# shuaigroup/Renormalizer

Hardware: AMD Instinct MI355X
Metric: TDVP-PS sweep site-updates/sec at (Nsite=50, Dbond=256, dphys=2/16) (higher is better)
Workload: dtype c128

## Files before the change

### include/mpsengine.h

```cpp
#ifndef MPSENGINE_H
#define MPSENGINE_H

#include <stddef.h>
#include <stdint.h>

#ifdef __cplusplus
extern "C" {
#endif

typedef struct mpse_ctx mpse_ctx;

enum {
  MPSE_OK = 0,
  MPSE_ERR_OOM = 1,
  MPSE_ERR_SHAPE = 2,
  MPSE_ERR_NOCONV = 3,
  MPSE_ERR_HIP = 4,
  MPSE_ERR_ARG = 5
};

enum { MPSE_F64 = 0, MPSE_C128 = 1 };
enum { MPSE_DOMAIN_L = 0, MPSE_DOMAIN_R = 1 };


// ... 6 lines not shown

int mpse_prof_get_ktiles(mpse_ctx* ctx, int variant, int64_t* ktiles);
int mpse_prof_get_svd_sweeps(mpse_ctx* ctx, int64_t* sweeps);
int mpse_prof_enable(mpse_ctx* ctx, int on);
int mpse_prof_reset(mpse_ctx* ctx);
int mpse_prof_get(mpse_ctx* ctx, int variant, double* total_ms, double* total_flops, double* total_bytes,
                  int64_t* launches);


int mpse_malloc(mpse_ctx* ctx, size_t bytes, void** dptr);
int mpse_free(mpse_ctx* ctx, void* dptr);
int mpse_pool_trim(mpse_ctx* ctx);
int mpse_mem_info(mpse_ctx* ctx, size_t* pool_bytes, size_t* in_use_bytes, size_t* device_free, size_t* device_total);
int mpse_memcpy_h2d(mpse_ctx* ctx, void* dst, const void* src_host, size_t bytes);
int mpse_memcpy_d2h(mpse_ctx* ctx, void* dst_host, const void* src, size_t bytes);
int mpse_memcpy_d2d(mpse_ctx* ctx, void* dst, const void* src, size_t bytes);
int mpse_memset_zero(mpse_ctx* ctx, void* dst, size_t bytes);
int mpse_memcpy_2d(mpse_ctx* ctx, void* dst, size_t dpitch, const void* src, size_t spitch, size_t width_bytes,
                   size_t height);

int mpse_cast_f64_to_c128(mpse_ctx* ctx, void* dst, const void* src, int64_t n);
int mpse_conj_inplace(mpse_ctx* ctx, void* x, int64_t n);
int mpse_scal(mpse_ctx* ctx, int dtype, void* x, int64_t n, double a_re, double a_im);
int mpse_axpy(mpse_ctx* ctx, int dtype, void* y, const void* x, int64_t n, double a_re, double a_im);
int mpse_mul_real(mpse_ctx* ctx, int dtype, void* x, const void* m_f64, int64_t n);
int mpse_davidson_precond(mpse_ctx* ctx, int dtype, void* out, const void* r, const void* hdiag_f64,
                          const void* mask_f64, int64_t n, double e, double shift);
int mpse_real_part(mpse_ctx* ctx, void* out_f64, const void* z_c128, int64_t n);
int mpse_dotc(mpse_ctx* ctx, int dtype, const void* x, const void* y, int64_t n, double* out_host);
int mpse_nrm2(mpse_ctx* ctx, int dtype, const void* x, int64_t n, double* out_host);

int mpse_scaled_rms(mpse_ctx* ctx, int dtype, const void* x, const void* y1, const void* y2, int64_t n, double rtol,
                    double atol, double* out_host);

int mpse_defer_begin(mpse_ctx* ctx, int list);
int mpse_defer_end(mpse_ctx* ctx);
int mpse_defer_arm(mpse_ctx* ctx, int list);
int mpse_defer_run(mpse_ctx* ctx, int list);
int mpse_defer_discard(mpse_ctx* ctx);


typedef struct {
  int64_t ext;
  int64_t lo_ext;
  int64_t s_hi;
  int64_t s_lo;
} mpse_index;

typedef struct {
  int dtype_a, dtype_b;
  int conj_a, conj_b;
  mpse_index m_a, k_a;
  mpse_index k_b, n_b;
  mpse_index m_c, n_c;
  int64_t batch;
  int64_t sb_a, sb_b, sb_c;
  double alpha_re, alpha_im;
  double beta_re, beta_im;
  int skip_zero_tiles;
} mpse_gemm_desc;

int mpse_gemm(mpse_ctx* ctx, const mpse_gemm_desc* desc, const void* A, const void* B, void* C);

int mpse_gemm_path_stats(mpse_ctx* ctx, int64_t* counts, int n);

int mpse_transpose_inner(mpse_ctx* ctx, int dtype, void* out, const void* in,
                         int64_t d0, int64_t d1, int64_t d2, int conj);


typedef struct {
  int64_t Dl_bra, Dl_ket;
  int64_t Dr_bra, Dr_ket;
  int64_t d0, d1;
  int64_t danc;
  int64_t wl, wm, wr;
  int64_t env_unit;
  int64_t danc1;
} mpse_dims;

int mpse_env_update(mpse_ctx* ctx, int dtype, int domain, const mpse_dims* dims,
                    const void* env, int env_dtype, const void* ket, const void* bra, int bra_conj,
                    const void* W, int w_dtype, void* out);

int mpse_env_update_multi(mpse_ctx* ctx, int dtype, int domain, const mpse_dims* dims, int n_mpo,
                          const int64_t* wl, const int64_t* wr, const void* env, int env_dtype,
                          const void* ket, const void* bra, int bra_conj, const void* const* W, int w_dtype, void* out);

int mpse_env_unit_channel(mpse_ctx* ctx, int dtype, const void* env, int64_t D, int64_t w, double tol,
                          int64_t* unit_host);

typedef struct {
  int nsite;
  mpse_dims dims;
  const void* L; int l_dtype;
  const void* R; int r_dtype;
  const void* W0; const void* W1; int w_dtype;
  int64_t l_unit, r_unit;
} mpse_heff;

int mpse_heff_apply(mpse_ctx* ctx, int dtype, const mpse_heff* h, const void* C, void* out);

int mpse_mpo_site_hint(mpse_ctx* ctx, const void* W_dev, const double* W_host_f64, int64_t wl, int64_t d, int64_t wr);

int mpse_heff_fused_stats(mpse_ctx* ctx, int64_t* bond_launches, int64_t* site_launches);

int mpse_heff_apply2(mpse_ctx* ctx, int dtype, const mpse_heff* h, const void* C, void* out);

enum { MPSE_LEG_UP = 0, MPSE_LEG_DOWN = 1 };
typedef struct {
  int64_t Dl, Dr, d_up, d_down;
  int64_t wl1, wr1, wl2, wr2;
  int leg1, leg2;
  int trans1, trans2;
  const void* L; int l_dtype;
  const void* R; int r_dtype;
  const void* W1; const void* W2; int w_dtype;
} mpse_heff_ft;

int mpse_heff_apply_ft(mpse_ctx* ctx, int dtype, const mpse_heff_ft* h, const void* C, void* out);

int mpse_env_update_ft(mpse_ctx* ctx, int dtype, int domain, const mpse_heff_ft* h, const void* env, int env_dtype,
                       const void* X, void* out);

int mpse_expm_centre_mask(mpse_ctx* ctx, const void* mask_dev, int64_t nbytes);

int mpse_expm_lanczos(mpse_ctx* ctx, int dtype, const mpse_heff* h, double dt_re, double dt_im,
                      const void* C, void* out, double rtol, double atol, int max_dim, int* nvec);
int mpse_expm_lanczos_batch(mpse_ctx* ctx, int dtype, int count, const mpse_heff* h, double dt_re, double dt_im,
                            const void* const* C, void* const* out, double rtol, double atol, int max_dim, int* nvec);
int mpse_expm_lanczos_batch_stats(mpse_ctx* ctx, int64_t* batched_members, int64_t* single_members);
int mpse_expm_lanczos_path_stats(mpse_ctx* ctx, int64_t* counts, int n);

int mpse_davidson(mpse_ctx* ctx, int dtype, const mpse_heff* h, int twolayer, const void* hdiag_f64,
                  const void* mask_f64, int nroots, int nguess, const void* guess, double tol, int max_cycle,
                  int max_space, double lindep, double shift, double* e_host, void* x_out, int* ncycle, int* nmatvec);

int mpse_pcg(mpse_ctx* ctx, int dtype, const mpse_heff* h, int twolayer, double shift, const void* diag_f64,
             const void* mask_f64, const void* b, void* x, double tol, int max_iter, int* iters_host,
             double* relres_host, double* lvalue_host);
int mpse_pcg_stats(mpse_ctx* ctx, int64_t* counts, int n);

int mpse_pcg_batch(mpse_ctx* ctx, int dtype, int count, const mpse_heff* h, int twolayer, const double* shift_host,
                   const void* const* diag_f64, const void* const* mask_f64, const void* const* b, void* const* x,
                   double tol, int max_iter, int* status_host, int* iters_host, double* relres_host,
                   double* lvalue_host);
int mpse_pcg_batch_stats(mpse_ctx* ctx, int64_t* counts, int n);
int mpse_pcg_batch_plan(int dtype, int64_t Dl, int64_t d, int64_t Dr, int64_t wl, int64_t wr, int64_t* info, int n);

int mpse_pcg_sum(mpse_ctx* ctx, int dtype, int nterms, const mpse_heff_ft* terms, const double* weights_host,
                 double shift, const void* diag_f64, const void* mask_f64, const void* b, void* x, double tol,
                 int max_iter, int* iters_host, double* relres_host, double* lvalue_host);
int mpse_pcg_sum_stats(mpse_ctx* ctx, int64_t* counts, int n);

int mpse_site_factor_ft(mpse_ctx* ctx, const mpse_heff_ft* h, void* S_f64);
int mpse_diag_ft(mpse_ctx* ctx, const mpse_heff_ft* h, const void* S_f64, double weight, double shift, int accumulate,
                 void* diag_f64);


int mpse_mps_overlap(mpse_ctx* ctx, int nsite, const void* const* bra, const int* bra_dtype, const void* const* ket,
                     const int* ket_dtype, const int64_t* dims , int conj_bra, double* out_re_im_host);
int mpse_mps_overlap_stats(mpse_ctx* ctx, int64_t* counts, int n);
int mpse_mps_overlap_plan(int nsite, const int64_t* dims, int any_complex, int64_t* info, int n);


int mpse_mps_sandwich(mpse_ctx* ctx, int nsite, const void* const* bra, const int* bra_dtype, const void* const* ket,
                      const int* ket_dtype, const void* const* W, const int* w_dtype, const int64_t* dims ,
// ... 60 lines not shown
```

### renormalizer_amd/csrc/mpse_contract.hip

```cpp
#include <deque>

#include "mpse_internal.h"
#include "mpse_plans.h"

using namespace mpse_plan;

namespace {

__device__ __forceinline__ long long off2(const mpse_index m, long long i) {
  if (m.lo_ext >= m.ext) return i * m.s_lo;
  const long long hi = i / m.lo_ext;
  return hi * m.s_hi + (i - hi * m.lo_ext) * m.s_lo;
}

template <typename T>
__global__ __launch_bounds__(256) void k_copy_strided(T* dst, const T* src, mpse_index mi, mpse_index ni, mpse_index mo,
                                                      mpse_index no, const int* skip) {
  if (skip && *skip) return;
  const long long nn = ni.ext;
  const long long total = mi.ext * nn;
  const long long stride = (long long)gridDim.x * blockDim.x;
  for (long long t = (long long)blockIdx.x * blockDim.x + threadIdx.x; t < total; t += stride) {
    const long long i = t / nn, j = t - i * nn;
    dst[off2(mo, i) + off2(no, j)] = src[off2(mi, i) + off2(ni, j)];
  }
}

template <bool CPLX>
__global__ __launch_bounds__(256) void k_unit_deviation(const double* env, int D, int w, unsigned long long* dev) {
  constexpr int E = CPLX ? 2 : 1;
  const int a = blockIdx.x;
  __shared__ double red[4];
  for (int b = 0; b < w; ++b) {
    const double* row = env + ((long long)a * w + b) * D * E;
    double m = 0.0;
    for (int c = threadIdx.x; c < D; c += 256) {
      double re = row[c * E] - (c == a ? 1.0 : 0.0);
      double v = fabs(re);
      if (!(v <= 1e300)) v = 1e300;
      if (CPLX) {
        double vi = fabs(row[c * E + 1]);
        if (!(vi <= 1e300)) vi = 1e300;
        v = fmax(v, vi);
      }
      m = fmax(m, v);
    }
    for (int o = 32; o > 0; o >>= 1) m = fmax(m, __shfl_xor(m, o));
    if ((threadIdx.x & 63) == 0) red[threadIdx.x >> 6] = m;
    __syncthreads();
    if (threadIdx.x == 0) {
      m = fmax(fmax(red[0], red[1]), fmax(red[2], red[3]));
      atomicMax(dev + b, (unsigned long long)__double_as_longlong(m));
    }
    __syncthreads();
  }
}

struct WsmArgs {
  const double* T1;
  double* T2;
  const double* W;
  int Da, d, wl, wr, N;
  const int* skip;
  const double* slices;
  long long slice_stride;
  int nslices, b_lo, b_hi;
};

template <bool CPLX>
__global__ __launch_bounds__(256) void k_wsmall(const WsmArgs g) {
  if (g.skip && *g.skip) return;
  constexpr int E = CPLX ? 2 : 1;
  __shared__ double s_w[16][16];
  const int nrow = g.wl * g.d, no = g.d * g.wr;
  {
    const int o = threadIdx.x >> 4, be = threadIdx.x & 15;
    double v = 0.0;
    if (o < no && be < nrow) {
      const int dd = o / g.wr, f = o - dd * g.wr, b = be / g.d, e = be - b * g.d;
      v = g.W[(((long long)b * g.d + dd) * g.d + e) * g.wr + f];
    }
    s_w[o][be] = v;
  }
  __syncthreads();
  const long long idx = (long long)blockIdx.x * 256 + threadIdx.x;
  if (idx >= (long long)g.Da * g.N) return;
  const int a = (int)(idx / g.N), n = (int)(idx - (long long)a * g.N);
  double xr[16], xi[16];
#pragma unroll
  for (int be = 0; be < 16; ++be) {
    xr[be] = 0.0;
    xi[be] = 0.0;
    if (be < nrow) {
      const int b = be / g.d, e = be - b * g.d;
      if (g.nslices > 0 && b >= g.b_lo && b < g.b_hi) {
        const double* src = g.slices + ((((long long)(b - g.b_lo) * g.Da + a) * g.d + e) * g.N + n) * E;
        for (int sl = 0; sl < g.nslices; ++sl) {
          xr[be] += src[0];
          if constexpr (CPLX) xi[be] += src[1];
          src += g.slice_stride * E;
        }
      } else {
        const double* src = g.T1 + ((((long long)b * g.Da + a) * g.d + e) * g.N + n) * E;
        xr[be] = src[0];
        if constexpr (CPLX) xi[be] = src[1];
      }
    }
// ... 57 lines not shown
  const int x0 = q * WM_CHUNK;
  for (int j = 0; j < g.ndst; ++j) {
    const WmixDstDev& D = g.dst[j];
    double ar[WM_CHUNK], ai[WM_CHUNK];
#pragma unroll
    for (int i = 0; i < WM_CHUNK; ++i) ar[i] = 0.0, ai[i] = 0.0;
    for (int t = 0; t < D.nterm; ++t) {
      const WmixTermDev& tm = D.term[t];
      const double* src = tm.src + ((long long)a * tm.s_a + k) * E;
      if (tm.ident) {
#pragma unroll
        for (int i = 0; i < WM_CHUNK; ++i)
          if (x0 + i < d) {
            const double* p = src + (long long)(x0 + i) * tm.s_d * E;
            ar[i] += p[0];
            if constexpr (CPLX) ai[i] += p[1];
          }
        continue;
      }
      const double* blk = s_blk + tm.slot * dd2;
      const int lo = tm.e_lo[q], hi = tm.e_hi[q];
      for (int e0 = lo; e0 < hi; e0 += 8) {
        double vr[8], vi[8];
#pragma unroll
        for (int u = 0; u < 8; ++u) {
          vr[u] = 0.0, vi[u] = 0.0;
          if (e0 + u < hi) {
            const double* p = src + (long long)(e0 + u) * tm.s_d * E;
            vr[u] = p[0];
            if constexpr (CPLX) vi[u] = p[1];
          }
        }
#pragma unroll
        for (int u = 0; u < 8; ++u)
          if (e0 + u < hi) {
#pragma unroll
            for (int i = 0; i < WM_CHUNK; ++i)
              if (x0 + i < d) {
                const double w = blk[(x0 + i) * d + e0 + u];
                ar[i] += w * vr[u];
                if constexpr (CPLX) ai[i] += w * vi[u];
              }
          }
      }
    }
    double* dst = D.dst + ((long long)a * D.s_a + k) * E;
#pragma unroll
    for (int i = 0; i < WM_CHUNK; ++i)
      if (x0 + i < d) {
        double* p = dst + (long long)(x0 + i) * D.s_d * E;
        if constexpr (CPLX)
          *reinterpret_cast<double2*>(p) = make_double2(ar[i], ai[i]);
        else
          p[0] = ar[i];
      }
  }
}

int copy_call(mpse_ctx* ctx, int dtype, const void* src, void* dst, mpse_index mi, mpse_index ni, mpse_index mo,
              mpse_index no, const int* skip) {
  const long long total = mi.ext * ni.ext;
  if (total <= 0) return MPSE_OK;
  long long nb = (total + 255) / 256;
  if (nb > 65536) nb = 65536;
  if (dtype == MPSE_C128)
    hipLaunchKernelGGL((k_copy_strided<double2>), dim3((unsigned)nb), dim3(256), 0, ctx->stream, (double2*)dst,
                       (const double2*)src, mi, ni, mo, no, skip);
  else
    hipLaunchKernelGGL((k_copy_strided<double>), dim3((unsigned)nb), dim3(256), 0, ctx->stream, (double*)dst,
                       (const double*)src, mi, ni, mo, no, skip);
  MPSE_HIP(ctx, hipGetLastError());
  return MPSE_OK;
}

struct PlanRun {
  mpse_ctx* ctx;
  int dtype;
  size_t es;
  const void* bufs[B_COUNT];
  SolveScope* sc;
  MatvecReq* mv;
  const int* skip;
  MatvecReq::Dot* dot;
  TmpBuf slices;
  int slices_used = 0;
  PlanRun(mpse_ctx* c, int dt, const void* const* b, SolveScope* s, MatvecReq* m)
      : ctx(c), dtype(dt), es(dtype_size(dt)), sc(s), mv(m), skip(s ? s->skip : nullptr),
        dot(m && m->dot.y ? &m->dot : nullptr), slices(c) {
    for (int i = 0; i < B_COUNT; ++i) bufs[i] = b[i];
  }
  template <class T>
  int resolve(int buf, int64_t off, int dt, T** p) const {
    if (!bufs[buf]) return mpse_fail(ctx, MPSE_ERR_ARG, "plan: missing buffer");
    *p = (T*)((char*)const_cast<void*>(bufs[buf]) + size_t(off) * dtype_size(dt));
    return MPSE_OK;
  }
};

int run_wsmall(PlanRun& r, const Step& s) {
  WsmArgs g;
  MPSE_TRY(r.resolve(s.a, s.a_off, s.dta, &g.W));
  MPSE_TRY(r.resolve(s.b, s.b_off, s.dtb, &g.T1));
  MPSE_TRY(r.resolve(s.c, s.c_off, s.dtb, &g.T2));
  g.Da = (int)s.w_Da, g.d = (int)s.w_d, g.wl = (int)s.w_wl, g.wr = (int)s.w_wr, g.N = (int)s.w_N;
  g.skip = r.skip;
  g.slices = r.slices_used > 0 ? r.slices.as<const double>() : nullptr;
  g.nslices = r.slices_used, g.slice_stride = s.slice_elems, g.b_lo = (int)s.slice_b_lo, g.b_hi = (int)s.slice_b_hi;
  r.slices_used = 0;
  const long long total = s.w_Da * s.w_N;
  const dim3 grid((unsigned)((total + 255) / 256));
  if (s.dtb == MPSE_C128)
    hipLaunchKernelGGL((k_wsmall<true>), grid, dim3(256), 0, r.ctx->stream, g);
  else
    hipLaunchKernelGGL((k_wsmall<false>), grid, dim3(256), 0, r.ctx->stream, g);
  MPSE_HIP(r.ctx, hipGetLastError());
  return MPSE_OK;
}

int run_wmix(PlanRun& r, const Step& s) {
  WmixArgs g;
  memset(&g, 0, sizeof(g));
  MPSE_TRY(r.resolve(s.b, 0, MPSE_F64, &g.W));
  g.ndst = (int)s.mix.size();
  g.Da = (int)s.wp_Da, g.d = (int)s.wp_d, g.wr = (int)s.wp_wr, g.Dk = (int)s.wp_Dk;
  g.nchunk = (g.d + WM_CHUNK - 1) / WM_CHUNK;
  g.skip = r.skip;
  int nslot = 0;
  for (int j = 0; j < g.ndst; ++j) {
    const WMixDst& q = s.mix[j];
    MPSE_TRY(r.resolve(q.dst, q.dst_off, r.dtype, &g.dst[j].dst));
    g.dst[j].s_a = q.s_a, g.dst[j].s_d = q.s_d, g.dst[j].nterm = q.nterm;
    for (int t = 0; t < q.nterm; ++t) {
      const WMixTerm& tm = q.term[t];
      WmixTermDev& o = g.dst[j].term[t];
      MPSE_TRY(r.resolve(tm.src, tm.src_off, r.dtype, &o.src));
      o.s_a = tm.s_a, o.s_d = tm.s_d, o.b = tm.b, o.f = tm.f, o.ident = tm.ident ? 1 : 0;
      o.slot = tm.ident ? 0 : nslot++;
      memcpy(o.e_lo, tm.e_lo, sizeof(o.e_lo));
      memcpy(o.e_hi, tm.e_hi, sizeof(o.e_hi));
    }
  }
  g.nslot = nslot;
  const size_t lds = size_t(nslot > 0 ? nslot : 1) * g.d * g.d * sizeof(double);
  if (lds > 64 * 1024) return mpse_fail(r.ctx, MPSE_ERR_SHAPE, "plan: MPO blocks of the elementwise step exceed the LDS");
  const long long total = (long long)s.wp_Da * g.nchunk * s.wp_Dk;
  const dim3 grid((unsigned)((total + 255) / 256));
  if (r.dtype == MPSE_C128)
    hipLaunchKernelGGL((k_wmix<true>), grid, dim3(256), lds, r.ctx->stream, g);
  else
    hipLaunchKernelGGL((k_wmix<false>), grid, dim3(256), lds, r.ctx->stream, g);
  ++r.ctx->gemm_paths[mpse_ctx::GP_WMIX];
  MPSE_HIP(r.ctx, hipGetLastError());
  return MPSE_OK;
}

int scan_flags(PlanRun& r, const ScanDesc& sd, TmpBuf& tmp, const unsigned char** flags, int* pitch, bool* stable) {
  if (!sd.on || !r.bufs[sd.buf]) return MPSE_OK;
  const char* ptr;
  MPSE_TRY(r.resolve(sd.buf, sd.off, sd.dt, &ptr));
  bool st = false;
  MPSE_TRY(occ_mask_get(r.ctx, r.sc, ptr, sd.dt, sd.r, sd.k, tmp, flags, pitch, &st));
  *stable = *stable && st;
  return MPSE_OK;
}

const unsigned char* centre_mask(const PlanRun& r, const Step& s, int* pitch) {
  const int64_t K = s.kb.ext, N = s.nb.ext;
  const int64_t nkw = ((K + 15) / 16 + 7) / 8, ntn = (N + 63) / 64;
  if (!r.sc || !r.sc->in_krylov(r.bufs[B_C]) || r.sc->cmask.bytes != ntn * nkw * 8) return nullptr;
  *pitch = (int)(nkw * 8);
  return static_cast<const unsigned char*>(r.sc->cmask.ptr);
}

int bind_epilogue_mix(PlanRun& r, const GGroupPlan& g, int i, GroupedDesc& gd) {
  if (gd.nmix > 0 || !r.bufs[g.wbuf]) return mpse_fail(r.ctx, MPSE_ERR_ARG, "plan: bad epilogue mix");
  gd.nmix = g.nmix, gd.mix_grp = i;
  gd.mix_w = r.bufs[g.wbuf];
  gd.mix_d = (int)g.mix_d, gd.mix_wr = (int)g.mix_wr, gd.mix_ld = g.mix_ld;
  for (int t = 0; t < g.nmix; ++t) {
    const EpiTerm& m = g.mix[t];
    MPSE_TRY(r.resolve(m.src, m.src_off, r.dtype, &gd.mix[t].src));
    gd.mix[t].b = m.b, gd.mix[t].f = m.f, gd.mix[t].delta = m.delta;
  }
  return MPSE_OK;
}

int run_ggemm(PlanRun& r, const Step& s) {
  GroupedDesc gd;
  gd.dta = s.dta, gd.dtb = s.dtb;
  gd.ma = s.ma, gd.ka = s.ka, gd.kb = s.kb, gd.nb = s.nb, gd.mc = s.mc, gd.nc = s.nc;
  gd.ngrp = (int)s.groups.size();
  TmpBuf MA(r.ctx), MB(r.ctx);
  const unsigned char *fa = nullptr, *fb = nullptr;
  bool stable = true;
  MPSE_TRY(scan_flags(r, s.scan_a, MA, &fa, &gd.am_pitch, &stable));
  MPSE_TRY(scan_flags(r, s.scan_b, MB, &fb, &gd.bm_pitch, &stable));
  int cm_pitch = 0;
  const unsigned char* cm = centre_mask(r, s, &cm_pitch);
  for (int i = 0; i < gd.ngrp; ++i) {
    const GGroupPlan& g = s.groups[i];
    GroupedGrp& o = gd.grp[i];
    MPSE_TRY(r.resolve(g.cbuf, g.c_off, r.dtype, &o.C));
    o.nseg = g.nseg;
    o.beta = g.beta;
    if (g.nmix > 0) MPSE_TRY(bind_epilogue_mix(r, g, i, gd));
    for (int q = 0; q < g.nseg; ++q) {
      const GSegPlan& sg = g.seg[q];
      MPSE_TRY(r.resolve(sg.abuf, sg.a_off, s.dta, &o.seg[q].A));
      MPSE_TRY(r.resolve(sg.bbuf, sg.b_off, s.dtb, &o.seg[q].B));
      if (fa && sg.am_row0 >= 0) o.seg[q].am = fa + size_t(sg.am_row0) * gd.am_pitch;
      if (sg.bm_kind == BM_SCAN && fb) {
        o.seg[q].bm = fb + sg.bm_kt0;
      } else if (sg.bm_kind == BM_CENTRE && cm) {
        o.seg[q].bm = cm;
        gd.bm_pitch = cm_pitch;
      }
    }
  }
  gd.masks_stable = stable;
  if (gd.ngrp == 1 && s.groups[0].split2) {
    if (!r.bufs[B_OUT2]) return mpse_fail(r.ctx, MPSE_ERR_ARG, "plan: missing second result");
    gd.split2 = true;
    gd.c2 = const_cast<void*>(r.bufs[B_OUT2]);
  }
  MPSE_TRY(gemm_grouped(r.ctx, gd, r.sc, s.completes ? r.dot : nullptr,
                        s.completes && r.mv && r.mv->out_mask.mask ? &r.mv->out_mask : nullptr));
  return MPSE_OK;
}

int run_product(PlanRun& r, const Step& s) {
  const int dtc = (s.dta == MPSE_C128 || s.dtb == MPSE_C128) ? MPSE_C128 : MPSE_F64;
  if (dtc != r.dtype)
    return mpse_fail(r.ctx, MPSE_ERR_ARG, "plan step dtype mismatch (got %d want %d)", dtc, r.dtype);
  const char *a, *b;
  char* c;
  MPSE_TRY(r.resolve(s.a, s.a_off, s.dta, &a));
  MPSE_TRY(r.resolve(s.b, s.b_off, s.dtb, &b));
  MPSE_TRY(r.resolve(s.c, s.c_off, dtc, &c));
  if (s.kind == K_COPY) return copy_call(r.ctx, dtc, a, c, s.ma, s.ka, s.mc, s.nc, r.skip);
  ProductReq rq;
  if (s.completes) rq.dot = r.dot;
  if (s.cin >= 0) {
    if (!r.bufs[s.cin]) return mpse_fail(r.ctx, MPSE_ERR_ARG, "plan: missing beta source");
    rq.cin = (const char*)r.bufs[s.cin] + size_t(s.cin_off) * dtype_size(dtc);
    rq.cin_m = s.mcin;
    rq.cin_n = s.ncin;
  }
  if (s.slices_to >= 0) {
    const size_t blk = size_t(s.mc.ext) * size_t(s.nc.ext) * dtype_size(dtc);
    if (r.slices.alloc(4 * blk) == MPSE_OK) {
      rq.slices = r.slices.p;
      rq.slices_cap = 4 * blk;
    }
  }
  MPSE_TRY(gemm_call(r.ctx, s.dta, s.dtb, s.conja, s.conjb, s.ma, s.ka, s.kb, s.nb, s.mc, s.nc, s.batch, s.sba, s.sbb,
                     s.sbc, a, b, c, 1.0, s.beta, s.skip_zero, r.sc, &rq));
  if (rq.slices_used > 0) r.slices_used = rq.slices_used;
  return MPSE_OK;
}

}

static int run_plan(mpse_ctx* ctx, int dtype, const Plan& p, const void* bufs_in[B_COUNT],
                    SolveScope* sc = nullptr, MatvecReq* mv = nullptr) {
  if (p.error) return mpse_fail(ctx, MPSE_ERR_SHAPE, "%s", p.error);
  TmpBuf t1(ctx), t2(ctx), t3(ctx);
  TmpBuf* tmp[3] = {&t1, &t2, &t3};
  PlanRun r(ctx, dtype, bufs_in, sc, mv);
  for (int i = 0; i < 3; ++i)
    if (p.tmp_elems[i]) {
      MPSE_TRY(tmp[i]->alloc(size_t(p.tmp_elems[i]) * r.es));
      r.bufs[B_T1 + i] = tmp[i]->p;
    }
  for (const Step& s : p.steps)
    MPSE_TRY(s.elementwise_w ? run_wsmall(r, s)
             : s.kind == K_WMIX ? run_wmix(r, s)
             : s.kind == K_GGEMM ? run_ggemm(r, s)
                                 : run_product(r, s));
  return MPSE_OK;
}

int heff_apply(mpse_ctx* ctx, int dtype, const mpse_heff* h, const void* C, void* out, SolveScope* sc,
               MatvecReq* mv) {
  if (!ctx || !h || !C || !out || !h->L || !h->R) return MPSE_ERR_ARG;
  MPSE_BIND(ctx);
  if (dtype != MPSE_C128 && (h->l_dtype == MPSE_C128 || h->r_dtype == MPSE_C128 || h->w_dtype == MPSE_C128))
    return mpse_fail(ctx, MPSE_ERR_ARG, "heff_apply: real centre with complex operator parts");
  std::shared_ptr<void> wi_keep;
  if (h->nsite == 1 && h->W0) {
    std::lock_guard<std::mutex> lock(ctx->pool_mu);
    auto it = ctx->wsite_info.find(h->W0);
    if (it != ctx->wsite_info.end()) wi_keep = it->second.info;
  }
  {
    bool taken = false;
    MPSE_TRY(heff_small_try(ctx, dtype, h, C, out, sc, mv, &taken));
    if (taken) return MPSE_OK;
    const WSiteInfo* wi0 = static_cast<const WSiteInfo*>(wi_keep.get());
    const bool wi_ok = wi0 && h->nsite == 1 && wi0->wl == h->dims.wl && wi0->d == h->dims.d0 && wi0->wr == h->dims.wr;
    MPSE_TRY(heff0_fused_try(ctx, dtype, h, C, wi_ok ? wi0->w.data() : nullptr, sc, mv, &taken));
    if (taken) return MPSE_OK;
  }
  MatvecReq::Parts* pr = mv && mv->parts.ptr ? &mv->parts : nullptr;
  const bool two_ok = pr && pr->cap_elems >= 2 * pr->n;
  Plan p = plan_heff(dtype, *h, static_cast<const WSiteInfo*>(wi_keep.get()), two_ok, fold_epi());
  if (pr) pr->used = 0;
  const void* bufs[B_COUNT] = {nullptr};
  bind_heff(bufs, *h, C, out);
  if (p.two_results) bufs[B_OUT2] = static_cast<char*>(pr->ptr) + size_t(pr->n) * dtype_size(dtype);
  MPSE_TRY(run_plan(ctx, dtype, p, bufs, sc, mv));
  if (p.two_results) pr->used = -2;
  return MPSE_OK;
}

extern "C" int mpse_heff_apply(mpse_ctx* ctx, int dtype, const mpse_heff* h, const void* C, void* out) {
  return heff_apply(ctx, dtype, h, C, out, nullptr, nullptr);
}

extern "C" int mpse_mpo_site_hint(mpse_ctx* ctx, const void* W_dev, const double* W_host, int64_t wl, int64_t d,
                                  int64_t wr) {
  if (!ctx || !W_dev) return MPSE_ERR_ARG;
  if (!W_host) {
    std::lock_guard<std::mutex> lock(ctx->pool_mu);
    ctx->wsite_info.erase(W_dev);
    return MPSE_OK;
  }
  if (wl <= 0 || d <= 0 || wr <= 0) return mpse_fail(ctx, MPSE_ERR_SHAPE, "mpo_site_hint: empty MPO site");
  std::shared_ptr<void> info = std::make_shared<WSiteInfo>(analyse_mpo_site(W_host, wl, d, wr));
  std::lock_guard<std::mutex> lock(ctx->pool_mu);
  ctx->wsite_info[W_dev] = mpse_ctx::WSiteEntry{info, size_t(wl) * size_t(d) * size_t(d) * size_t(wr) * sizeof(double)};
  return MPSE_OK;
}

extern "C" int mpse_env_update(mpse_ctx* ctx, int dtype, int domain, const mpse_dims* dims, const void* env,
                               int env_dtype, const void* ket, const void* bra, int bra_conj, const void* W,
                               int w_dtype, void* out) {
  if (!ctx || !dims || !env || !ket || !W || !out) return MPSE_ERR_ARG;
  if (MPSE_RECORDING(ctx)) {
    const mpse_dims dc = *dims;
    ctx->defer_ops[ctx->defer_recording].push_back([=] {
      return mpse_env_update(ctx, dtype, domain, &dc, env, env_dtype, ket, bra, bra_conj, W, w_dtype, out);
    });
    return MPSE_OK;
  }
  MPSE_BIND(ctx);
  if (dtype != MPSE_C128 && (env_dtype == MPSE_C128 || w_dtype == MPSE_C128))
    return mpse_fail(ctx, MPSE_ERR_ARG, "env_update: real sites with complex env/mpo");
  if (!bra) {
    bra = ket;
    if (dims->Dl_bra != dims->Dl_ket || dims->Dr_bra != dims->Dr_ket)
      return mpse_fail(ctx, MPSE_ERR_SHAPE, "env_update: bra==NULL needs equal bonds");
  }
  std::shared_ptr<void> wi_keep;
  {
    static const bool fold_on = [] {
      const char* e = getenv("MPSE_ENV_WFOLD");
      return !(e && e[0] == '0');
    }();
    std::lock_guard<std::mutex> lock(ctx->pool_mu);
    auto it = ctx->wsite_info.find(W);
    if (fold_on && it != ctx->wsite_info.end()) wi_keep = it->second.info;
  }
  Plan p = plan_env(dtype, domain, *dims, env_dtype, w_dtype, bra_conj, static_cast<const WSiteInfo*>(wi_keep.get()));
  const void* bufs[B_COUNT] = {nullptr};
  bind_env(bufs, env, ket, bra, out, 1, &W);
  return run_plan(ctx, dtype, p, bufs);
}

extern "C" int mpse_env_update_multi(mpse_ctx* ctx, int dtype, int domain, const mpse_dims* dims, int n_mpo,
                                     const int64_t* wl, const int64_t* wr, const void* env, int env_dtype,
                                     const void* ket, const void* bra, int bra_conj, const void* const* W, int w_dtype,
                                     void* out) {
  if (!ctx || !dims || !env || !ket || !W || !wl || !wr || !out) return MPSE_ERR_ARG;
  MPSE_BIND(ctx);
  if (n_mpo < 1 || n_mpo > 4) return mpse_fail(ctx, MPSE_ERR_ARG, "env_update_multi: 1 to 4 MPO layers, got %d", n_mpo);
  if (dtype != MPSE_C128 && (env_dtype == MPSE_C128 || w_dtype == MPSE_C128))
    return mpse_fail(ctx, MPSE_ERR_ARG, "env_update_multi: real sites with complex env/mpo");
  if (!bra) {
    bra = ket;
    if (dims->Dl_bra != dims->Dl_ket || dims->Dr_bra != dims->Dr_ket)
      return mpse_fail(ctx, MPSE_ERR_SHAPE, "env_update_multi: bra==NULL needs equal bonds");
  }
  Plan p = plan_env_multi(dtype, domain, *dims, n_mpo, wl, wr, env_dtype, w_dtype, bra_conj);
  for (int i = 0; i < n_mpo; ++i)
    if (!W[i]) return MPSE_ERR_ARG;
  const void* bufs[B_COUNT] = {nullptr};
  bind_env(bufs, env, ket, bra, out, n_mpo, W);
  return run_plan(ctx, dtype, p, bufs);
}

int heff_apply2(mpse_ctx* ctx, int dtype, const mpse_heff* h, const void* C, void* out, SolveScope* sc) {
  if (!ctx || !h || !C || !out || !h->L || !h->R || !h->W0) return MPSE_ERR_ARG;
  MPSE_BIND(ctx);
  if (dtype != MPSE_C128 && (h->l_dtype == MPSE_C128 || h->r_dtype == MPSE_C128 || h->w_dtype == MPSE_C128))
    return mpse_fail(ctx, MPSE_ERR_ARG, "heff_apply2: real centre with complex operator parts");
  Plan p = plan_heff2(dtype, *h);
  const void* bufs[B_COUNT] = {nullptr};
  bind_heff(bufs, *h, C, out);
  return run_plan(ctx, dtype, p, bufs, sc);
}

extern "C" int mpse_heff_apply2(mpse_ctx* ctx, int dtype, const mpse_heff* h, const void* C, void* out) {
  return heff_apply2(ctx, dtype, h, C, out, nullptr);
}

int heff_apply_ft(mpse_ctx* ctx, int dtype, const mpse_heff_ft* h, const void* C, void* out, SolveScope* sc) {
  if (!ctx || !h || !C || !out || !h->L || !h->R || !h->W1 || !h->W2) return MPSE_ERR_ARG;
  MPSE_BIND(ctx);
  if (dtype != MPSE_C128 && (h->l_dtype == MPSE_C128 || h->r_dtype == MPSE_C128 || h->w_dtype == MPSE_C128))
    return mpse_fail(ctx, MPSE_ERR_ARG, "heff_apply_ft: real centre with complex operator parts");
  Plan p = plan_heff_ft(dtype, *h);
  const void* bufs[B_COUNT] = {nullptr};
  bind_heff_ft(bufs, *h, C, out);
  return run_plan(ctx, dtype, p, bufs, sc);
}

extern "C" int mpse_heff_apply_ft(mpse_ctx* ctx, int dtype, const mpse_heff_ft* h, const void* C, void* out) {
  return heff_apply_ft(ctx, dtype, h, C, out, nullptr);
}

extern "C" int mpse_env_update_ft(mpse_ctx* ctx, int dtype, int domain, const mpse_heff_ft* h, const void* env,
                                  int env_dtype, const void* X, void* out) {
  if (!ctx || !h || !env || !X || !out || !h->W1 || !h->W2) return MPSE_ERR_ARG;
  MPSE_BIND(ctx);
  if (dtype != MPSE_C128 && (env_dtype == MPSE_C128 || h->w_dtype == MPSE_C128))
    return mpse_fail(ctx, MPSE_ERR_ARG, "env_update_ft: real site with complex env/mpo");
  Plan p = plan_env_ft(dtype, domain, *h, env_dtype);
  const void* const W[2] = {h->W1, h->W2};
  const void* bufs[B_COUNT] = {nullptr};
  bind_env(bufs, env, X, X, out, 2, W);
  return run_plan(ctx, dtype, p, bufs);
}

extern "C" int mpse_env_unit_channel(mpse_ctx* ctx, int dtype, const void* env, int64_t D, int64_t w, double tol,
                                     int64_t* unit_host) {
  if (!ctx || !env || !unit_host) return MPSE_ERR_ARG;
  MPSE_BIND(ctx);
  *unit_host = 0;
  if (D <= 0 || w <= 0 || w > 2048) return MPSE_OK;
  unsigned long long* dev = reinterpret_cast<unsigned long long*>(ctx->dscratch);
  MPSE_HIP(ctx, hipMemsetAsync(dev, 0, size_t(w) * sizeof(double), ctx->stream));
  if (dtype == MPSE_C128)
    hipLaunchKernelGGL((k_unit_deviation<true>), dim3((unsigned)D), dim3(256), 0, ctx->stream, (const double*)env, (int)D,
                       (int)w, dev);
  else
    hipLaunchKernelGGL((k_unit_deviation<false>), dim3((unsigned)D), dim3(256), 0, ctx->stream, (const double*)env,
                       (int)D, (int)w, dev);
  MPSE_HIP(ctx, hipGetLastError());
  if (w <= 1024) {
// ... 14 lines not shown
```

### renormalizer_amd/csrc/mpse_gemm.hip

```cpp
#include <cstdlib>

#include "mpse_device.h"
#include "mpse_internal.h"
#include "mpse_plans.h"

typedef double v4d __attribute__((ext_vector_type(4)));

static unsigned long long* gemm_trace_ptr(const mpse_ctx* ctx) {
  static const bool f0_only = [] {
    const char* e = getenv("MPSE_GEMM_TRACE_ONLY");
    return e && e[0] == 'f';
  }();
  return (ctx->prof_on && !f0_only) ? ctx->gemm_trace : nullptr;
}

namespace {

struct IdxMap {
  long long s_hi, s_lo;
  int ext, lo;
};

constexpr int GMAX_GRP = 8, GMAX_SEG = 4, GMAX_MIX = 8;
struct GMix {
  const double* src;
  int b, f, delta, pad;
};
struct GSeg {
  const double* A;
  const double* B;
  const unsigned char* am;
  const unsigned char* bm;
};
struct GGrp {
  GSeg seg[GMAX_SEG];
  double* C;
  int nseg;
  int use_beta;
};
struct GemmGroups {
  GGrp g[GMAX_GRP];
  int ngrp, tiles_m_grp, nkt_seg, am_pitch, bm_pitch;
  int split2, cpd;
  double* C2;
  const unsigned long long* flags;
  int nmix, mix_grp, mix_d, mix_wr;
  long long mix_ld;
  const double* mix_w;
  GMix mix[GMAX_MIX];
  const unsigned char* omask;
  int om_pitch, om_d;
  int dot4;
};

struct GemmArgs {
  const double* A;
  const double* B;
  double* C;
  IdxMap mA, kA, kB, nB, mC, nC;
  long long sbA, sbB, sbC;
  int M, N, K;
  int tiles_m, tiles_n;
  int mtiles_m, mtiles_n;
  int a_kfast, b_kfast;
  int conjA, conjB;
  int use_beta;
  double alpha_re, alpha_im, beta_re, beta_im;
  int skew;
  int die_group;
  int slice_fast;
  const int* perm;
  int ksplit;
  int kt_per_split;
  double* ws;
  const unsigned long long* amask;
  const unsigned long long* bmask;
  int nkw;
  unsigned long long* kt_counter;
  const int* skip;
  const double* dot_y;
  double* dot_part;
  const double* Cin;
  IdxMap mCin, nCin;
  unsigned long long* trace;
  GemmGroups gg;
};


__device__ __forceinline__ void dot_acc(double& re, double& im, double2 c, double2 y) {
  re += c.x * y.x + c.y * y.y;
  im += c.x * y.y - c.y * y.x;
}

__device__ __forceinline__ long long idx_off(const IdxMap& m, int i) {
  if (m.lo == 0x7fffffff) return (long long)i * m.s_lo;
  const int hi = i / m.lo;
  const int l = i - hi * m.lo;
  return (long long)hi * m.s_hi + (long long)l * m.s_lo;
}

__device__ __forceinline__ void trace_record(const GemmArgs& g, bool ca, bool cb, unsigned long long t0,
                                             unsigned long long rt0, unsigned long long t1, unsigned long long t2,
                                             unsigned long long t3, int ktd) {
  const unsigned long long slot = atomicAdd(g.trace, 1ull);
  if (slot >= GEMM_TRACE_CAP) return;
  unsigned long long* r = g.trace + 1 + slot * GEMM_TRACE_WORDS;
  r[0] = ((unsigned long long)gridDim.x << 32) | (unsigned long long)blockIdx.x;
  r[1] = ((unsigned long long)(ca ? 1 : 0) << 62) | ((unsigned long long)(cb ? 1 : 0) << 61) |
         ((unsigned long long)g.ksplit << 40) | ((unsigned long long)(unsigned)g.K << 8);
  const unsigned hw = __builtin_amdgcn_s_getreg((31 << 11) | 4), xc = __builtin_amdgcn_s_getreg((31 << 11) | 20);
  r[2] = (unsigned long long)(unsigned)ktd | ((unsigned long long)(((xc & 0xf) << 16) | (hw & 0xffff)) << 32);
  r[3] = t0;
  r[4] = t1;
  r[5] = t2;
  r[6] = t3;
  r[7] = __builtin_readcyclecounter();
  r[8] = rt0;
  r[9] = __builtin_amdgcn_s_memrealtime();
}

#ifndef MPSE_GEMM_3M
#define MPSE_GEMM_3M 1
#endif
constexpr int BM = 64, BN = 64, BK = 16, LDK = BK + 1;

template <bool CA, bool CB, bool KS, int WS, int WI = 2, bool GRP = false>
__global__ __launch_bounds__(64 * WS * WS * (2 / WI), WS == 1 ? 1 : WI == 1 ? 4 : ((CA && CB) ? 2 : 3)) void k_gemm(const GemmArgs g) {
  static_assert(!GRP || (KS && WS == 2), "grouped launches use the single-level 64 x 64 kernel");
  constexpr int TBM = 32 * WS, TBN = 32 * WS, NT = 64 * WS * WS * (2 / WI);
  static_assert(WI == 2 || (WI == 1 && WS == 2), "eight-wave form only for 64 x 64 tiles");
  constexpr int LD = WS == 2 ? 80 : 48;
  constexpr int NLD = TBM * BK / NT;
  constexpr bool CC = CA || CB;
  constexpr int EA = CA ? 2 : 1, EB = CB ? 2 : 1, EC = CC ? 2 : 1;
  __shared__ double smem[(2 + (CA ? 1 : 0) + (CB ? 1 : 0)) * BK * LD];
  if (g.skip && *g.skip) return;
  const unsigned long long tr0 = g.trace ? __builtin_readcyclecounter() : 0ull;
  const unsigned long long rt0 = g.trace ? __builtin_amdgcn_s_memrealtime() : 0ull;
  unsigned long long tr1 = 0, tr2 = 0, tr3 = 0;
  double* sAr = smem;
  double* sAi = sAr + BK * LD;
  double* sBr = smem + (CA ? 2 : 1) * BK * LD;
  double* sBi = sBr + BK * LD;

  const int tid = threadIdx.x;
  const int lane = tid & 63;
  const int wave = tid >> 6;
  const int wm = WS == 2 ? wave >> 1 : 0, wn = WS == 2 ? wave & 1 : 0;
  constexpr int WROWS = 16 * WI;

  const int ntile = g.tiles_m * g.tiles_n;
  const int bid = blockIdx.x;
  int bs = bid / ntile;
  int t = bid - bs * ntile;
  int half = 0;
  if constexpr (GRP) {
    if (g.gg.split2) {
      if ((ntile & 7) == 0) {
        const int m2 = 2 * (ntile >> 3), r = bid >> 3, cpd = g.gg.cpd;
        const int q = (r < cpd || m2 <= cpd) ? r : (m2 - 1) - (r - cpd);
        half = q & 1;
        t = ((q >> 1) << 3) | (bid & 7);
      } else {
        half = bid & 1;
        t = bid >> 1;
      }
      bs = half;
    }
  }
  if (g.slice_fast) {
    t = bid / g.ksplit;
    bs = bid - t * g.ksplit;
  }
  const int b = bs / g.ksplit;
  const int ks_id = bs - b * g.ksplit;
  bool dead = false;
  if (g.perm) {
    t = g.perm[(ks_id & 1) ? ntile - 1 - t : t];
    if constexpr (GRP) {
      dead = t < 0;
      t = dead ? ~t : t;
    }
  }
  int tm = t / g.tiles_n;
  int tn = t - tm * g.tiles_n;
  if constexpr (GRP) {
    if (dead) {
      if (g.dot_y && tid == 0) {
        const long long slot = (long long)bs * ntile + t;
        g.dot_part[2 * slot] = 0.0;
        g.dot_part[2 * slot + 1] = 0.0;
      }
      if (g.trace && tid == 0) trace_record(g, CA, CB, tr0, rt0, tr0, tr0, tr0, 0);
      return;
    }
  }
  if (g.die_group == 1) {
    const int x = t & 7, j = t >> 3;
    tm = x + 8 * (j / g.tiles_n);
    tn = j % g.tiles_n;
  } else if (g.die_group == 2) {
    const int x = t & 7, j = t >> 3;
    tn = x + 8 * (j / g.tiles_m);
    tm = j % g.tiles_m;
  }
  if (g.skew && !g.perm && !g.die_group) tn = (tn + tm) % g.tiles_n;

  int grp = 0;
  if constexpr (GRP) {
    grp = tm / g.gg.tiles_m_grp;
    tm -= grp * g.gg.tiles_m_grp;
  }
  const GGrp& gp = g.gg.g[grp];
  const double* A = GRP ? gp.seg[0].A : g.A + (long long)b * g.sbA * EA;
  const double* B = GRP ? gp.seg[0].B : g.B + (long long)b * g.sbB * EB;
  double* C = GRP ? (half ? g.gg.C2 : gp.C) : g.C + (long long)b * g.sbC * EC;

  int ai[NLD], ak[NLD], bj[NLD], bk[NLD];
  long long aoff[NLD], boff[NLD];
#pragma unroll
  for (int r = 0; r < NLD; ++r) {
    if (g.a_kfast) {
      ak[r] = tid % BK;
      ai[r] = tid / BK + (NT / BK) * r;
    } else {
      ai[r] = tid % TBM;
      ak[r] = tid / TBM + (NT / TBM) * r;
    }
    if (g.b_kfast) {
      bk[r] = tid % BK;
      bj[r] = tid / BK + (NT / BK) * r;
    } else {
      bj[r] = tid % TBN;
      bk[r] = tid / TBN + (NT / TBN) * r;
// ... 697 lines not shown
  __shared__ unsigned key[2048], ckey[2048];
  __shared__ int colw[2048];
  __shared__ unsigned char die_of[2048], dead[2048];
  const int ntile = tiles_m * tiles_n, tid = threadIdx.x;
  const bool part = by_die && tiles_n % 8 == 0 && tiles_n <= 2048;
  for (int c = tid; c < 2048; c += 1024) colw[c] = 0;
  __syncthreads();
  for (int i = tid; i < 2048; i += 1024) {
    unsigned cnt = 0;
    dead[i] = 0;
    if (i < ntile) {
      const int tm = i / tiles_n, tn = i - tm * tiles_n;
      if (gg.ngrp > 0) {
        const int grp = tm / gg.tiles_m_grp, tml = tm - grp * gg.tiles_m_grp;
        const GGrp& G = gg.g[grp];
        const bool off = gg.omask && !mpse_plan::out_tile_live(gg.omask, gg.om_pitch, gg.om_d, om_N, om_M, tm, tn);
        dead[i] = off ? 1 : 0;
        for (int q = 0; q < G.nseg; ++q)
          for (int l = 0; l < gg.nkt_seg; ++l) {
            unsigned v = off ? 0 : 1;
            if (G.seg[q].am) v &= G.seg[q].am[(long long)tml * gg.am_pitch + l];
            if (G.seg[q].bm) v &= G.seg[q].bm[(long long)tn * gg.bm_pitch + l];
            cnt += v;
            if (flags_out) flags_out[(long long)i * flags_pitch + q * gg.nkt_seg + l] = (unsigned char)v;
          }
        if (flags_out)
          for (int l = G.nseg * gg.nkt_seg; l < flags_pitch; ++l) flags_out[(long long)i * flags_pitch + l] = 0;
      } else {
        for (int w = 0; w < nkw; ++w) {
          unsigned long long x = 0x0101010101010101ull;
          if (amask) x &= amask[(long long)tm * nkw + w];
          if (bmask) x &= bmask[(long long)tn * nkw + w];
          const int valid = nkt - 8 * w;
          if (valid < 8) x &= (1ull << (8 * valid)) - 1ull;
          cnt += __popcll(x);
        }
      }
      if (part) atomicAdd(&colw[tn], (int)cnt);
    }
    key[i] = cnt;
  }
  __syncthreads();
  if (part) {
    for (int c = tid; c < 2048; c += 1024) ckey[c] = c < tiles_n ? ((unsigned)colw[c] << 11) | (unsigned)(2047 - c) : 0u;
    __syncthreads();
    bitonic_desc(ckey, tid, pow2_at_least(tiles_n));
    for (int r = tid; r < tiles_n; r += 1024) {
      const int c = 2047 - (int)(ckey[r] & 2047u), r16 = r & 15;
      die_of[c] = (unsigned char)(r16 < 8 ? r16 : 15 - r16);
    }
    __syncthreads();
  }
  for (int i = tid; i < 2048; i += 1024) {
    unsigned k = 0;
    if (i < ntile) {
      const unsigned die = part ? die_of[i % tiles_n] : 0u;
      k = (die << 28) | (key[i] << 16) | (unsigned)(0xFFFF - i);
    }
    key[i] = k;
  }
  __syncthreads();
  bitonic_desc(key, tid, pow2_at_least(ntile));
  const int per_die = ntile / 8;
  for (int i = tid; i < ntile; i += 1024) {
    const int s = part ? (7 - (i & 7)) * per_die + (i >> 3) : i;
    const int t = 0xFFFF - (int)(key[s] & 0xFFFFu);
    perm[i] = dead[t] ? ~t : t;
  }
}

template <bool CC>
__global__ __launch_bounds__(256) void k_splitk_reduce(const GemmArgs g, int batch) {
  constexpr int EC = CC ? 2 : 1;
  if (g.skip && *g.skip) return;
  const long long mn = (long long)g.M * g.N;
  const int rows = g.M * batch;
  double dre = 0.0, dim = 0.0;
  for (int row = blockIdx.y; row < rows; row += gridDim.y) {
    const int b = row / g.M;
    const int i = row - b * g.M;
    const double* wrow = g.ws + ((long long)b * g.ksplit * mn + (long long)i * g.N) * EC;
    double* crow = g.C + ((long long)b * g.sbC + idx_off(g.mC, i)) * EC;
    for (int j = blockIdx.x * 256 + threadIdx.x; j < g.N; j += gridDim.x * 256) {
      const double* w = wrow + (long long)j * EC;
      double xr = 0, xi = 0;
      int s = 0;
      for (; s + 4 <= g.ksplit; s += 4) {
        if constexpr (CC) {
          const double2 v0 = *reinterpret_cast<const double2*>(w + (long long)s * mn * EC);
          const double2 v1 = *reinterpret_cast<const double2*>(w + (long long)(s + 1) * mn * EC);
          const double2 v2 = *reinterpret_cast<const double2*>(w + (long long)(s + 2) * mn * EC);
          const double2 v3 = *reinterpret_cast<const double2*>(w + (long long)(s + 3) * mn * EC);
          xr += v0.x;
          xi += v0.y;
          xr += v1.x;
          xi += v1.y;
          xr += v2.x;
          xi += v2.y;
          xr += v3.x;
          xi += v3.y;
        } else {
          const double v0 = w[(long long)s * mn], v1 = w[(long long)(s + 1) * mn];
          const double v2 = w[(long long)(s + 2) * mn], v3 = w[(long long)(s + 3) * mn];
          xr += v0;
          xr += v1;
          xr += v2;
          xr += v3;
        }
      }
      for (; s < g.ksplit; ++s) {
        if constexpr (CC) {
          const double2 v = *reinterpret_cast<const double2*>(w + (long long)s * mn * EC);
          xr += v.x;
          xi += v.y;
        } else {
          xr += w[(long long)s * mn];
        }
      }
      const long long co = idx_off(g.nC, j);
      double* p = crow + co * EC;
      const double* pin = g.Cin ? g.Cin + (idx_off(g.mCin, i) + idx_off(g.nCin, j)) * EC : p;
      if constexpr (CC) {
        double2 o = make_double2(g.alpha_re * xr - g.alpha_im * xi, g.alpha_re * xi + g.alpha_im * xr);
        if (g.use_beta) {
          const double2 c0 = *reinterpret_cast<const double2*>(pin);
          o.x += g.beta_re * c0.x - g.beta_im * c0.y;
          o.y += g.beta_re * c0.y + g.beta_im * c0.x;
        }
        *reinterpret_cast<double2*>(p) = o;
        if (g.dot_y) dot_acc(dre, dim, o, reinterpret_cast<const double2*>(g.dot_y)[idx_off(g.mC, i) + co]);
      } else {
        double o = g.alpha_re * xr;
        if (g.use_beta) o += g.beta_re * (*pin);
        *p = o;
        if (g.dot_y) dre += o * g.dot_y[idx_off(g.mC, i) + co];
      }
    }
  }
  if (g.dot_y) {
    block_allsum2(dre, dim);
    if (threadIdx.x == 0) {
      const long long bid = (long long)blockIdx.y * gridDim.x + blockIdx.x;
      g.dot_part[2 * bid] = dre;
      g.dot_part[2 * bid + 1] = dim;
    }
  }
}

struct OccOperand {
  const double* base;
  IdxMap rmap, kmap;
  int nrows, tiles, cplx, kfast;
  long long sb;
  unsigned char* flags;
};
__global__ __launch_bounds__(256) void k_tile_occ(OccOperand oa, OccOperand ob, int K, int nkw, int batch,
                                                  const int* skip) {
  if (skip && *skip) return;
  const int wave = threadIdx.x >> 6, lane = threadIdx.x & 63;
  const int kt = blockIdx.x * 4 + wave, t = blockIdx.y;
  const bool second = (int)blockIdx.z >= batch;
  const OccOperand& o = second ? ob : oa;
  const int b = second ? blockIdx.z - batch : blockIdx.z;
  if (t >= o.tiles || kt * BK >= K) return;
  const int E = o.cplx ? 2 : 1;
  const double* base = o.base + (long long)b * o.sb * E;
  bool nz = false;
  if (o.kfast) {
    const int k = kt * BK + (lane & 15);
    const bool kin = k < K;
    const long long ko = idx_off(o.kmap, kin ? k : K - 1);
    double v0[16], v1[16];
#pragma unroll
    for (int i = 0; i < 16; ++i) {
      const int r = min(t * BM + i * 4 + (lane >> 4), o.nrows - 1);
      const double* q = base + (idx_off(o.rmap, r) + ko) * E;
      v0[i] = q[0];
      v1[i] = o.cplx ? q[1] : 0.0;
    }
#pragma unroll
    for (int i = 0; i < 16; ++i) {
      const bool in = (t * BM + i * 4 + (lane >> 4)) < o.nrows && kin;
      nz |= in && (v0[i] != 0.0 || v1[i] != 0.0);
    }
  } else {
    const int r = t * BM + lane;
    if (r < o.nrows) {
      const double* p = base + idx_off(o.rmap, r) * E;
      double v0[16], v1[16];
#pragma unroll
      for (int i = 0; i < 16; ++i) {
        const int k = min(kt * BK + i, K - 1);
        const double* q = p + idx_off(o.kmap, k) * E;
        v0[i] = q[0];
        v1[i] = o.cplx ? q[1] : 0.0;
      }
#pragma unroll
      for (int i = 0; i < 16; ++i) nz |= (kt * BK + i < K) && (v0[i] != 0.0 || v1[i] != 0.0);
    }
  }
  const bool any = __ballot(nz) != 0ull;
  if (lane == 0) o.flags[((long long)b * o.tiles + t) * nkw * 8 + kt] = any ? 1 : 0;
}

bool to_map(const mpse_index& s, IdxMap* m) {
  if (s.ext < 0 || s.ext > 0x7fffffffLL) return false;
  m->ext = (int)s.ext;
  long long lo = s.lo_ext <= 0 ? 1 : s.lo_ext;
  m->s_hi = s.s_hi;
  m->s_lo = s.s_lo;
  if (lo >= s.ext) {
    m->s_hi = 0;
  } else if (lo == 1) {
    m->s_lo = s.s_hi;
    m->s_hi = 0;
    lo = s.ext;
  } else if (s.s_hi == lo * s.s_lo) {
    m->s_hi = 0;
    lo = s.ext;
  }
  if (lo >= s.ext) lo = 0x7fffffffLL;
  m->lo = (int)lo;
  return true;
}

inline bool is_single(const IdxMap& m) { return m.lo == 0x7fffffff; }

template <bool CPLX>
__global__ __launch_bounds__(256) void k_transpose_inner(double* out, const double* in, long long d0, int d1,
                                                         int d2, int conj) {
  constexpr int E = CPLX ? 2 : 1;
// ... 37 lines not shown
    return double((x.ext - 1) / x.lo) * double(x.s_hi) + double(x.lo - 1) * double(x.s_lo);
  };
  return (span(m) + span(k) + 1.0) * (cplx ? 16.0 : 8.0) < 4.0e9;
}
bool fast_ok(const GemmArgs& g, bool ca, bool cb) { return span_ok(g.mA, g.kA, ca) && span_ok(g.nB, g.kB, cb); }

bool fill_maps(GemmArgs& g, const mpse_index& ma, const mpse_index& ka, const mpse_index& kb, const mpse_index& nb,
               const mpse_index& mc, const mpse_index& nc) {
  if (!to_map(ma, &g.mA) || !to_map(ka, &g.kA) || !to_map(kb, &g.kB) || !to_map(nb, &g.nB) || !to_map(mc, &g.mC) ||
      !to_map(nc, &g.nC))
    return false;
  g.M = g.mA.ext, g.N = g.nB.ext, g.K = g.kA.ext;
  g.tiles_m = g.mtiles_m = (g.M + BM - 1) / BM;
  g.tiles_n = g.mtiles_n = (g.N + BN - 1) / BN;
  g.a_kfast = fastest(g.kA) <= fastest(g.mA);
  g.b_kfast = fastest(g.kB) <= fastest(g.nB);
  return true;
}

SolveScope::OccKey occ_key(const void* p, const IdxMap& rm, const IdxMap& km, long long sb, long long batch, bool cplx) {
  SolveScope::OccKey k;
  memset(&k, 0, sizeof(k));
  k.ptr = p;
  k.r_ext = rm.ext, k.r_lo = rm.lo, k.r_shi = rm.s_hi, k.r_slo = rm.s_lo;
  k.k_ext = km.ext, k.k_lo = km.lo, k.k_shi = km.s_hi, k.k_slo = km.s_lo;
  k.sb = sb, k.nrows = rm.ext, k.tiles = (rm.ext + BM - 1) / BM, k.nkw = ((km.ext + BK - 1) / BK + 7) / 8;
  k.batch = (int)batch, k.K = km.ext, k.cplx = cplx ? 1 : 0;
  return k;
}
size_t occ_bytes(const SolveScope::OccKey& k) { return size_t(k.batch) * k.tiles * k.nkw * 8; }

struct OccMask {
  void* mask = nullptr;
  bool scan = false;
  bool stable = true;
};
int occ_mask_source(mpse_ctx* ctx, SolveScope* keep, const SolveScope::OccKey& key, const void* given, void* tmp,
                    OccMask* m) {
  m->stable = keep || given;
  if (keep)
    for (const auto& e : keep->occ_cache)
      if (memcmp(&e.key, &key, sizeof(key)) == 0) {
        m->mask = e.mask;
        return MPSE_OK;
      }
  m->scan = !given;
  if (given) {
    m->mask = const_cast<void*>(given);
  } else if (keep) {
    MPSE_TRY(mpse_malloc(ctx, occ_bytes(key), &m->mask));
    keep->occ_cache.push_back({key, m->mask});
  } else {
    m->mask = tmp;
  }
  return MPSE_OK;
}
OccOperand occ_operand(const SolveScope::OccKey& k, const IdxMap& rm, const IdxMap& km, int kfast, const OccMask& m) {
  return OccOperand{static_cast<const double*>(k.ptr), rm, km, k.nrows, m.scan ? k.tiles : 0, k.cplx, kfast, k.sb,
                    static_cast<unsigned char*>(m.mask)};
}

int perm_source(mpse_ctx* ctx, SolveScope* keep, SolveScope::PermEntry key, size_t bytes, TmpBuf& tmp, int** perm,
                bool* sort) {
  *sort = false;
  if (keep)
    for (const auto& e : keep->perm_cache)
      if (e.amask == key.amask && e.bmask == key.bmask && e.tiles_m == key.tiles_m && e.tiles_n == key.tiles_n &&
          e.nkt == key.nkt) {
        *perm = static_cast<int*>(e.perm);
        return MPSE_OK;
      }
  *sort = true;
  if (keep) {
    MPSE_TRY(mpse_malloc(ctx, bytes, &key.perm));
    keep->perm_cache.push_back(key);
    *perm = static_cast<int*>(key.perm);
  } else {
    MPSE_TRY(tmp.alloc(bytes));
    *perm = tmp.as<int>();
  }
  return MPSE_OK;
}

void launch_gemm(mpse_ctx* ctx, const GemmArgs& g, long long nwg, bool ca, bool cb, bool fast, bool wide, bool grouped,
                 dim3 rgrid = dim3(0), int batch = 1) {
  using Kern = void (*)(const GemmArgs);
  static const Kern plain[4][3] = {
      {k_gemm<true, true, true, 2, 1>, k_gemm<true, true, true, 2>, k_gemm<true, true, false, 2>},
      {k_gemm<true, false, true, 2, 1>, k_gemm<true, false, true, 2>, k_gemm<true, false, false, 2>},
      {k_gemm<false, true, true, 2, 1>, k_gemm<false, true, true, 2>, k_gemm<false, true, false, 2>},
      {k_gemm<false, false, true, 2, 1>, k_gemm<false, false, true, 2>, k_gemm<false, false, false, 2>}};
  static void (*const reduce[2])(const GemmArgs, int) = {k_splitk_reduce<true>, k_splitk_reduce<false>};
  static const Kern groups[2][2] = {
      {k_gemm<true, true, true, 2, 1, true>, k_gemm<true, true, true, 2, 2, true>},
      {k_gemm<false, true, true, 2, 1, true>, k_gemm<false, true, true, 2, 2, true>}};
  const int form = fast && wide ? 0 : fast ? 1 : 2;
  const Kern k = grouped ? groups[ca ? 0 : 1][form] : plain[(ca ? 0 : 2) + (cb ? 0 : 1)][form];
  hipLaunchKernelGGL(k, dim3((unsigned)nwg), dim3(form == 0 ? 512 : 256), 0, ctx->stream, g);
  if (rgrid.x) hipLaunchKernelGGL(reduce[(ca || cb) ? 0 : 1], rgrid, dim3(256), 0, ctx->stream, g, batch);
}

void count_paths(long long* gp, const mpse_plan::GemmPlan& p, bool batched) {
  const bool masked = p.fast && p.masks;
  ++gp[mpse_ctx::GP_LAUNCH];
  gp[mpse_ctx::GP_GENERAL] += !p.fast;
  gp[mpse_ctx::GP_WIDE] += p.wide;
  gp[mpse_ctx::GP_SPLIT_B1] += p.ksplit > 1 && !batched;
  gp[mpse_ctx::GP_SPLIT_BN] += p.ksplit > 1 && batched;
  gp[mpse_ctx::GP_DIE1] += p.die_group == 1;
  gp[mpse_ctx::GP_DIE2] += p.die_group == 2;
  gp[mpse_ctx::GP_SKEW] += !p.order && !p.die_group;
  gp[mpse_ctx::GP_ORDER] += p.order;
  gp[mpse_ctx::GP_MASK] += masked;
  gp[mpse_ctx::GP_MASK_GLOBAL] += masked && p.nkw > 64;
}
void count_paths(long long* gp, const GroupedDesc& d) {
  ++gp[mpse_ctx::GP_GROUPED];
  gp[mpse_ctx::GP_GROUPED_SPLIT2] += d.split2;
  gp[mpse_ctx::GP_GROUPED_MIX] += d.nmix > 0;
}

}

static int gemm_impl(mpse_ctx* ctx, const mpse_gemm_desc* d, const void* A, const void* B, void* C, int skip_zero,
                     SolveScope* sc, ProductReq* rq) {
  if (!ctx || !d) return MPSE_ERR_ARG;
  MPSE_BIND(ctx);
  if ((d->dtype_a != MPSE_F64 && d->dtype_a != MPSE_C128) || (d->dtype_b != MPSE_F64 && d->dtype_b != MPSE_C128))
    return mpse_fail(ctx, MPSE_ERR_ARG, "mpse_gemm: unknown dtype");
  if (d->m_a.ext != d->m_c.ext || d->n_b.ext != d->n_c.ext || d->k_a.ext != d->k_b.ext)
    return mpse_fail(ctx, MPSE_ERR_SHAPE, "mpse_gemm: extents disagree (M %lld/%lld N %lld/%lld K %lld/%lld)",
                     (long long)d->m_a.ext, (long long)d->m_c.ext, (long long)d->n_b.ext, (long long)d->n_c.ext,
                     (long long)d->k_a.ext, (long long)d->k_b.ext);
  if (d->m_a.ext == 0 || d->n_b.ext == 0 || d->batch <= 0) return MPSE_OK;
  if (!A || !B || !C) return mpse_fail(ctx, MPSE_ERR_ARG, "mpse_gemm: null operand");
  GemmArgs g = {};
  g.A = (const double*)A;
  g.B = (const double*)B;
  g.C = (double*)C;
  if (!fill_maps(g, d->m_a, d->k_a, d->k_b, d->n_b, d->m_c, d->n_c))
    return mpse_fail(ctx, MPSE_ERR_SHAPE, "mpse_gemm: extent out of range");
  g.sbA = d->sb_a;
  g.sbB = d->sb_b;
  g.sbC = d->sb_c;
  const bool ca = d->dtype_a == MPSE_C128, cb = d->dtype_b == MPSE_C128;
  g.conjA = d->conj_a && ca;
  g.conjB = d->conj_b && cb;
  g.alpha_re = d->alpha_re;
  g.alpha_im = d->alpha_im;
  g.beta_re = d->beta_re;
  g.beta_im = d->beta_im;
  g.use_beta = (d->beta_re != 0.0 || d->beta_im != 0.0);
  if (rq && rq->cin) {
    if (d->batch != 1 || !g.use_beta || !to_map(rq->cin_m, &g.mCin) || !to_map(rq->cin_n, &g.nCin) ||
        g.mCin.ext != g.mC.ext || g.nCin.ext != g.nC.ext)
      return mpse_fail(ctx, MPSE_ERR_ARG, "mpse_gemm: beta source needs batch == 1, beta != 0 and the extents of C");
    g.Cin = static_cast<const double*>(rq->cin);
  }
  g.skip = sc ? sc->skip : nullptr;
  g.skew = 1;
  if (!ctx->gemm_trace_checked) {
    ctx->gemm_trace_checked = true;
    if (getenv("MPSE_GEMM_TRACE")) {
      void* pt = nullptr;
      if (hipMalloc(&pt, (1 + GEMM_TRACE_CAP * GEMM_TRACE_WORDS) * sizeof(unsigned long long)) == hipSuccess) {
        (void)hipMemsetAsync(pt, 0, sizeof(unsigned long long), ctx->stream);
        ctx->gemm_trace = static_cast<unsigned long long*>(pt);
      }
    }
  }
  g.trace = gemm_trace_ptr(ctx);

  MatvecReq::Dot* dot = rq ? rq->dot : nullptr;
  const bool compact = is_single(g.mC) && is_single(g.nC) && g.mC.s_lo == g.N && (g.nC.s_lo == 1 || g.N == 1);
  const bool slices = rq && rq->slices && compact && d->alpha_re == 1.0 && d->alpha_im == 0.0;
  const mpse_plan::GemmPlan p = mpse_plan::launch_plan(
      {g.M, g.N, g.K, d->batch, n_cu_of(ctx), ca, cb, skip_zero, is_single(g.kA) && is_single(g.kB), fast_ok(g, ca, cb),
       dot != nullptr, dot ? dot->cap : 0, slices, slices ? rq->slices_cap : 0, g.use_beta != 0});
  if (p.nwg > 0x7fffffffLL) return mpse_fail(ctx, MPSE_ERR_SHAPE, "mpse_gemm: grid too large");
  g.ksplit = p.ksplit;
  g.kt_per_split = p.kt_per_split;
  g.slice_fast = g.ksplit > 1 && d->batch == 1;
  g.die_group = p.die_group;
  TmpBuf WSB(ctx), MSK(ctx), PERM(ctx);
  if (p.leave_slices) {
    g.ws = static_cast<double*>(rq->slices);
    rq->slices_used = g.ksplit;
  } else if (g.ksplit > 1) {
    MPSE_TRY(WSB.alloc(p.ws_bytes));
    g.ws = WSB.as<double>();
  }
  if (p.dot_producers) {
    g.dot_y = static_cast<const double*>(dot->y);
    g.dot_part = dot->part;
    dot->nb_out = (int)p.dot_producers;
  }
  mpse_ctx::ProfRec rec;
  const int variant = (ca ? 1 : 0) + (cb ? 2 : 0);
  const double mnk = double(g.M) * double(g.N) * double(g.K) * double(d->batch);
  const bool prof_this = prof_begin(
      ctx, variant, mnk * ((ca && cb) ? 8.0 : (ca || cb) ? 4.0 : 2.0),
      double(d->batch) * (double(g.M) * g.K * (ca ? 16 : 8) + double(g.K) * g.N * (cb ? 16 : 8) +
                          double(g.M) * g.N * ((ca || cb) ? 16 : 8) * (g.use_beta ? 2 : 1)),
      &rec);
  g.kt_counter = prof_this && ctx->prof_ktiles ? ctx->prof_ktiles + variant : nullptr;

  OccMask ma, mb;
  if (p.masks) {
    g.nkw = p.nkw;
    const bool sa = skip_zero & 1, sb = skip_zero & 2;
    const SolveScope::OccKey ka = occ_key(g.A, g.mA, g.kA, g.sbA, d->batch, ca);
    const SolveScope::OccKey kb = occ_key(g.B, g.nB, g.kB, g.sbB, d->batch, cb);
    SolveScope* const keep_a = sa && sc && sc->in_env(g.A) ? sc : nullptr;
    SolveScope* const keep_b = sb && sc && sc->in_env(g.B) ? sc : nullptr;
    const void* centre = (sb && sc && sc->in_krylov(g.B) && d->batch == 1 && (long long)occ_bytes(kb) == sc->cmask.bytes)
                             ? sc->cmask.ptr : nullptr;
    const size_t tmp_a = sa && !keep_a ? occ_bytes(ka) : 0, tmp_b = sb && !keep_b && !centre ? occ_bytes(kb) : 0;
    if (tmp_a + tmp_b) MPSE_TRY(MSK.alloc(tmp_a + tmp_b));
    if (sa) MPSE_TRY(occ_mask_source(ctx, keep_a, ka, nullptr, MSK.p, &ma));
    if (sb) MPSE_TRY(occ_mask_source(ctx, keep_b, kb, centre, MSK.as<char>() + tmp_a, &mb));
    if (ma.scan || mb.scan) {
      const OccOperand oa = occ_operand(ka, g.mA, g.kA, g.a_kfast, ma), ob = occ_operand(kb, g.nB, g.kB, g.b_kfast, mb);
      const dim3 og((p.nkt + 3) / 4, oa.tiles > ob.tiles ? oa.tiles : ob.tiles, (unsigned)(2 * d->batch));
      hipLaunchKernelGGL(k_tile_occ, og, dim3(256), 0, ctx->stream, oa, ob, g.K, g.nkw, (int)d->batch, g.skip);
    }
    g.amask = static_cast<const unsigned long long*>(ma.mask);
    g.bmask = static_cast<const unsigned long long*>(mb.mask);
  }

  if (p.order) {
    SolveScope* const keep = sc && sc->keeps_env_masks && ma.stable && mb.stable ? sc : nullptr;
    int* pp = nullptr;
    bool sort = false;
    MPSE_TRY(perm_source(ctx, keep, {g.amask, g.bmask, g.tiles_m, g.tiles_n, p.nkt, nullptr},
                         size_t(g.tiles_m) * g.tiles_n * sizeof(int), PERM, &pp, &sort));
    if (sort)
      hipLaunchKernelGGL(k_tile_order, dim3(1), dim3(1024), 0, ctx->stream, g.amask, g.bmask, g.nkw, p.nkt, g.tiles_m,
                         g.tiles_n, 1, pp, g.skip, GemmGroups(), (unsigned char*)nullptr, 0, 0, 0);
    g.perm = pp;
  }

  count_paths(ctx->gemm_paths, p, d->batch > 1);
  const bool reduce = g.ksplit > 1 && !p.leave_slices;
  launch_gemm(ctx, g, p.nwg, ca, cb, p.fast, p.wide, false, reduce ? dim3((unsigned)p.rgx, (unsigned)p.rgy) : dim3(0),
              (int)d->batch);
  if (prof_this) prof_end(ctx, rec);
  MPSE_HIP(ctx, hipGetLastError());
  return MPSE_OK;
}

int occ_mask_get(mpse_ctx* ctx, SolveScope* sc, const void* ptr, int dtype, mpse_index r, mpse_index k,
                 TmpBuf& tmp, const unsigned char** flags, int* pitch, bool* stable) {
  IdxMap rm, km;
  if (!to_map(r, &rm) || !to_map(k, &km) || !is_single(km))
    return mpse_fail(ctx, MPSE_ERR_SHAPE, "occupancy scan: K index must be single level");
  const SolveScope::OccKey key = occ_key(ptr, rm, km, 0, 1, dtype == MPSE_C128);
  SolveScope* const keep = sc && sc->in_env(ptr) ? sc : nullptr;
  OccMask m;
  if (!keep) MPSE_TRY(tmp.alloc(occ_bytes(key)));
  MPSE_TRY(occ_mask_source(ctx, keep, key, nullptr, tmp.p, &m));
  if (m.scan) {
    const OccOperand oa = occ_operand(key, rm, km, fastest(km) <= fastest(rm), m);
    OccOperand ob = oa;
    ob.tiles = 0;
    hipLaunchKernelGGL(k_tile_occ, dim3(((key.K + BK - 1) / BK + 3) / 4, key.tiles, 2), dim3(256), 0, ctx->stream, oa, ob,
                       key.K, key.nkw, 1, sc ? sc->skip : nullptr);
    MPSE_HIP(ctx, hipGetLastError());
  }
  *flags = static_cast<const unsigned char*>(m.mask);
  *pitch = key.nkw * 8;
  *stable = m.stable;
  return MPSE_OK;
}

static double grouped_bytes(const GroupedDesc& d, double M, double N, double K, bool ca) {
  const void* seen[3][GMAX_GRP * GMAX_SEG + GMAX_MIX];
  int n[3] = {0, 0, 0};
  auto fresh = [&](int w, const void* p) {
    for (int i = 0; i < n[w]; ++i)
      if (seen[w][i] == p) return false;
    seen[w][n[w]++] = p;
    return true;
  };
  double bytes = 0.0, betas = 0.0;
  for (int i = 0; i < d.ngrp; ++i) {
    for (int q = 0; q < d.grp[i].nseg; ++q) {
      if (fresh(0, d.grp[i].seg[q].A)) bytes += M * K * (ca ? 16.0 : 8.0);
      if (fresh(1, d.grp[i].seg[q].B)) bytes += K * N * 16.0;
    }
    bytes += M * N * 16.0;
    betas += d.grp[i].beta != 0.0 ? 1.0 : 0.0;
  }
  if (d.nmix > 0) {
    betas -= 1.0;
    const int w = (K == N && ca) ? 0 : 2;
    for (int t = 0; t < d.nmix; ++t)
      if (fresh(w, d.mix[t].src)) bytes += M * N * 16.0;
  }
  return bytes + betas * M * N * 16.0;
}

int gemm_grouped(mpse_ctx* ctx, const GroupedDesc& d, SolveScope* sc, MatvecReq::Dot* dot,
                 const MatvecReq::OutMask* om) {
  GemmArgs g = {};
  if (d.ngrp < 1 || d.ngrp > GMAX_GRP) return mpse_fail(ctx, MPSE_ERR_ARG, "grouped product: 1 .. %d groups", GMAX_GRP);
  if (!fill_maps(g, d.ma, d.ka, d.kb, d.nb, d.mc, d.nc))
    return mpse_fail(ctx, MPSE_ERR_SHAPE, "grouped product: extent out of range");
  if (g.M != g.mC.ext || g.N != g.nC.ext || g.K != g.kB.ext) return mpse_fail(ctx, MPSE_ERR_SHAPE, "grouped product: extents disagree");
  if (g.M == 0 || g.N == 0) return MPSE_OK;
  const bool ca = d.dta == MPSE_C128, cb = d.dtb == MPSE_C128;
  if (!is_single(g.kA) || !is_single(g.kB) || !fast_ok(g, ca, cb) || g.K % BK != 0 || g.K < BK ||
      (d.ngrp > 1 && g.M % BM != 0) || !cb)
    return mpse_fail(ctx, MPSE_ERR_SHAPE, "grouped product: needs single-level K indices, K a multiple of %d, group "
                     "heights a multiple of %d and a complex second operand", BK, BM);
  if (d.split2 && (d.ngrp != 1 || !d.c2 || g.M % BM != 0))
    return mpse_fail(ctx, MPSE_ERR_ARG, "grouped product: halved tiles need one group, whole tile rows and a second result");
  g.alpha_re = 1.0, g.beta_re = 1.0;
  g.ksplit = 1;
  g.skip = sc ? sc->skip : nullptr;
  g.skew = 1;
  g.trace = gemm_trace_ptr(ctx);
  GemmGroups& gg = g.gg;
// ... 154 lines not shown
```

### renormalizer_amd/csrc/mpse_internal.h

```cpp
#pragma once
#include <hip/hip_runtime.h>

#include <cstdarg>
#include <cstdlib>
#include <cstdint>
#include <cstdio>
#include <cstring>
#include <functional>
#include <map>
#include <memory>
#include <mutex>
#include <string>
#include <unordered_map>
#include <vector>

#include "../../include/mpsengine.h"

struct mpse_ctx {
  int device = 0;
  hipStream_t stream = nullptr;
  int n_cu = 0;
  char err[512] = {0};
  char dev_name[128] = {0};

  std::mutex pool_mu;
  std::multimap<size_t, void*> free_blocks;
  std::unordered_map<void*, size_t> live;
  size_t pool_bytes = 0;
  size_t in_use_bytes = 0;
  unsigned long long n_device_allocs = 0;

  struct ProfRec {
    hipEvent_t e0, e1;
    int variant;
    double flops, bytes;
  };
  bool prof_on = false;
  int prof_stride = 1;
  long long prof_counter = 0;
  std::vector<ProfRec> prof_pending;
  std::vector<hipEvent_t> prof_free_events;
  static constexpr int PROF_NVAR = 8;
  int64_t prof_svd_sweeps = 0;
  double prof_ms[PROF_NVAR] = {0};
  double prof_flops[PROF_NVAR] = {0};
  double prof_bytes[PROF_NVAR] = {0};
  int64_t prof_launches[PROF_NVAR] = {0};
  unsigned long long* prof_ktiles = nullptr;

  char* stage = nullptr;
  char* stage_dev = nullptr;
  size_t stage_size = 0, stage_pos = 0;

  enum PinnedSlot {
    PIN_SCALAR2 = 0,
    PIN_FLAG = 8,
    PIN_LZ_SCAL = 16,
    PIN_LZ_CTL = 24,
    PIN_ENV_UNIT = 32,
    PIN_PCG_CTL = 40,
    PIN_DAVIDSON = 64,
    PIN_BATCH_CTL = 3700,
    PIN_QR_STATUS = 3990,
    PIN_SLOTS_END = 4000,
    PIN_DOUBLES = 4096,
    PIN_SEQ = PIN_DOUBLES - 1
  };
  double* pinned = nullptr;
  double* pinned_dev = nullptr;
  unsigned long long publish_seq = 0;
  double* dscratch = nullptr;
  unsigned int flag_gen = 0;
  std::unordered_map<unsigned long long, int> lz_hint;
  struct WSiteEntry {
    std::shared_ptr<void> info;
    size_t bytes = 0;
  };
  std::unordered_map<const void*, WSiteEntry> wsite_info;
  std::vector<std::function<int()>> defer_ops[2];
  int defer_recording = -1;
  int defer_armed = -1;
  bool defer_hold = false;
  std::vector<void*> defer_frees;
  struct CMask {
    const void* ptr = nullptr;
    long long bytes = 0;
  } cmask_pending;
  unsigned long long* gemm_trace = nullptr;
  bool gemm_trace_checked = false;
  long long f0_launches[2] = {0, 0};
  enum GemmPath {
    GP_LAUNCH, GP_GENERAL, GP_WIDE, GP_SPLIT_B1, GP_SPLIT_BN, GP_DIE1, GP_DIE2, GP_SKEW, GP_ORDER, GP_MASK,
    GP_MASK_GLOBAL, GP_GROUPED, GP_GROUPED_SPLIT2, GP_GROUPED_MIX, GP_WMIX, GP_GROUPED_OUTMASK, GP_COUNT
  };
  long long gemm_paths[GP_COUNT] = {0};
  long long qr_chol_calls = 0, qr_chol_fallbacks = 0, qr_calls = 0;
  bool qr_optimistic = false;
  int qr_scheme = -1;
  int* qr_words_dev = nullptr;
  long long lz_batch_members = 0, lz_batch_single = 0;
  enum LzPath {
    LP_SYNC, LP_ASYNC_DONE, LP_HOST_FIRST, LP_HOST_LATER, LP_LIMIT, LP_BD_ASYNC, LP_BD_SYNC, LP_FULL, LP_CONV,
    LP_NOCONV, LP_MERGED, LP_WAITS, LP_GROW, LP_PARTS, LP_VMASK, LP_UNVEC, LP_RESCALE, LP_ALIAS_RESTART, LP_COUNT
  };
  long long lz_paths[LP_COUNT] = {0};
  enum PcgStat {
    PS_SOLVES, PS_ITERS, PS_MATVECS, PS_WAITS, PS_END_TOL, PS_END_MAXITER, PS_END_CURVATURE, PS_TWOLAYER, PS_MASKED,
    PS_COUNT
  };
  long long pcg_stats[PS_COUNT] = {0};
  enum PcgSumStat { PSS_SOLVES, PSS_ITERS, PSS_TERM_APPLIES, PSS_WAITS, PSS_DIAGS, PSS_COUNT };
  long long pcg_sum_stats[PSS_COUNT] = {0};
  enum PcgBatchStat { PB_MEMBERS, PB_SINGLE, PB_SETS, PB_MATVEC_LAUNCHES, PB_WAITS, PB_COUNT };
  long long pcg_batch_stats[PB_COUNT] = {0};
  enum OverlapStat { OV_CHAIN, OV_ENQUEUED, OV_SITES, OV_COUNT };
  long long overlap_stats[OV_COUNT] = {0};
  enum SandwichStat { SW_CHAIN, SW_ENQUEUED, SW_SITES, SW_COUNT };
  long long sandwich_stats[SW_COUNT] = {0};
  enum CorrStat { CR_CHAIN, CR_ENQUEUED, CR_SITES, CR_ENTRIES, CR_COUNT };
  long long corr_stats[CR_COUNT] = {0};
  enum Rdm1Stat { RD_CHAIN, RD_ENQUEUED, RD_SITES, RD_MATRICES, RD_COUNT };
  long long rdm1_stats[RD_COUNT] = {0};
  enum Rdm2Stat { RD2_CHAIN, RD2_ENQUEUED, RD2_SITES, RD2_PAIRS, RD2_COUNT };
  long long rdm2_stats[RD2_COUNT] = {0};
};
int qr_words(mpse_ctx* ctx);

int mpse_fail(mpse_ctx* ctx, int code, const char* fmt, ...);
inline int mpse_bind(mpse_ctx* ctx) {
  int cur = -1;
  if (hipGetDevice(&cur) == hipSuccess && cur == ctx->device) return MPSE_OK;
  if (hipSetDevice(ctx->device) != hipSuccess) return mpse_fail(ctx, MPSE_ERR_HIP, "hipSetDevice(%d) failed", ctx->device);
  return MPSE_OK;
}
int stage_h2d(mpse_ctx* ctx, void* dst, const void* src_host, size_t bytes);
int device_zero(mpse_ctx* ctx, void* dst, size_t bytes);
inline void wsite_written(mpse_ctx* ctx, const void* dst, size_t bytes) {
  if (!dst || !bytes) return;
  std::lock_guard<std::mutex> lock(ctx->pool_mu);
  if (ctx->wsite_info.empty()) return;
  const char* lo = static_cast<const char*>(dst);
  for (auto it = ctx->wsite_info.begin(); it != ctx->wsite_info.end();) {
    const char* w = static_cast<const char*>(it->first);
    if (lo < w + it->second.bytes && w < lo + bytes)
      it = ctx->wsite_info.erase(it);
    else
      ++it;
  }
}
void prof_drain(mpse_ctx* ctx);
bool prof_begin(mpse_ctx* ctx, int variant, double flops, double bytes, mpse_ctx::ProfRec* rec);
void prof_end(mpse_ctx* ctx, const mpse_ctx::ProfRec& rec);
struct ProfScope {
  mpse_ctx* ctx;
  mpse_ctx::ProfRec rec;
  bool on;
  ProfScope(mpse_ctx* c, int variant, double flops, double bytes) : ctx(c), on(prof_begin(c, variant, flops, bytes, &rec)) {}
  ProfScope(const ProfScope&) = delete;
  ProfScope& operator=(const ProfScope&) = delete;
  void end() {
    if (on) prof_end(ctx, rec);
    on = false;
  }
  ~ProfScope() {
    if (!on) return;
    ctx->prof_free_events.push_back(rec.e0);
    ctx->prof_free_events.push_back(rec.e1);
  }
};

#define MPSE_HIP(ctx, call)                                                              \
  do {                                                                                   \
    hipError_t _e = (call);                                                              \
    if (_e != hipSuccess)                                                                \
      return mpse_fail((ctx), (_e == hipErrorOutOfMemory) ? MPSE_ERR_OOM : MPSE_ERR_HIP, \
                       "%s:%d %s -> %s", __FILE__, __LINE__, #call, hipGetErrorString(_e)); \
// ... 54 lines not shown
  mpse_ctx* ctx;
  const int* skip = nullptr;
  bool keeps_env_masks = false;
  const char* env_lo[2] = {nullptr, nullptr};
  const char* env_hi[2] = {nullptr, nullptr};
  mpse_ctx::CMask cmask;
  const char* krylov_lo = nullptr;
  const char* krylov_hi = nullptr;

  struct OccKey {
    const void* ptr;
    long long r_ext, r_lo, r_shi, r_slo, k_ext, k_lo, k_shi, k_slo, sb;
    int nrows, tiles, nkw, batch, K, cplx;
  };
  struct OccEntry {
    OccKey key;
    void* mask;
  };
  std::vector<OccEntry> occ_cache;
  struct PermEntry {
    const void *amask, *bmask;
    int tiles_m, tiles_n, nkt;
    void* perm;
  };
  std::vector<PermEntry> perm_cache;
  struct SmallRt {
    const void* src = nullptr;
    void* rt = nullptr;
    size_t bytes = 0;
  } small_rt;
  struct F0Cache {
    void* buf = nullptr;
    const void *L = nullptr, *R = nullptr, *W = nullptr, *cmask = nullptr;
    int Dl = 0, Dr = 0, w = 0, nsite = -1;
  } f0;

  explicit SolveScope(mpse_ctx* c) : ctx(c) {}
  SolveScope(const SolveScope&) = delete;
  SolveScope& operator=(const SolveScope&) = delete;
  ~SolveScope() {
    for (auto& e : occ_cache) mpse_free(ctx, e.mask);
    for (auto& e : perm_cache) mpse_free(ctx, e.perm);
    if (f0.buf) mpse_free(ctx, f0.buf);
    if (small_rt.rt) mpse_free(ctx, small_rt.rt);
  }
  bool in_env(const void* p) const {
    const char* c = static_cast<const char*>(p);
    return keeps_env_masks && ((c >= env_lo[0] && c < env_hi[0]) || (c >= env_lo[1] && c < env_hi[1]));
  }
  bool in_krylov(const void* p) const {
    const char* c = static_cast<const char*>(p);
    return cmask.ptr && c && c >= krylov_lo && c < krylov_hi;
  }
};

struct MatvecReq {
  struct Dot {
    const void* y = nullptr;
    double* part = nullptr;
    int cap = 0;
    int nb_out = 0;
  } dot;
  struct Parts {
    void* ptr = nullptr;
    long long cap_elems = 0, n = 0;
    int used = 0;
    bool masked_ok = false;
    const unsigned long long* mask = nullptr;
    int mask_row = 0, mask_tiles = 0;
  } parts;
  struct OutMask {
    const unsigned char* mask = nullptr;
    int row = 0, pitch = 0;
  } out_mask;
};

struct ProductReq {
  MatvecReq::Dot* dot = nullptr;
  const void* cin = nullptr;
  mpse_index cin_m{}, cin_n{};
  void* slices = nullptr;
  size_t slices_cap = 0;
  int slices_used = 0;
};

int heff_apply(mpse_ctx* ctx, int dtype, const mpse_heff* h, const void* C, void* out, SolveScope* sc,
               MatvecReq* mv);
int heff_apply2(mpse_ctx* ctx, int dtype, const mpse_heff* h, const void* C, void* out, SolveScope* sc);
int heff_apply_ft(mpse_ctx* ctx, int dtype, const mpse_heff_ft* h, const void* C, void* out, SolveScope* sc);
int heff_small_try(mpse_ctx* ctx, int dtype, const mpse_heff* h, const void* C, void* out, SolveScope* sc,
                   MatvecReq* mv, bool* taken);

struct BatchMember {
  const void* L;
  const void* R;
  const void* W;
  void* Rt;
  const void* C;
  void* out;
};
template <class T>
__host__ __device__ inline T* member_ptr(T* p, unsigned m, long long mstride) {
  return p ? reinterpret_cast<T*>(reinterpret_cast<uintptr_t>(p) + uintptr_t(m) * uintptr_t(mstride)) : p;
}
bool heff_small_batch_plan(const mpse_heff* h, int dtype, int64_t n, int dot_cap, size_t* rt_bytes, int* nparts,
                           int* nb_dot);
int heff_small_batch_rt(mpse_ctx* ctx, int dtype, const mpse_heff* h, int B, const BatchMember* mem, const int* skip0,
                        long long mstride);
int heff_small_batch_apply(mpse_ctx* ctx, int dtype, const mpse_heff* h, int B, const BatchMember* mem,
                           const void* C0, void* parts0, int64_t n, double* dot_part0, int dot_cap, const int* skip0,
                           long long mstride);
constexpr int SM2_WMAX = 8;
constexpr int SM2_DMAX = 16;
constexpr int SM2_BMAX = 64;
constexpr int SM2_LDS_MAX = 65536;
constexpr int SM2_NNZ_LDS = 1024;
struct Small2Plan {
  int Dl, Dr, d, wl, wr;
  int jh, nslice, G;
  int rows, pitch, nnz_lds;
  int ptr_dbl, idx_dbl, csr_dbl;
  int off_A, off_B;
  int lds;
};
struct Pcg2Member {
  const double *L, *R, *W;
  double* Lt;
  int *csr_ptr, *csr_idx;
  double* csr_val;
  const double *mask, *diag, *b;
  double *x, *y, *q, *r, *p;
  double *part_bb, *part_pq, *part_bx, *part_rz0, *part_rz1;
  void* ctl;
  double shift;
};
bool small2_plan(int dtype, int64_t Dl, int64_t d, int64_t Dr, int64_t wl, int64_t wr, Small2Plan* p);
int small2_prep(mpse_ctx* ctx, int dtype, const Small2Plan& p, int B, const Pcg2Member* mem);
int small2_apply(mpse_ctx* ctx, int dtype, const Small2Plan& p, int B, const Pcg2Member* mem, int mode);
int heff0_fused_parts(const mpse_heff* h, int dtype);
int heff0_fused_try(mpse_ctx* ctx, int dtype, const mpse_heff* h, const void* C, const double* w_host,
                    SolveScope* sc, MatvecReq* mv, bool* taken);

int gemm_call(mpse_ctx* ctx, int dta, int dtb, int conja, int conjb, mpse_index ma, mpse_index ka,
              mpse_index kb, mpse_index nb, mpse_index mc, mpse_index nc, int64_t batch, int64_t sba,
              int64_t sbb, int64_t sbc, const void* A, const void* B, void* C, double alpha = 1.0,
              double beta = 0.0, int skip_zero = 0, SolveScope* sc = nullptr, ProductReq* rq = nullptr);

struct GroupedSeg {
  const void* A = nullptr;
  const void* B = nullptr;
  const unsigned char* am = nullptr;
  const unsigned char* bm = nullptr;
};
struct GroupedMixTerm {
  const void* src = nullptr;
  int b = 0, f = 0, delta = 0;
};
struct GroupedGrp {
  GroupedSeg seg[4];
  void* C = nullptr;
  int nseg = 0;
  double beta = 0.0;
};
struct GroupedDesc {
  int dta = MPSE_F64, dtb = MPSE_F64;
  mpse_index ma{}, ka{}, kb{}, nb{}, mc{}, nc{};
// ... 53 lines not shown
```

### renormalizer_amd/csrc/mpse_plans.h

```cpp
#pragma once
#include <cassert>
#include <cstdint>
#include <cstdlib>
#include <algorithm>
#include <cstring>
#include <utility>
#include <vector>

#include "../../include/mpsengine.h"

namespace mpse_plan {

enum Buf { B_L = 0, B_R, B_W0, B_W1, B_C, B_BRA, B_OUT, B_T1, B_T2, B_T3, B_W2, B_W3, B_OUT2, B_COUNT };
inline int w_buf(int layer) { return layer == 0 ? B_W0 : layer == 1 ? B_W1 : layer == 2 ? B_W2 : B_W3; }

enum Kind { K_GEMM = 0, K_COPY = 1, K_WMIX = 2, K_GGEMM = 3 };


constexpr int G_MAXGRP = 8, G_MAXSEG = 4, WM_MAXDST = 4, WM_MAXTERM = 4;
constexpr int EPI_MAXTERM = 8, EPI_MAXBAND = 2;

struct WBlock {
  int b, f;
  bool ident;
// ... 14 lines not shown
        for (int64_t e = 0; e < d; ++e) {
          const double v = w[((b * d + x) * d + e) * wr + f];
          if (v != 0.0) any = true;
          if (v != (x == e ? 1.0 : 0.0)) ident = false;
        }
      if (any) r.blocks.push_back(WBlock{(int)b, (int)f, ident});
    }
  return r;
}

constexpr int WM_CHUNK = 4, WM_MAXCHUNKS = 8;
struct WMixTerm {
  int b = 0, f = 0;
  bool ident = false;
  int src = 0;
  int64_t src_off = 0, s_a = 0, s_d = 0;
  unsigned char e_lo[WM_MAXCHUNKS] = {0}, e_hi[WM_MAXCHUNKS] = {0};
};
struct WMixDst {
  int dst = 0;
  int64_t dst_off = 0, s_a = 0, s_d = 0;
  int nterm = 0;
  WMixTerm term[WM_MAXTERM];
};
enum BMaskKind { BM_NONE = 0, BM_SCAN = 1, BM_CENTRE = 2 };
struct GSegPlan {
  int abuf = 0;
  int64_t a_off = 0;
  int bbuf = 0;
  int64_t b_off = 0;
  int64_t am_row0 = -1;
  int bm_kind = BM_NONE;
  int64_t bm_kt0 = 0;
};
struct EpiTerm {
  int src = 0;
  int64_t src_off = 0;
  int b = 0, f = 0;
  int delta = 0;
};
struct GGroupPlan {
  int nseg = 0;
  GSegPlan seg[G_MAXSEG];
  int cbuf = 0;
  int64_t c_off = 0;
  double beta = 0.0;
  int nmix = 0;
  EpiTerm mix[EPI_MAXTERM];
  int wbuf = B_W0;
  int64_t mix_d = 0, mix_wr = 0, mix_ld = 0;
  bool split2 = false;
};
struct ScanDesc {
  bool on = false;
  int buf = 0, dt = MPSE_F64;
  int64_t off = 0;
  mpse_index r{}, k{};
};

struct Step {
  int a, b, c;
  int64_t a_off, b_off, c_off;
  int dta, dtb;
  int conja, conjb;
  mpse_index ma, ka, kb, nb, mc, nc;
  int64_t batch, sba, sbb, sbc;
  int kind = K_GEMM;
  double beta = 0.0;
  int skip_zero = 0;
  bool is_wstep = false;
  int64_t w_Da = 0, w_wl = 0, w_d = 0, w_wr = 0, w_N = 0;
  std::vector<WMixDst> mix;
  int64_t wp_Da = 0, wp_d = 0, wp_Dk = 0, wp_wr = 0;
  std::vector<GGroupPlan> groups;
  ScanDesc scan_a, scan_b;
  int cin = -1;
  int64_t cin_off = 0;
  mpse_index mcin{}, ncin{};
  bool elementwise_w = false;
  int slices_to = -1;
  int64_t slice_b_lo = 0, slice_b_hi = 0;
  int64_t slice_elems = 0;
  bool completes = false;
};

struct Plan {
  std::vector<Step> steps;
  int64_t tmp_elems[3] = {0, 0, 0};
  bool two_results = false;
  const char* error = nullptr;
};

inline mpse_index i1(int64_t ext, int64_t stride) { return mpse_index{ext, ext > 0 ? ext : 1, 0, stride}; }
inline mpse_index i2(int64_t hi, int64_t lo, int64_t s_hi, int64_t s_lo) {
  return mpse_index{hi * lo, lo > 0 ? lo : 1, s_hi, s_lo};
}

constexpr int VIEW_MAXDIM = 8;
struct View {
  int buf = 0, dt = MPSE_F64;
  int64_t off = 0;
  int n = 0;
  char lab[VIEW_MAXDIM] = {0};
  int64_t ex[VIEW_MAXDIM] = {0}, st[VIEW_MAXDIM] = {0};
  View() {}
  View(int b, int d, std::initializer_list<std::pair<char, int64_t>> l) : buf(b), dt(d) {
    assert(l.size() <= size_t(VIEW_MAXDIM));
    for (auto& q : l) lab[n] = q.first, ex[n] = q.second, ++n;
    int64_t s = 1;
    for (int i = n; i-- > 0;) st[i] = s, s *= ex[i];
  }
  int find(char c) const {
    for (int i = 0; i < n; ++i)
      if (lab[i] == c) return i;
    return -1;
  }
  int64_t ext(char c) const {
    const int i = find(c);
    return i < 0 ? -1 : ex[i];
  }
  int64_t stride(char c) const {
    const int i = find(c);
    return i < 0 ? 0 : st[i];
  }
  View sub(char c, int64_t first, int64_t count) const {
    View v = *this;
    const int i = find(c);
    assert(i >= 0);
    v.off += first * st[i], v.ex[i] = count;
    return v;
  }
  View as(const char* labels) const {
    View v = *this;
    for (int i = 0; i < n && labels[i]; ++i) v.lab[i] = labels[i];
    return v;
  }
};

inline bool labels_index(const View& v, const char* labels, mpse_index* out) {
  int64_t le[2], ls[2], total = 1;
  int nl = 0;
  for (const char* c = labels; *c; ++c) {
    const int i = v.find(*c);
    if (i < 0) return false;
    const int64_t e = v.ex[i], st = v.st[i];
    total *= e;
    if (e == 1) continue;
    if (nl > 0 && ls[nl - 1] == e * st) {
      le[nl - 1] *= e, ls[nl - 1] = st;
    } else {
      if (nl == 2) return false;
      le[nl] = e, ls[nl] = st, ++nl;
    }
  }
  *out = nl == 0 ? i1(total, 1) : nl == 1 ? i1(le[0], ls[0]) : i2(le[0], le[1], ls[0], ls[1]);
  return true;
}

inline bool product_maps(Step& s, const View& A, const View& B, const View& C, const char* m, const char* k, const char* n) {
  return labels_index(A, m, &s.ma) && labels_index(A, k, &s.ka) && labels_index(B, k, &s.kb) && labels_index(B, n, &s.nb) &&
         labels_index(C, m, &s.mc) && labels_index(C, n, &s.nc);
}

inline Step* contract(Plan& p, const View& A, const View& B, const View& C, const char* m, const char* k, const char* n,
                      const char* batch = "", const char* loops = "", int conja = 0) {
  if (p.error) return nullptr;
// ... 423 lines not shown
  for (int64_t b = 0; b < (int64_t)a.tmp_of.size(); ++b) {
    if (a.direct_f[b] < 0 && a.tmp_of[b] < 0) continue;
    const View Lb = a.L.sub('b', b, 1), dst = a.direct_f[b] >= 0 ? a.dest(a.direct_f[b]) : a.T1.sub('t', a.tmp_of[b], 1);
    GGroupPlan g;
    g.nseg = 1;
    g.seg[0].abuf = Lb.buf, g.seg[0].a_off = Lb.off, g.seg[0].am_row0 = b * (a.L.ext('a') / 64);
    g.seg[0].bbuf = a.C.buf, g.seg[0].b_off = a.C.off, g.seg[0].bm_kind = BM_CENTRE;
    g.cbuf = dst.buf, g.c_off = dst.off;
    ga.groups.push_back(g);
  }
  if (!ga.groups.empty()) p.steps.push_back(ga);
}

inline void fold_emit_mix(Plan& p, const FoldAnalysis& a) {
  Step mix{};
  mix.kind = K_WMIX;
  mix.b = B_W0;
  mix.dta = a.C.dt, mix.dtb = MPSE_F64;
  mix.wp_Da = a.L.ext('a'), mix.wp_d = a.C.ext('x'), mix.wp_Dk = a.C.ext('k'), mix.wp_wr = a.R.ext('f');
  for (int64_t f : a.mixed) {
    const View dst = a.dest(f);
    WMixDst q;
    q.dst = dst.buf, q.dst_off = dst.off, q.s_a = dst.stride('a'), q.s_d = dst.stride('x');
    for (const WBlock* k : a.by_f[f]) q.term[q.nterm++] = wmix_term(*a.wi, *k, a.src(k->b));
    mix.mix.push_back(q);
  }
  if (!mix.mix.empty()) p.steps.push_back(mix);
}

inline void fold_emit_r(Plan& p, const FoldAnalysis& a) {
  Step gc{};
  gc.kind = K_GGEMM;
  gc.dta = a.C.dt, gc.dtb = a.R.dt;
  product_maps(gc, a.T2, a.R, a.OUT, "ax", "k", "l");
  gc.batch = 1;
  gc.scan_b.on = true;
  gc.scan_b.buf = a.R.buf, gc.scan_b.dt = a.R.dt, gc.scan_b.off = a.R.off;
  labels_index(a.R, "l", &gc.scan_b.r), labels_index(a.R, "fk", &gc.scan_b.k);
  std::vector<GSegPlan> segs;
  for (int64_t f = 0; f < (int64_t)a.present.size(); ++f) {
    if (!a.present[f] || f == a.ru) continue;
    const View P = a.alias[f] ? a.C : a.T2.sub('p', a.plane_of[f], 1), Rf = a.R.sub('f', f, 1);
    GSegPlan sg;
    sg.abuf = P.buf, sg.a_off = P.off;
    sg.bbuf = Rf.buf, sg.b_off = Rf.off;
    sg.bm_kind = BM_SCAN, sg.bm_kt0 = f * (a.R.ext('k') / 16);
    segs.push_back(sg);
  }
  for (size_t i = 0; i < segs.size(); i += G_MAXSEG) {
    Step st = gc;
    GGroupPlan g;
    g.cbuf = a.OUT.buf, g.c_off = a.OUT.off;
    g.beta = (a.out_init || i > 0) ? 1.0 : 0.0;
    if (a.split2) g.split2 = true, p.two_results = true;
    for (size_t j = i; j < segs.size() && j < i + G_MAXSEG; ++j) g.seg[g.nseg++] = segs[j];
    if (a.epi && i == 0) {
      g.wbuf = B_W0, g.mix_d = a.C.ext('x'), g.mix_wr = a.R.ext('f'), g.mix_ld = a.T2.stride('x');
      for (const auto& kd : a.epi_diag) {
        const View src = a.src(kd.first->b);
        EpiTerm& t = g.mix[g.nmix++];
        t.b = kd.first->b, t.f = kd.first->f, t.delta = kd.second;
        t.src = src.buf, t.src_off = src.off;
      }
    }
    st.groups.push_back(g);
    p.steps.push_back(st);
  }
}

inline Plan plan_heff1_fold(int dtype, const mpse_heff& h, const WSiteInfo& wi, bool two_results = false,
                            bool mix_epilogue = false) {
  Plan p;
  const FoldAnalysis a = fold_analyse(dtype, h, wi, two_results, mix_epilogue);
  if ((p.error = a.error)) return p;
  p.tmp_elems[0] = a.ntmp * a.T1.stride('t');
  p.tmp_elems[1] = a.nplanes * a.T2.stride('p');
  fold_emit_l(p, a);
  fold_emit_mix(p, a);
  fold_emit_r(p, a);
  return marked(std::move(p));
}


inline bool push_env_wmix(Plan& p, const WSiteInfo& wi, bool in_left, int w_dtype, const View& src, const View& dst) {
  const int64_t d = wi.d, nout = in_left ? wi.wr : wi.wl;
  if (d > 32 || (d + WM_CHUNK - 1) / WM_CHUNK > WM_MAXCHUNKS) return false;
  std::vector<std::vector<const WBlock*>> by_out(nout);
  int64_t nslot = 0;
  for (const WBlock& k : wi.blocks) {
    by_out[in_left ? k.f : k.b].push_back(&k);
    nslot += k.ident ? 0 : 1;
  }
  for (auto& v : by_out)
    if ((int)v.size() > WM_MAXTERM) return false;
  if (!wmix_fits_lds(nslot, d)) return false;
  Step mix{};
  mix.kind = K_WMIX;
  mix.b = B_W0;
  mix.dta = src.dt, mix.dtb = w_dtype;
  mix.wp_Da = src.ext('a'), mix.wp_d = d, mix.wp_Dk = src.ext('k'), mix.wp_wr = wi.wr;
  Step part = mix;
  for (int64_t o = 0; o < nout; ++o) {
    const View dv = dst.sub('c', o, 1);
    WMixDst q;
    q.dst = dv.buf, q.dst_off = dv.off, q.s_a = dv.stride('a'), q.s_d = dv.stride('x');
    for (const WBlock* k : by_out[o]) q.term[q.nterm++] = wmix_term(wi, *k, src.sub('c', in_left ? k->b : k->f, 1));
    part.mix.push_back(q);
    if ((int)part.mix.size() == WM_MAXDST) {
      p.steps.push_back(part);
      part = mix;
    }
  }
  if (!part.mix.empty()) p.steps.push_back(part);
  return true;
}

inline Step* push_bra_l(Plan& p, int ybuf, int dtype, int bra_conj, int64_t A, int64_t anc, int64_t wr, int64_t Drk, int64_t Drb) {
  const View BRA(B_BRA, dtype, {{'A', A}, {'g', anc}, {'p', Drb}}), Y(ybuf, dtype, {{'A', A}, {'f', wr}, {'g', anc}, {'h', Drk}});
  return contract(p, BRA, Y, View(B_OUT, dtype, {{'p', Drb}, {'f', wr}, {'h', Drk}}), "p", "Ag", "fh", "", "", bra_conj);
}
inline Step* push_bra_r(Plan& p, int ybuf, int dtype, int bra_conj, int64_t K, int64_t wl, int64_t Dlk, int64_t Dlb) {
  const View BRA(B_BRA, dtype, {{'p', Dlb}, {'K', K}}), Y(ybuf, dtype, {{'h', Dlk}, {'q', wl}, {'K', K}});
  return contract(p, BRA, Y, View(B_OUT, dtype, {{'p', Dlb}, {'q', wl}, {'h', Dlk}}), "p", "K", "qh", "", "", bra_conj);
}

inline Plan plan_env(int dtype, int domain, const mpse_dims& s, int env_dtype, int w_dtype, int bra_conj,
                     const WSiteInfo* wi = nullptr) {
  Plan p;
  const bool wfold = wi && dtype == MPSE_C128 && w_dtype == MPSE_F64 && s.d0 >= 8 && (s.danc <= 1) && wi->wl == s.wl &&
                     wi->d == s.d0 && wi->wr == s.wr;
  const int64_t d = s.d0, wl = s.wl, wr = s.wr;
  const int64_t anc = s.danc > 0 ? s.danc : 1;
  const int64_t Dlb = s.Dl_bra, Dlk = s.Dl_ket, Drb = s.Dr_bra, Drk = s.Dr_ket;
  if (domain == MPSE_DOMAIN_L) {
    const int64_t N = d * anc * Drk;
    p.tmp_elems[0] = Dlb * wl * N;
    p.tmp_elems[1] = Dlb * d * wr * anc * Drk;
    push_env_times(p, B_L, env_dtype, B_C, dtype, B_T1, Dlb, wl, Dlk, N, s.env_unit, true);
    if (!(wfold && push_env_wmix(p, *wi, true, w_dtype, View(B_T1, dtype, {{'c', wl}, {'a', Dlb}, {'x', d}, {'k', Drk}}),
                                 View(B_T2, dtype, {{'a', Dlb}, {'x', d}, {'c', wr}, {'k', Drk}}))))
      push_w(p, B_W0, w_dtype, B_T1, B_T2, dtype, Dlb, wl, d, wr, anc * Drk);
    if (Step* st = push_bra_l(p, B_T2, dtype, bra_conj, Dlb * d, anc, wr, Drk, Drb))
      st->skip_zero = skip_pays(Drb, Dlb * d * anc, wr * Drk, 1);
    return marked(std::move(p));
  }
  if (domain == MPSE_DOMAIN_R) {
    p.tmp_elems[0] = Dlk * d * anc * wr * Drb;
    p.tmp_elems[1] = Dlk * wl * d * anc * Drb;
    const int64_t M = Dlk * d * anc;
    const int64_t u = (s.env_unit >= 1 && s.env_unit <= wr && Drb == Drk && unit_pays(M, Drk, Drb)) ? s.env_unit - 1 : -1;
    const View A(B_C, dtype, {{'m', M}, {'c', Drk}}), R(B_L, env_dtype, {{'a', Drb}, {'b', wr}, {'c', Drk}});
    const View X(B_T1, dtype, {{'m', M}, {'b', wr}, {'a', Drb}});
    if (u >= 0) copy(p, A.as("ma"), X.sub('b', u, 1), "m", "a");
    const ChannelRanges cr(u, wr);
    for (int r = 0; r < 2; ++r) {
      const int64_t b0 = cr.lo[r], nb = cr.hi[r] - cr.lo[r];
      if (nb <= 0) continue;
      if (Step* st = contract(p, A, R.sub('b', b0, nb), X.sub('b', b0, nb), "m", "c", "ba"))
        st->skip_zero = skip_pays(M, Drk, nb * Drb);
    }
    if (!(wfold && push_env_wmix(p, *wi, false, w_dtype, View(B_T1, dtype, {{'a', Dlk}, {'x', d}, {'c', wr}, {'k', Drb}}),
                                 View(B_T2, dtype, {{'a', Dlk}, {'c', wl}, {'x', d}, {'k', Drb}}))))
      contract(p, View(B_W0, w_dtype, {{'q', wl}, {'y', d}, {'e', d}, {'b', wr}}),
               View(B_T1, dtype, {{'h', Dlk}, {'e', d}, {'g', anc}, {'b', wr}, {'a', Drb}}),
               View(B_T2, dtype, {{'h', Dlk}, {'q', wl}, {'y', d}, {'g', anc}, {'a', Drb}}), "qy", "eb", "a", "h", "g");
    if (Step* st = push_bra_r(p, B_T2, dtype, bra_conj, d * anc * Drb, wl, Dlk, Dlb))
      st->skip_zero = skip_pays(Dlb, d * anc * Drb, wl * Dlk, 1);
    return marked(std::move(p));
  }
  p.error = "env: bad domain";
  return p;
}


inline Plan plan_env_multi(int dtype, int domain, const mpse_dims& s, int n, const int64_t* wl, const int64_t* wr,
                           int env_dtype, int w_dtype, int bra_conj) {
  Plan p;
  if (n < 1 || n > 4) {
    p.error = "env_multi: 1 to 4 MPO layers";
    return p;
  }
  const int64_t d = s.d0, anc = s.danc > 0 ? s.danc : 1;
  const int64_t Dlb = s.Dl_bra, Dlk = s.Dl_ket, Drb = s.Dr_bra, Drk = s.Dr_ket;
  int64_t WL = 1, WR = 1;
  for (int i = 0; i < n; ++i) WL *= wl[i], WR *= wr[i];
  const bool left = domain == MPSE_DOMAIN_L;
  if (!left && domain != MPSE_DOMAIN_R) {
    p.error = "env: bad domain";
    return p;
  }
  int64_t win[4], wout[4];
  for (int i = 0; i < n; ++i) win[i] = left ? wl[i] : wr[i], wout[i] = left ? wr[i] : wl[i];
  const int64_t Da = left ? Dlb : Drb;
  const int64_t Dh = left ? Drk : Dlk;
  int64_t cur = Da * d * anc * Dh;
  for (int i = 0; i < n; ++i) cur *= win[i];
  int64_t maxsz = cur;
  {
    int64_t t = cur;
    for (int i = n - 1; i >= 0; --i) {
      t = t / win[i] * wout[i];
      if (t > maxsz) maxsz = t;
    }
  }
  p.tmp_elems[0] = p.tmp_elems[1] = maxsz;
  int tb = B_T1;
  if (left) {
    push_env_times(p, B_L, env_dtype, B_C, dtype, tb, Dlb, WL, Dlk, d * anc * Drk, 0, true);
    int64_t P = WL, F = 1;
    for (int i = n - 1; i >= 0; --i) {
      P /= wl[i];
      View W(w_buf(i), w_dtype, {{'b', wl[i]}, {'y', d}, {'x', d}, {'f', wr[i]}});
      View Tin(tb, dtype, {{'P', P}, {'b', wl[i]}, {'a', Dlb}, {'x', d}, {'N', F * anc * Drk}});
      const int to = tb == B_T1 ? B_T2 : B_T1;
      View Tout(to, dtype, {{'P', P}, {'a', Dlb}, {'y', d}, {'f', wr[i]}, {'N', F * anc * Drk}});
      contract(p, W, Tin, Tout, "yf", "bx", "N", "a", "P");
      tb = to;
      F *= wr[i];
    }
    push_bra_l(p, tb, dtype, bra_conj, Dlb * d, anc, WR, Drk, Drb);
    return marked(std::move(p));
  }
  contract(p, View(B_C, dtype, {{'m', Dlk * d * anc}, {'c', Drk}}), View(B_L, env_dtype, {{'a', Drb}, {'b', WR}, {'c', Drk}}),
           View(tb, dtype, {{'m', Dlk * d * anc}, {'b', WR}, {'a', Drb}}), "m", "c", "ba");
  int64_t P = WR, Q = 1;
  for (int i = n - 1; i >= 0; --i) {
    P /= wr[i];
    View W(w_buf(i), w_dtype, {{'q', wl[i]}, {'y', d}, {'x', d}, {'b', wr[i]}});
    View Tin(tb, dtype, {{'h', Dlk}, {'Q', Q}, {'x', d}, {'g', anc}, {'P', P}, {'b', wr[i]}, {'a', Drb}});
    const int to = tb == B_T1 ? B_T2 : B_T1;
    View Tout(to, dtype, {{'h', Dlk}, {'q', wl[i]}, {'Q', Q}, {'y', d}, {'g', anc}, {'P', P}, {'a', Drb}});
    contract(p, W, Tin, Tout, "qy", "xb", "Pa", "h", "Qg");
    tb = to;
    Q *= wl[i];
  }
  push_bra_r(p, tb, dtype, bra_conj, d * anc * Drb, WL, Dlk, Dlb);
  return marked(std::move(p));
}

inline Plan plan_heff2(int dtype, const mpse_heff& h) {
  Plan p;
  const mpse_dims& s = h.dims;
  const int64_t Dl = s.Dl_ket, Dr = s.Dr_ket, wl = s.wl, wr = s.wr, d0 = s.d0;
  if (h.nsite != 1 && h.nsite != 2) {
    p.error = "heff (two layers): one- or two-site centres only";
    return p;
  }
  if ((s.Dl_bra > 0 && s.Dl_bra != Dl) || (s.Dr_bra > 0 && s.Dr_bra != Dr)) {
    p.error = "heff (two layers): bra bonds must equal ket bonds";
    return p;
// ... 123 lines not shown
inline Plan plan_env_ft(int dtype, int domain, const mpse_heff_ft& h, int env_dtype) {
  Plan p;
  if ((p.error = ft_check(h))) return p;
  p.tmp_elems[0] = p.tmp_elems[1] = p.tmp_elems[2] = ft_tmp_elems(h, domain == MPSE_DOMAIN_R);
  const int64_t Dl = h.Dl, Dr = h.Dr, du = h.d_up, dv = h.d_down;
  const int conj = dtype == MPSE_C128 ? 1 : 0;
  if (domain == MPSE_DOMAIN_L) {
    mpse_heff_ft hl = h;
    hl.l_dtype = env_dtype;
    char dud[4] = "d";
    const char* kr;
    View T3 = ft_chain_l(p, dtype, hl, &dud[1], &dud[2], &kr);
    View BRA(B_BRA, dtype, {{'d', Dl}, {dud[1], du}, {dud[2], dv}, {'k', Dr}});
    View O(B_OUT, dtype, {{'j', Dr}, {'g', h.wr1}, {'i', h.wr2}, {'k', Dr}});
    contract(p, BRA, T3, O, "k", dud, kr, "", "", conj);
    return marked(std::move(p));
  }
  if (domain != MPSE_DOMAIN_R) {
    p.error = "env: bad domain";
    return p;
  }
  const bool t1 = h.trans1 != 0, t2 = h.trans2 != 0;
  View X(B_C, dtype, {{'a', Dl}, {'u', du}, {'v', dv}, {'j', Dr}});
  View R(B_L, env_dtype, {{'j', Dr}, {'g', h.wr1}, {'i', h.wr2}, {'k', Dr}});
  View T1(B_T1, dtype, {{'a', Dl}, {'u', du}, {'v', dv}, {'g', h.wr1}, {'i', h.wr2}, {'k', Dr}});
  contract(p, X, R, T1, "auv", "j", "gik");
  View O(B_OUT, dtype, {{'a', Dl}, {'b', h.wl1}, {'c', h.wl2}, {'d', Dl}});
  if (h.leg1 == MPSE_LEG_UP && h.leg2 == MPSE_LEG_UP) {
    View W1 = ft_w_view(B_W0, h.w_dtype, t1, 'b', h.wl1, 'u', 'x', du, 'g', h.wr1);
    View W2 = ft_w_view(B_W1, h.w_dtype, t2, 'c', h.wl2, 'x', 'y', du, 'i', h.wr2);
    View T2(B_T2, dtype, {{'a', Dl}, {'b', h.wl1}, {'x', du}, {'v', dv}, {'i', h.wr2}, {'k', Dr}});
    contract(p, W1, T1, T2, "bx", "ug", "vik", "a");
    View T3(B_T3, dtype, {{'a', Dl}, {'b', h.wl1}, {'c', h.wl2}, {'y', du}, {'v', dv}, {'k', Dr}});
    contract(p, W2, T2, T3, "cy", "xi", "vk", "ab");
    View BRA(B_BRA, dtype, {{'d', Dl}, {'y', du}, {'v', dv}, {'k', Dr}});
    contract(p, BRA, T3, O, "d", "yvk", "abc", "", "", conj);
    return marked(std::move(p));
  }
  if (h.leg1 == MPSE_LEG_DOWN && h.leg2 == MPSE_LEG_DOWN) {
    View W1 = ft_w_view(B_W0, h.w_dtype, t1, 'b', h.wl1, 'v', 's', dv, 'g', h.wr1);
    View W2 = ft_w_view(B_W1, h.w_dtype, t2, 'c', h.wl2, 's', 't', dv, 'i', h.wr2);
    View T2(B_T2, dtype, {{'a', Dl}, {'u', du}, {'b', h.wl1}, {'s', dv}, {'i', h.wr2}, {'k', Dr}});
    contract(p, W1, T1, T2, "bs", "vg", "ik", "au");
    View T3(B_T3, dtype, {{'a', Dl}, {'u', du}, {'b', h.wl1}, {'c', h.wl2}, {'t', dv}, {'k', Dr}});
    contract(p, W2, T2, T3, "ct", "si", "k", "aub");
    View BRA(B_BRA, dtype, {{'d', Dl}, {'u', du}, {'t', dv}, {'k', Dr}});
    contract(p, BRA, T3, O, "d", "utk", "abc", "", "", conj);
    return marked(std::move(p));
  }
  View W1 = ft_w_view(B_W0, h.w_dtype, t1, 'b', h.wl1, 'u', 'x', du, 'g', h.wr1);
  View W2 = ft_w_view(B_W1, h.w_dtype, t2, 'c', h.wl2, 'v', 's', dv, 'i', h.wr2);
  View T2(B_T2, dtype, {{'a', Dl}, {'b', h.wl1}, {'x', du}, {'v', dv}, {'i', h.wr2}, {'k', Dr}});
  contract(p, W1, T1, T2, "bx", "ug", "vik", "a");
  View T3(B_T3, dtype, {{'a', Dl}, {'b', h.wl1}, {'x', du}, {'c', h.wl2}, {'s', dv}, {'k', Dr}});
  contract(p, W2, T2, T3, "cs", "vi", "k", "abx");
  View BRA(B_BRA, dtype, {{'d', Dl}, {'x', du}, {'s', dv}, {'k', Dr}});
  contract(p, BRA, T3, O, "d", "xsk", "abc", "", "", conj);
  return marked(std::move(p));
}


inline int die_group_rule(long long ntile, int tiles_m, int tiles_n, double size_a, double size_b) {
  if (ntile < 64) return 0;
  if (size_a >= size_b && tiles_m % 8 == 0) return 1;
  if (tiles_n % 8 == 0) return 2;
  return tiles_m % 8 == 0 ? 1 : 0;
}
inline bool order_pays(long long ntile, long long nwg, int n_cu, bool always = false) {
  return (always || nwg > 2LL * n_cu) && ntile <= 2048;
}

struct GemmShape {
  long long M, N, K, batch;
  int n_cu;
  bool ca, cb;
  int skip_hint;
  bool k_single;
  bool fast_ok;
  bool dot;
  long long dot_cap;
  bool slices;
  unsigned long long slices_cap;
  bool use_beta;
};
struct GemmPlan {
  int tiles_m, tiles_n, nkt;
  int ksplit, kt_per_split;
  unsigned long long ws_bytes;
  bool leave_slices;
  long long nwg;
  bool fast, wide;
  bool masks;
  int nkw;
  bool order;
  int die_group;
  long long rgx, rgy;
  long long dot_producers;
};
inline GemmPlan launch_plan(const GemmShape& s) {
  GemmPlan p{};
  p.tiles_m = int((s.M + 63) / 64), p.tiles_n = int((s.N + 63) / 64), p.nkt = int((s.K + 15) / 16);
  const long long ntile = (long long)p.tiles_m * p.tiles_n, base = ntile * s.batch;
  p.ksplit = 1;
  p.kt_per_split = p.nkt > 0 ? p.nkt : 1;
  if (base < s.n_cu && p.nkt >= 4) {
    const long long want = (s.n_cu + base - 1) / base, maxs = p.nkt / 2;
    const int S = int(want < maxs ? want : maxs);
    if (S > 1) {
      p.kt_per_split = (p.nkt + S - 1) / S;
      p.ksplit = (p.nkt + p.kt_per_split - 1) / p.kt_per_split;
      p.ws_bytes = (unsigned long long)s.batch * p.ksplit * s.M * s.N * ((s.ca || s.cb) ? 16 : 8);
      p.leave_slices = s.slices && !s.dot && s.batch == 1 && !s.use_beta && p.ws_bytes <= s.slices_cap;
    }
  }
  p.nwg = base * p.ksplit;
  p.rgx = (s.N + 255) / 256 > 64 ? 64 : (s.N + 255) / 256;
  p.rgy = s.M * s.batch > 32768 ? 32768 : s.M * s.batch;
  if (s.dot && s.batch == 1) {
    long long producers = base;
    if (p.ksplit > 1) {
      const long long cap_y = s.dot_cap / p.rgx;
      if (cap_y >= 1 && p.rgy > cap_y) p.rgy = cap_y;
      producers = p.rgx * p.rgy;
    }
    if (producers >= 1 && producers <= s.dot_cap) p.dot_producers = producers;
  }
  p.masks = (s.skip_hint & 3) && s.k_single && p.nkt >= 2 && s.batch <= 16384;
  p.nkw = p.masks ? (p.nkt + 7) / 8 : 0;
  p.order = s.batch == 1 && p.masks && order_pays(ntile, ntile * p.ksplit, s.n_cu);
  if (!p.order && p.ksplit == 1 && s.batch == 1)
    p.die_group = die_group_rule(ntile, p.tiles_m, p.tiles_n, double(s.M) * (s.ca ? 2 : 1), double(s.N) * (s.cb ? 2 : 1));
  p.fast = s.k_single && s.fast_ok;
  p.wide = p.fast && p.nwg <= s.n_cu && p.nkt >= 2;
  return p;
}

#if defined(__HIPCC__)
__host__ __device__
#endif
inline bool out_tile_live(const unsigned char* mask, int pitch, int d, int Dr, int M, int tm, int tn) {
  const int r1 = 64 * tm + 64 < M ? 64 * tm + 64 : M, l0 = 64 * tn, l1 = 64 * tn + 63 < Dr - 1 ? 64 * tn + 63 : Dr - 1;
  for (int r = 64 * tm; r < r1; ++r) {
    const int a = r / d, sg = r - a * d;
    for (int ct = (sg * Dr + l0) >> 6; ct <= (sg * Dr + l1) >> 6; ++ct)
      if (mask[(long long)ct * pitch + (a >> 4)]) return true;
  }
  return false;
}

struct GroupedPlan {
  int tiles_m, tiles_n, nkw, die_group;
  bool order, wide;
  long long nwg;
};
inline GroupedPlan grouped_plan(long long M, long long N, int ngrp, int nkt_max, bool any_mask, bool split2, bool ca,
                                int n_cu, bool out_mask = false) {
  GroupedPlan p{};
  p.tiles_m = int((M + 63) / 64) * ngrp, p.tiles_n = int((N + 63) / 64);
  const long long ntile = (long long)p.tiles_m * p.tiles_n;
  p.nwg = ntile * (split2 ? 2 : 1);
  p.nkw = (any_mask && (nkt_max + 7) / 8 <= 64) ? (nkt_max + 7) / 8 : 0;
  p.order = p.nkw > 0 && order_pays(ntile, ntile, n_cu, split2 || out_mask);
  if (!p.order) p.die_group = die_group_rule(ntile, p.tiles_m, p.tiles_n, double(M) * ngrp * (ca ? 2 : 1), double(N) * 2);
  p.wide = p.nwg <= n_cu;
  return p;
}

}
```

### renormalizer_amd/engine.py

```python
import collections
import ctypes as C
import math
import os
import threading

import numpy as np

_HERE = os.path.dirname(os.path.abspath(__file__))
LIB_PATH = os.environ.get("RENO_MPSENGINE") or os.path.join(_HERE, "csrc", "libmpsengine.so")

F64, C128 = 0, 1
MPSE_OK, MPSE_ERR_OOM, MPSE_ERR_SHAPE, MPSE_ERR_NOCONV, MPSE_ERR_HIP, MPSE_ERR_ARG = 0, 1, 2, 3, 4, 5
DOMAIN_L, DOMAIN_R = 0, 1

STATUS = {0: "OK", 1: "OOM", 2: "SHAPE", 3: "NOCONV", 4: "HIP", 5: "ARG"}


PcgResult = collections.namedtuple("PcgResult", "status iters relres lvalue")


class EngineError(RuntimeError):
    pass


# ... 34 lines not shown

class mpse_heff_ft(C.Structure):
    _fields_ = [("Dl", C.c_int64), ("Dr", C.c_int64), ("d_up", C.c_int64), ("d_down", C.c_int64),
                ("wl1", C.c_int64), ("wr1", C.c_int64), ("wl2", C.c_int64), ("wr2", C.c_int64),
                ("leg1", C.c_int), ("leg2", C.c_int), ("trans1", C.c_int), ("trans2", C.c_int),
                ("L", C.c_void_p), ("l_dtype", C.c_int),
                ("R", C.c_void_p), ("r_dtype", C.c_int),
                ("W1", C.c_void_p), ("W2", C.c_void_p), ("w_dtype", C.c_int)]


def idx1(ext, stride):
    return mpse_index(int(ext), max(int(ext), 1), 0, int(stride))


def idx2(hi, lo, s_hi, s_lo):
    return mpse_index(int(hi) * int(lo), max(int(lo), 1), int(s_hi), int(s_lo))


def dtype_code(dt):
    dt = np.dtype(dt)
    if dt == np.float64:
        return F64
    if dt == np.complex128:
        return C128
    raise TypeError(f"unsupported dtype {dt}; the engine computes in float64 / complex128")


_i64p = C.POINTER(C.c_int64)
_dblp = C.POINTER(C.c_double)

_SIGNATURES = {
    "mpse_ctx_create": [C.c_int, C.POINTER(C.c_void_p)],
    "mpse_ctx_destroy": [C.c_void_p],
    "mpse_sync": [C.c_void_p],
    "mpse_device_info": [C.c_void_p, C.c_char_p, C.c_size_t, C.POINTER(C.c_int), C.POINTER(C.c_void_p)],
    "mpse_prof_enable": [C.c_void_p, C.c_int],
    "mpse_prof_reset": [C.c_void_p],
    "mpse_prof_get": [C.c_void_p, C.c_int, _dblp, _dblp, _dblp, C.POINTER(C.c_int64)],
    "mpse_prof_get_ktiles": [C.c_void_p, C.c_int, C.POINTER(C.c_int64)],
    "mpse_prof_get_svd_sweeps": [C.c_void_p, C.POINTER(C.c_int64)],
    "mpse_mpo_site_hint": [C.c_void_p, C.c_void_p, C.c_void_p, C.c_int64, C.c_int64, C.c_int64],
    "mpse_block_qr_stats": [C.c_void_p] + [C.POINTER(C.c_int64)] * 3,
    "mpse_heff_fused_stats": [C.c_void_p] + [C.POINTER(C.c_int64)] * 2,
    "mpse_block_qr_optimistic": [C.c_void_p, C.c_int],
    "mpse_block_qr_scheme": [C.c_void_p, C.c_int],
    "mpse_block_qr_check": [C.c_void_p, C.POINTER(C.c_int)],
    "mpse_block_qr_pass_stats": [C.c_void_p] + [C.POINTER(C.c_int64)] * 2,
    "mpse_malloc": [C.c_void_p, C.c_size_t, C.POINTER(C.c_void_p)],
    "mpse_free": [C.c_void_p, C.c_void_p],
    "mpse_pool_trim": [C.c_void_p],
    "mpse_mem_info": [C.c_void_p] + [C.POINTER(C.c_size_t)] * 4,
    "mpse_memcpy_h2d": [C.c_void_p, C.c_void_p, C.c_void_p, C.c_size_t],
    "mpse_memcpy_d2h": [C.c_void_p, C.c_void_p, C.c_void_p, C.c_size_t],
    "mpse_memcpy_d2d": [C.c_void_p, C.c_void_p, C.c_void_p, C.c_size_t],
    "mpse_memset_zero": [C.c_void_p, C.c_void_p, C.c_size_t],
    "mpse_memcpy_2d": [C.c_void_p, C.c_void_p, C.c_size_t, C.c_void_p, C.c_size_t, C.c_size_t, C.c_size_t],
    "mpse_cast_f64_to_c128": [C.c_void_p, C.c_void_p, C.c_void_p, C.c_int64],
    "mpse_conj_inplace": [C.c_void_p, C.c_void_p, C.c_int64],
    "mpse_scal": [C.c_void_p, C.c_int, C.c_void_p, C.c_int64, C.c_double, C.c_double],
    "mpse_axpy": [C.c_void_p, C.c_int, C.c_void_p, C.c_void_p, C.c_int64, C.c_double, C.c_double],
    "mpse_mul_real": [C.c_void_p, C.c_int, C.c_void_p, C.c_void_p, C.c_int64],
    "mpse_davidson_precond": [C.c_void_p, C.c_int, C.c_void_p, C.c_void_p, C.c_void_p, C.c_void_p, C.c_int64,
                              C.c_double, C.c_double],
    "mpse_real_part": [C.c_void_p, C.c_void_p, C.c_void_p, C.c_int64],
    "mpse_dotc": [C.c_void_p, C.c_int, C.c_void_p, C.c_void_p, C.c_int64, _dblp],
    "mpse_nrm2": [C.c_void_p, C.c_int, C.c_void_p, C.c_int64, _dblp],
    "mpse_scaled_rms": [C.c_void_p, C.c_int, C.c_void_p, C.c_void_p, C.c_void_p, C.c_int64, C.c_double, C.c_double, _dblp],
    "mpse_expm_centre_mask": [C.c_void_p, C.c_void_p, C.c_int64],
    "mpse_defer_begin": [C.c_void_p, C.c_int],
    "mpse_defer_end": [C.c_void_p],
    "mpse_defer_arm": [C.c_void_p, C.c_int],
    "mpse_defer_run": [C.c_void_p, C.c_int],
    "mpse_defer_discard": [C.c_void_p],
    "mpse_gemm": [C.c_void_p, C.POINTER(mpse_gemm_desc), C.c_void_p, C.c_void_p, C.c_void_p],
    "mpse_gemm_path_stats": [C.c_void_p, _i64p, C.c_int],
    "mpse_transpose_inner": [C.c_void_p, C.c_int, C.c_void_p, C.c_void_p, C.c_int64, C.c_int64, C.c_int64, C.c_int],
    "mpse_env_update": [C.c_void_p, C.c_int, C.c_int, C.POINTER(mpse_dims), C.c_void_p, C.c_int, C.c_void_p,
                        C.c_void_p, C.c_int, C.c_void_p, C.c_int, C.c_void_p],
    "mpse_heff_apply": [C.c_void_p, C.c_int, C.POINTER(mpse_heff), C.c_void_p, C.c_void_p],
    "mpse_heff_apply2": [C.c_void_p, C.c_int, C.POINTER(mpse_heff), C.c_void_p, C.c_void_p],
    "mpse_env_update_multi": [C.c_void_p, C.c_int, C.c_int, C.POINTER(mpse_dims), C.c_int, _i64p, _i64p, C.c_void_p,
                              C.c_int, C.c_void_p, C.c_void_p, C.c_int, C.POINTER(C.c_void_p), C.c_int, C.c_void_p],
    "mpse_env_unit_channel": [C.c_void_p, C.c_int, C.c_void_p, C.c_int64, C.c_int64, C.c_double, _i64p],
    "mpse_expm_lanczos": [C.c_void_p, C.c_int, C.POINTER(mpse_heff), C.c_double, C.c_double, C.c_void_p, C.c_void_p,
                          C.c_double, C.c_double, C.c_int, C.POINTER(C.c_int)],
    "mpse_expm_lanczos_batch": [C.c_void_p, C.c_int, C.c_int, C.POINTER(mpse_heff), C.c_double, C.c_double,
                                C.POINTER(C.c_void_p), C.POINTER(C.c_void_p), C.c_double, C.c_double, C.c_int,
                                C.POINTER(C.c_int)],
    "mpse_expm_lanczos_batch_stats": [C.c_void_p, _i64p, _i64p],
    "mpse_expm_lanczos_path_stats": [C.c_void_p, _i64p, C.c_int],
    "mpse_davidson": [C.c_void_p, C.c_int, C.POINTER(mpse_heff), C.c_int, C.c_void_p, C.c_void_p, C.c_int, C.c_int,
                      C.c_void_p, C.c_double, C.c_int, C.c_int, C.c_double, C.c_double, _dblp, C.c_void_p,
                      C.POINTER(C.c_int), C.POINTER(C.c_int)],
    "mpse_pcg": [C.c_void_p, C.c_int, C.POINTER(mpse_heff), C.c_int, C.c_double, C.c_void_p, C.c_void_p, C.c_void_p,
                 C.c_void_p, C.c_double, C.c_int, C.POINTER(C.c_int), _dblp, _dblp],
    "mpse_pcg_stats": [C.c_void_p, _i64p, C.c_int],
    "mpse_pcg_batch": [C.c_void_p, C.c_int, C.c_int, C.POINTER(mpse_heff), C.c_int, _dblp, C.POINTER(C.c_void_p),
                       C.POINTER(C.c_void_p), C.POINTER(C.c_void_p), C.POINTER(C.c_void_p), C.c_double, C.c_int,
                       C.POINTER(C.c_int), C.POINTER(C.c_int), _dblp, _dblp],
    "mpse_pcg_batch_stats": [C.c_void_p, _i64p, C.c_int],
    "mpse_pcg_batch_plan": [C.c_int, C.c_int64, C.c_int64, C.c_int64, C.c_int64, C.c_int64, _i64p, C.c_int],
    "mpse_heff_apply_ft": [C.c_void_p, C.c_int, C.POINTER(mpse_heff_ft), C.c_void_p, C.c_void_p],
    "mpse_env_update_ft": [C.c_void_p, C.c_int, C.c_int, C.POINTER(mpse_heff_ft), C.c_void_p, C.c_int, C.c_void_p,
                           C.c_void_p],
    "mpse_pcg_sum": [C.c_void_p, C.c_int, C.c_int, C.POINTER(mpse_heff_ft), _dblp, C.c_double, C.c_void_p, C.c_void_p,
                     C.c_void_p, C.c_void_p, C.c_double, C.c_int, C.POINTER(C.c_int), _dblp, _dblp],
    "mpse_pcg_sum_stats": [C.c_void_p, _i64p, C.c_int],
    "mpse_site_factor_ft": [C.c_void_p, C.POINTER(mpse_heff_ft), C.c_void_p],
    "mpse_diag_ft": [C.c_void_p, C.POINTER(mpse_heff_ft), C.c_void_p, C.c_double, C.c_double, C.c_int, C.c_void_p],
    "mpse_mps_overlap": [C.c_void_p, C.c_int, C.POINTER(C.c_void_p), C.POINTER(C.c_int), C.POINTER(C.c_void_p),
                         C.POINTER(C.c_int), _i64p, C.c_int, _dblp],
    "mpse_mps_overlap_stats": [C.c_void_p, _i64p, C.c_int],
    "mpse_mps_overlap_plan": [C.c_int, _i64p, C.c_int, _i64p, C.c_int],
    "mpse_mps_sandwich": [C.c_void_p, C.c_int, C.POINTER(C.c_void_p), C.POINTER(C.c_int), C.POINTER(C.c_void_p),
                          C.POINTER(C.c_int), C.POINTER(C.c_void_p), C.POINTER(C.c_int), _i64p, C.c_int, _dblp],
    "mpse_mps_sandwich_stats": [C.c_void_p, _i64p, C.c_int],
    "mpse_mps_sandwich_plan": [C.c_int, _i64p, C.c_int, _i64p, C.c_int],
    "mpse_mps_corr": [C.c_void_p, C.c_int, C.POINTER(C.c_void_p), C.POINTER(C.c_int), _i64p, C.c_int, C.POINTER(C.c_int),
                      _dblp, _dblp, _dblp, _dblp],
    "mpse_mps_corr_stats": [C.c_void_p, _i64p, C.c_int],
    "mpse_mps_corr_plan": [C.c_int, _i64p, C.c_int, C.c_int, _i64p, C.c_int],
    "mpse_mps_rdm1": [C.c_void_p, C.c_int, C.POINTER(C.c_void_p), C.POINTER(C.c_int), _i64p, C.c_int, C.POINTER(C.c_int),
                      _dblp],
    "mpse_mps_rdm1_stats": [C.c_void_p, _i64p, C.c_int],
    "mpse_mps_rdm1_plan": [C.c_int, _i64p, C.c_int, C.c_int, _i64p, C.c_int],
    "mpse_mps_rdm2": [C.c_void_p, C.c_int, C.POINTER(C.c_void_p), C.POINTER(C.c_int), _i64p, C.c_int, C.POINTER(C.c_int),
                      _dblp],
    "mpse_mps_rdm2_stats": [C.c_void_p, _i64p, C.c_int],
    "mpse_mps_rdm2_plan": [C.c_int, _i64p, C.c_int, C.POINTER(C.c_int), C.c_int, _i64p, C.c_int],
    "mpse_truncate_select": [_dblp, _i64p, C.c_int64, C.c_int64, C.c_double, _i64p, _i64p],
    "mpse_block_qr": [C.c_void_p, C.c_int, C.c_void_p, C.c_int64, C.c_int64, C.c_int, _i64p, _i64p, _i64p, _i64p,
                      C.c_int, C.c_void_p, C.c_void_p, C.c_int64],
    "mpse_block_svd": [C.c_void_p, C.c_int, C.c_void_p, C.c_int64, C.c_int64, C.c_int, _i64p, _i64p, _i64p, _i64p,
                       C.c_void_p, C.c_void_p, _dblp, C.c_int64],
    "mpse_block_svd_full": [C.c_void_p, C.c_int, C.c_void_p, C.c_int64, C.c_int64, C.c_int, _i64p, _i64p, _i64p, _i64p,
                            _i64p, C.c_void_p, C.c_int64, C.c_void_p, C.c_int64, _dblp, C.c_int64],
    "mpse_gather_cols": [C.c_void_p, C.c_int, C.c_void_p, C.c_void_p, C.c_int64, C.c_int64, _i64p, _dblp, C.c_int64],
    "mpse_gather_rows": [C.c_void_p, C.c_int, C.c_void_p, C.c_void_p, C.c_int64, _i64p, _dblp, C.c_int64],
}
EXPORTED_SYMBOLS = sorted(list(_SIGNATURES) + ["mpse_last_error", "mpse_version"])


def load_library(path=LIB_PATH):
    if not os.path.exists(path):
        raise EngineError(
            f"{path} not found: build it with `python -c 'import __graft_entry__ as g; g.build()'` "
            "(hipcc --offload-arch=gfx950).  renormalizer_amd has no CPU fallback.")
    lib = C.CDLL(path)
    for name, args in _SIGNATURES.items():
        fn = getattr(lib, name)
        fn.argtypes = args
        fn.restype = C.c_int
    lib.mpse_last_error.argtypes = [C.c_void_p]
    lib.mpse_last_error.restype = C.c_char_p
    lib.mpse_version.argtypes = []
    lib.mpse_version.restype = C.c_char_p
    return lib


def _chain_plan(lib_fn, dims, row_len, row, info_names, *extra):
    rows = [[int(x) for x in r] for r in dims]
    assert all(len(r) == row_len for r in rows), f"dims rows are ({row})"
    flat = (C.c_int64 * max(row_len * len(rows), 1))(*[x for r in rows for x in r])
    info = (C.c_int64 * len(info_names))()
    ok = lib_fn(len(rows), flat, *extra, info, len(info))
    return bool(ok), dict(zip(info_names, (int(v) for v in info)))
# ... 504 lines not shown
        rows = cls.corr_dims(sites)
        n = len(rows)
        if n == 0:
            raise ValueError(f"{call}: no sites")
        sel = check_selection(call, sel, n)
        return rows, n, sel, (C.c_int64 * (4 * n))(*[int(x) for r in rows for x in r])

    def mps_corr(self, sites, sel, x_mats, y_mats, z_mats):
        rows = self.corr_dims(sites)
        n, nsel = len(rows), len(sel)
        if n == 0 or nsel == 0 or not (len(x_mats) == len(y_mats) == len(z_mats) == nsel):
            raise ValueError(f"mps_corr: {n} sites, {nsel} selected, {len(x_mats)}/{len(y_mats)}/{len(z_mats)} matrices")
        packed = []
        for mats in (x_mats, y_mats, z_mats):
            flat = []
            for k, m in zip(sel, mats):
                m = np.ascontiguousarray(m, dtype=np.complex128)
                d = rows[k][1] if 0 <= int(k) < n else m.shape[0]
                if m.shape != (d, d):
                    raise ValueError(f"mps_corr: a local matrix of site {k} has shape {m.shape}, the site has d = {d}")
                flat.append(m.reshape(-1))
            packed.append(np.ascontiguousarray(np.concatenate(flat)).view(np.float64))
        dims = (C.c_int64 * (4 * n))(*[int(x) for r in rows for x in r])
        out = np.zeros((nsel, nsel), dtype=np.complex128)
        self._check(self.lib.mpse_mps_corr(
            self.ctx, n, *_site_args(sites), dims, nsel, (C.c_int * nsel)(*[int(k) for k in sel]),
            *[p.ctypes.data_as(_dblp) for p in packed], out.ctypes.data_as(_dblp)))
        return out

    RDM1_STATS = ("chain_kernel", "enqueued", "sites", "matrices")

    def mps_rdm1_stats(self):
        return self._stats_dict(self.lib.mpse_mps_rdm1_stats, self.RDM1_STATS)

    def mps_rdm1(self, sites, sel):
        rows, n, sel, dims = self._sel_dims("mps_rdm1", sites, sel)
        sizes = [rows[k][1] ** 2 for k in sel]
        out = np.zeros(sum(sizes), dtype=np.complex128)
        self._check(self.lib.mpse_mps_rdm1(
            self.ctx, n, *_site_args(sites), dims, len(sel), (C.c_int * len(sel))(*sel), out.ctypes.data_as(_dblp)))
        ends = np.cumsum(sizes)
        return [out[e - sz:e].reshape(rows[k][1], rows[k][1]) for k, sz, e in zip(sel, sizes, ends)]

    RDM2_STATS = ("chain_kernel", "enqueued", "sites", "pairs")

    def mps_rdm2_stats(self):
        return self._stats_dict(self.lib.mpse_mps_rdm2_stats, self.RDM2_STATS)

    def mps_rdm2(self, sites, sel):
        rows, n, sel, dims = self._sel_dims("mps_rdm2", sites, sel)
        if len(sel) < 2:
            raise ValueError(f"mps_rdm2: a pair needs two selected sites, the selection is {sel}")
        pairs = [(k, l) for i, k in enumerate(sel) for l in sel[i + 1:]]
        sizes = [rows[k][1] ** 2 * rows[l][1] ** 2 for k, l in pairs]
        out = np.zeros(sum(sizes), dtype=np.complex128)
        self._check(self.lib.mpse_mps_rdm2(
            self.ctx, n, *_site_args(sites), dims, len(sel), (C.c_int * len(sel))(*sel), out.ctypes.data_as(_dblp)))
        ends = np.cumsum(sizes)
        return {(k, l): out[e - sz:e].reshape(rows[k][1], rows[k][1], rows[l][1], rows[l][1])
                for (k, l), sz, e in zip(pairs, sizes, ends)}

    def block_qr_stats(self):
        a, b, c = C.c_int64(), C.c_int64(), C.c_int64()
        self._check(self.lib.mpse_block_qr_stats(self.ctx, C.byref(a), C.byref(b), C.byref(c)))
        return a.value, b.value, c.value

    def heff_fused_stats(self):
        a, b = C.c_int64(), C.c_int64()
        self._check(self.lib.mpse_heff_fused_stats(self.ctx, C.byref(a), C.byref(b)))
        return a.value, b.value

    GEMM_PATHS = ("launches", "general", "eight_wave", "split_b1", "split_batched", "die_group1", "die_group2", "skew",
                  "tile_order", "masks", "masks_global", "grouped", "grouped_split2")

    def gemm_path_stats(self):
        return self._stats_dict(self.lib.mpse_gemm_path_stats, self.GEMM_PATHS)

    def wfold_path_stats(self):
        n = len(self.GEMM_PATHS)
        v = (C.c_int64 * (n + 3))()
        self._check(self.lib.mpse_gemm_path_stats(self.ctx, v, n + 3))
        return {"grouped_mix": int(v[n]), "wmix": int(v[n + 1]), "grouped_outmask": int(v[n + 2])}

    def block_qr_optimistic(self, on):
        self._check(self.lib.mpse_block_qr_optimistic(self.ctx, int(bool(on))))

    def block_qr_scheme(self, scheme):
        self._check(self.lib.mpse_block_qr_scheme(self.ctx, int(scheme)))

    def block_qr_check(self):
        v = C.c_int(0)
        self._check(self.lib.mpse_block_qr_check(self.ctx, C.byref(v)))
        return bool(v.value)

    def block_qr_pass_stats(self):
        a, b = C.c_int64(0), C.c_int64(0)
        self._check(self.lib.mpse_block_qr_pass_stats(self.ctx, C.byref(a), C.byref(b)))
        return a.value, b.value

    def prof_get(self):
        names = {0: "f64xf64", 1: "c128xf64", 2: "f64xc128", 3: "c128xc128", 4: "lanczos_vec", 5: "block_qr", 6: "block_svd",
                 7: "heff_fused"}
        issued_per_mac = {0: 2.0, 1: 4.0, 2: 4.0, 3: 6.0}
        out = {}
        for v, nm in names.items():
            ms, fl, by, n = C.c_double(), C.c_double(), C.c_double(), C.c_int64()
            self._check(self.lib.mpse_prof_get(self.ctx, v, C.byref(ms), C.byref(fl), C.byref(by), C.byref(n)))
            out[nm] = dict(ms=ms.value, flops=fl.value, bytes=by.value, launches=n.value)
            if v < 4:
                kt = C.c_int64()
                self._check(self.lib.mpse_prof_get_ktiles(self.ctx, v, C.byref(kt)))
                out[nm]["ktiles"] = kt.value
                out[nm]["issued_flops"] = kt.value * 65536.0 * issued_per_mac[v]
        sw = C.c_int64()
        self._check(self.lib.mpse_prof_get_svd_sweeps(self.ctx, C.byref(sw)))
        out["block_svd"]["sweeps"] = sw.value
        return out

    def empty(self, shape, dtype=np.float64):
        if isinstance(shape, (int, np.integer)):
            shape = (shape,)
        dtype = np.dtype(dtype)
        dtype_code(dtype)
        n = math.prod(int(x) for x in shape)
        buf = _Buffer(self, n * dtype.itemsize)
        return DeviceTensor(self, buf, 0, shape, dtype)

    def zeros(self, shape, dtype=np.float64):
        t = self.empty(shape, dtype)
        self._check(self.lib.mpse_memset_zero(self.ctx, t.ptr, t.nbytes))
        return t

    def asdevice(self, a, dtype=None):
        if isinstance(a, DeviceTensor):
            if dtype is not None and np.dtype(dtype) != a.dtype:
                if np.dtype(dtype) == np.complex128:
                    return a.to_complex()
                raise TypeError("cannot cast complex device tensor to real")
            return a
        a = np.asarray(a)
        if dtype is None:
            dtype = np.complex128 if np.iscomplexobj(a) else np.float64
        a = np.ascontiguousarray(a, dtype=dtype)
        t = self.empty(a.shape, a.dtype)
        if a.size:
            self._check(self.lib.mpse_memcpy_h2d(self.ctx, t.ptr, a.ctypes.data, a.nbytes))
        return t

    def copy_block(self, dst, dst_row0, dst_col0, src):
        assert dst.dtype == src.dtype and dst.ndim == 2 and src.ndim == 2
        es = dst.dtype.itemsize
        rows, cols = src.shape
        assert dst_row0 + rows <= dst.shape[0] and dst_col0 + cols <= dst.shape[1]
        self._check(self.lib.mpse_memcpy_2d(self.ctx, dst.ptr + (dst_row0 * dst.shape[1] + dst_col0) * es,
                                            dst.shape[1] * es, src.ptr, cols * es, cols * es, rows))

    def copy_sub(self, dst, dst_row0, dst_col0, src, src_row0, src_col0, rows, cols):
        assert dst.dtype == src.dtype and dst.ndim == 2 and src.ndim == 2
        assert dst_row0 + rows <= dst.shape[0] and dst_col0 + cols <= dst.shape[1]
        assert src_row0 + rows <= src.shape[0] and src_col0 + cols <= src.shape[1]
        if rows == 0 or cols == 0:
            return
        es = dst.dtype.itemsize
        self._check(self.lib.mpse_memcpy_2d(self.ctx, dst.ptr + (dst_row0 * dst.shape[1] + dst_col0) * es,
                                            dst.shape[1] * es, src.ptr + (src_row0 * src.shape[1] + src_col0) * es,
                                            src.shape[1] * es, cols * es, rows))
# ... 50 lines not shown
```

### renormalizer_amd/mps/lib.py

```python
import ctypes as C
import os

import numpy as np

from ..engine import DOMAIN_L, DOMAIN_R, DeviceTensor, get_engine, mpse_dims


def _as_w(eng, mo):
    if isinstance(mo, DeviceTensor):
        return mo
    return eng.asdevice(np.asarray(mo))


_UNIT_PREDICTIONS = {}


def predict_unit_channel(mo_host, domain, unit_in):
    if unit_in <= 0 or mo_host is None:
        return 0
    key = (id(mo_host), domain, int(unit_in))
    hit = _UNIT_PREDICTIONS.get(key)
    if hit is not None and hit[0] is mo_host:
        return hit[1]
    w = np.asarray(mo_host)
    u = int(unit_in) - 1
    eye = np.eye(w.shape[1])
    out = 0
    if domain == "L" and u < w.shape[0]:
        for g in range(w.shape[3]):
            if np.array_equal(w[u, :, :, g], eye) and not np.any(np.delete(w[:, :, :, g], u, axis=0)):
                out = g + 1
                break
    elif domain == "R" and u < w.shape[3]:
        for q in range(w.shape[0]):
            if np.array_equal(w[q, :, :, u], eye) and not np.any(np.delete(w[q], u, axis=2)):
                out = q + 1
                break
    if len(_UNIT_PREDICTIONS) > 4096:
        _UNIT_PREDICTIONS.clear()
    _UNIT_PREDICTIONS[key] = (mo_host, out)
    return out


def contract_one_site(environ, ms, mo, domain, ms_conj=None, canonical_mo_host=None):
    assert domain in ["L", "R"]
    eng = ms.eng
    mo = _as_w(eng, mo)
    bra = ms if ms_conj is None else ms_conj
    if ms.ndim not in (3, 4):
        raise ValueError(f"MPS ndim is not 3 or 4, got {ms.ndim}")
    cplx = ms.is_complex or environ.is_complex or bra.is_complex or mo.is_complex
    dt = np.complex128 if cplx else np.float64
    ket = ms.to_complex() if cplx else ms
    bra = bra.to_complex() if cplx else bra
    d = mpse_dims()
    d.Dl_ket, d.Dr_ket = ket.shape[0], ket.shape[-1]
    d.Dl_bra, d.Dr_bra = bra.shape[0], bra.shape[-1]
    d.d0, d.d1 = ket.shape[1], 1
    d.danc = ket.shape[2] if ket.ndim == 4 else 1
    d.wl, d.wr, d.wm = mo.shape[0], mo.shape[3], 1
    d.env_unit = environ.unit
    if domain == "L":
        assert environ.shape == (d.Dl_bra, d.wl, d.Dl_ket), (environ.shape, bra.shape, mo.shape, ket.shape)
        oshape = (d.Dr_bra, d.wr, d.Dr_ket)
    else:
        assert environ.shape == (d.Dr_bra, d.wr, d.Dr_ket), (environ.shape, bra.shape, mo.shape, ket.shape)
        oshape = (d.Dl_bra, d.wl, d.Dl_ket)
    out = eng.empty(oshape, dt)
    eng._check(eng.lib.mpse_env_update(
        eng.ctx, out.code, DOMAIN_L if domain == "L" else DOMAIN_R, C.byref(d), environ.ptr, environ.code,
        ket.ptr, bra.ptr, 1 if ms_conj is None else 0, mo.ptr, mo.code, out.ptr))
    if ms_conj is None and oshape[0] == oshape[2]:
        deferred = eng.recording_list >= 0
        if canonical_mo_host is not None and ms.ndim == 3 and environ.unit > 0:
            out.unit = predict_unit_channel(canonical_mo_host, domain, environ.unit)
            if VERIFY_UNIT and oshape[0] >= UNIT_MIN_BOND and not deferred:
                measured = find_unit_channel(out)
                if measured != out.unit and eng.block_qr_check():
                    raise ArithmeticError("unit channel of an environment behind a block QR that broke down")
                assert measured == out.unit, f"unit channel predicted {out.unit}, measured {measured}"
        elif oshape[0] >= UNIT_MIN_BOND and not deferred:
            out.unit = find_unit_channel(out)
    return out


def contract_one_site_multi_mpo(environ, ms, mos, domain, ms_conj=None):
    assert domain in ["L", "R"]
    eng = ms.eng
    mos = [_as_w(eng, mo) for mo in mos]
    n = len(mos)
    bra = ms if ms_conj is None else ms_conj
    if ms.ndim not in (3, 4):
        raise ValueError(f"MPS ndim is not 3 or 4, got {ms.ndim}")
    if environ.ndim != n + 2:
        raise ValueError(f"environment with {environ.ndim - 2} MPO legs for {n} MPO sites")
    wcplx = any(mo.is_complex for mo in mos)
    cplx = ms.is_complex or environ.is_complex or bra.is_complex or wcplx
    dt = np.complex128 if cplx else np.float64
    ket = ms.to_complex() if cplx else ms
    bra = bra.to_complex() if cplx else bra
    if wcplx:
        mos = [mo.to_complex() for mo in mos]
    d = mpse_dims()
    d.Dl_ket, d.Dr_ket = ket.shape[0], ket.shape[-1]
    d.Dl_bra, d.Dr_bra = bra.shape[0], bra.shape[-1]
    d.d0, d.d1 = ket.shape[1], 1
    d.danc = ket.shape[2] if ket.ndim == 4 else 1
    wl = (C.c_int64 * n)(*[mo.shape[0] for mo in mos])
    wr = (C.c_int64 * n)(*[mo.shape[3] for mo in mos])
    ptrs = (C.c_void_p * n)(*[mo.ptr for mo in mos])
    if domain == "L":
        assert environ.shape == (d.Dl_bra,) + tuple(wl) + (d.Dl_ket,), (environ.shape, tuple(wl))
        oshape = (d.Dr_bra,) + tuple(wr) + (d.Dr_ket,)
    else:
        assert environ.shape == (d.Dr_bra,) + tuple(wr) + (d.Dr_ket,), (environ.shape, tuple(wr))
        oshape = (d.Dl_bra,) + tuple(wl) + (d.Dl_ket,)
    out = eng.empty(oshape, dt)
    eng._check(eng.lib.mpse_env_update_multi(
        eng.ctx, out.code, DOMAIN_L if domain == "L" else DOMAIN_R, C.byref(d), n, wl, wr, environ.ptr, environ.code,
        ket.ptr, bra.ptr, 1 if ms_conj is None else 0, ptrs, mos[0].code, out.ptr))
    return out


UNIT_TOL = 1e-12
UNIT_MIN_BOND = 128
VERIFY_UNIT = False


def find_unit_channel(env):
    eng = env.eng
    unit = C.c_int64(0)
    eng._check(eng.lib.mpse_env_unit_channel(eng.ctx, env.code, env.ptr, env.shape[0], env.shape[1], UNIT_TOL,
                                             C.byref(unit)))
    return int(unit.value)


class Environ:

    def __init__(self, mps, mpo, domain=None, mps_conj=None):
        self.eng = get_engine()
        self._virtual_disk = {}
        self.multi = isinstance(mpo, (list, tuple))
        if self.multi:
            self.sentinel = self.eng.ones((1,) * (len(mpo) + 2), np.float64)
        else:
            self.sentinel = self.eng.ones((1, 1, 1), np.float64)
            self.sentinel.unit = 1
        self._construct(mps, mpo, domain, mps_conj)

    def _mo(self, mpo, idx):
        if isinstance(mpo, (list, tuple)):
            return [self._mo(m, idx) for m in mpo]
        return mpo.device(idx, self.eng) if hasattr(mpo, "device") else _as_w(self.eng, mpo[idx])

    def _step(self, tensor, ms, mo, domain, ms_conj):
        if isinstance(mo, list):
            return contract_one_site_multi_mpo(tensor, ms, mo, domain, ms_conj=ms_conj)
        return contract_one_site(tensor, ms, mo, domain, ms_conj=ms_conj)

    def _construct(self, mps, mpo, domain=None, mps_conj=None):
        assert domain in ["L", "R", None]
        if domain is None:
            self._construct(mps, mpo, "L", mps_conj)
            self._construct(mps, mpo, "R", mps_conj)
            return
        n = len(mps)
        rng = range(0, n - 1) if domain == "L" else range(n - 1, 0, -1)
        self.write("L", -1, self.sentinel)
        self.write("R", n, self.sentinel)
        tensor = self.sentinel
        for idx in rng:
            cj = None if mps_conj is None else mps_conj[idx]
            tensor = self._step(tensor, mps[idx], self._mo(mpo, idx), domain, cj)
            self.write(domain, idx, tensor)

    def GetLR(self, domain, siteidx, mps, mpo, itensor=None, method="Scratch", mps_conj=None, canonical=False):
        assert domain in ["L", "R"]
        assert method in ["Enviro", "System", "Scratch"]
        if mps_conj is None:
            mps_conj = [None] * len(mps)
        if siteidx not in range(len(mps)):
            return self.sentinel
        if method == "Scratch":
            itensor = self.sentinel
            sites = range(siteidx + 1) if domain == "L" else range(len(mps) - 1, siteidx - 1, -1)
            for i in sites:
                itensor = self._step(itensor, mps[i], self._mo(mpo, i), domain, mps_conj[i])
        elif method == "Enviro":
            itensor = self.read(domain, siteidx)
        else:
            if itensor is None:
                itensor = self.read(domain, siteidx + (-1 if domain == "L" else 1))
            mo = self._mo(mpo, siteidx)
            if canonical and not isinstance(mo, list) and mps_conj[siteidx] is None and hasattr(mpo, "device"):
                itensor = contract_one_site(itensor, mps[siteidx], mo, domain, canonical_mo_host=mpo[siteidx])
            else:
                itensor = self._step(itensor, mps[siteidx], mo, domain, mps_conj[siteidx])
            self.write(domain, siteidx, itensor)
        return itensor

    def write(self, domain, siteidx, tensor):
        self._virtual_disk[(domain, siteidx)] = tensor

    def drop(self, domain):
        for key in [k for k, v in self._virtual_disk.items() if k[0] == domain and v is not self.sentinel]:
            del self._virtual_disk[key]

    def read(self, domain, siteidx):
        return self._virtual_disk[(domain, siteidx)]
```

### renormalizer_amd/mps/mps.py

```python
import ctypes
import logging
import os
import threading
from typing import Dict, List

import numpy as np

from ..engine import DeviceTensor, EngineError, get_engine
from ..lib.krylov import expm_krylov
from ..model import Model, Op, OpSum
from ..utils import CompressConfig, CompressCriteria, EvolveConfig, EvolveMethod, OptimizeConfig
from . import svd_qn
from .hop_expr import centre_tile_mask, hop_expr
from . import lib as _lib
from .lib import Environ, contract_one_site
from .mpo import Mpo
from .svd_qn import add_outer, get_qn_mask

logger = logging.getLogger("renormalizer_amd")


def _vn_entropy(p):
    p = np.asarray(p, dtype=float)
    assert np.allclose(p[p < 0], 0)
# ... 1293 lines not shown
        return new

    def _evolve_tdvp_ps_sweeps(self, mpo, evolve_dt, learn_qr=False) -> "Mps":
        cfg = self.evolve_config
        eng = get_engine()
        sw = _PsSweep(self, mpo, evolve_dt, learn_qr)
        mps, evolve_dt, local_steps = sw.mps, sw.evolve_dt, sw.local_steps
        prepare, split_site, absorb, note_qr = sw.prepare, sw.split_site, sw.absorb, sw.note_qr

        same_dtype = mps.is_complex or (evolve_dt.real == 0 and not mpo.is_complex)
        pipelined = (cfg.ivp_solver == "krylov" and same_dtype and os.environ.get("MPSE_DEFER", "1") != "0"
                     and not _lib.VERIFY_UNIT)
        try:
            for _ in range(2):
                order = list(mps.iter_idx_list(full=True))
                centre = mps[order[0]]
                ready = prepare(order[0], list(centre.shape))
                after_site = None
                if pipelined and ready[1]:
                    out = eng.empty(centre.shape, centre.dtype)
                    with eng.recording(0):
                        after_site = (out,) + split_site(order[0], out, ready, list(centre.shape))
                for imps in order:
                    shape = list(centre.shape)
                    hop, split = ready[0], ready[1]
                    if not split:
                        mps_t, j = _local_propagate(cfg, hop, -1j * evolve_dt / 2, centre)
                        local_steps.append(j)
                        mps[imps] = mps_t.reshape(shape)
                        continue
                    if not pipelined:
                        mps_t, j = _local_propagate(cfg, hop, -1j * evolve_dt / 2, centre)
                        local_steps.append(j)
                        hop_b, bond, nbr = split_site(imps, mps_t, ready, shape)
                        note_qr(imps)
                        ready = prepare(nbr, list(mps[nbr].shape[:-1]) + [bond.shape[1]] if not mps.to_right
                                        else [bond.shape[0]] + list(mps[nbr].shape[1:]))
                        b_t, j = _local_propagate(cfg, hop_b, 1j * evolve_dt / 2, bond)
                        local_steps.append(j)
                        centre = mps[nbr] = absorb(b_t.reshape(bond.shape), nbr)
                        continue
                    out, hop_b, bond, nbr = after_site
                    eng.arm(0)
                    _, j = expm_krylov(hop, -1j * evolve_dt / 2, centre, out=out)
                    local_steps.append(j)
                    note_qr(imps)
                    b_out = eng.empty(bond.shape, bond.dtype)
                    with eng.recording(1):
                        new_centre = absorb(b_out, nbr)
                    mps[nbr] = new_centre
                    ready = prepare(nbr, list(new_centre.shape))
                    after_site = None
                    if ready[1]:
                        out = eng.empty(new_centre.shape, new_centre.dtype)
                        with eng.recording(0):
                            after_site = (out,) + split_site(nbr, out, ready, list(new_centre.shape))
                    eng.arm(1)
                    _, j = expm_krylov(hop_b, 1j * evolve_dt / 2, bond, out=b_out)
                    local_steps.append(j)
                    centre = new_centre
                mps._switch_direction()
        except BaseException:
            eng.defer_discard()
            raise
        return sw.finish()


class _PsSweep:

    def __init__(self, src, mpo, evolve_dt, learn_qr=False, carry=None):
        eng = get_engine()
        self.eng, self.mpo, self.learn_qr = eng, mpo, learn_qr
        self.carry = _CARRY if carry is None else carry
        if np.iscomplex(evolve_dt):
            mps = src.copy()
        else:
            mps = src.to_complex()
        self.evolve_dt = complex(evolve_dt)
        self.mps = mps
        self.n = len(mps)
        ahead = "R" if mps.to_right else "L"
        environ = _carried_environ(mps, mpo, ahead, self.carry)
        if environ is None:
            environ = Environ(mps, mpo, ahead)
        self.environ = environ
        self.local_steps = []
        self.q = len(mps.qntot)
        self.hh_sites = _householder_sites(mps)
        self.hh_sites.tick()
        self.qr_redone = eng.block_qr_stats()[2]
        self.use_cmask = os.environ.get("MPSE_CENTRE_MASK", "1") != "0"

    def note_qr(self, imps):
        if self.learn_qr:
            now = self.eng.block_qr_stats()[2]
            if now != self.qr_redone:
                self.hh_sites.note((imps, self.mps.to_right))
            self.qr_redone = now

    def prepare(self, imps, shape):
        mps, eng, n = self.mps, self.eng, self.n
        hop = hop_expr(self.environ.read("L", imps - 1), self.environ.read("R", imps + 1), [self.mpo.device(imps, eng)],
                       shape)
        split = (not mps.to_right and imps != 0) or (mps.to_right and imps != n - 1)
        qnbigl = qnbigr = plan = None
        if split:
            qnbigl, qnbigr, _ = mps._get_big_qn([imps], need_mat=False)
            plan = svd_qn.block_plan(qnbigl, qnbigr, mps.qntot)
            if self.use_cmask and len(shape) == 3 and shape[0] * shape[0] * shape[1] * shape[2] >= (1 << 22):
                if mps.to_right:
                    ql, qr = qnbigl, qnbigr
                else:
                    ql = add_outer(np.array(mps.qn[imps]), mps._get_sigmaqn(imps))
                    qr = np.array(mps.qn[imps + 1])
                hop.cmask = centre_tile_mask(eng, ql, qr, mps.qntot, shape)
        return hop, split, qnbigl, qnbigr, plan

    def split_site(self, imps, centre, ready, shape):
        mps, eng, mpo, environ, q = self.mps, self.eng, self.mpo, self.environ, self.q
        hop, _, qnbigl, qnbigr, plan = ready
        l_array, r_array = hop.l, hop.r
        u, qnlset, v, qnrset = svd_qn.svd_qn(centre, qnbigl, qnbigr, mps.qntot, QR=True,
                                             system="L" if mps.to_right else "R", full_matrices=False, plan=plan,
                                             householder=(imps, mps.to_right) in self.hh_sites)
        vt = v.T
        if not mps.to_right:
            mps[imps] = vt.reshape([-1] + shape[1:])
            mps.qn[imps] = np.array(qnrset, dtype=int).reshape(-1, q)
            mps.qnidx = imps - 1
            r_array = environ.GetLR("R", imps, mps, mpo, itensor=r_array, method="System", canonical=True)
            hop_b = hop_expr(l_array, r_array, [], u.shape)
            if self.use_cmask and u.shape[0] * u.shape[1] >= (1 << 14):
                hop_b.cmask = centre_tile_mask(eng, qnbigl, np.array(qnrset, dtype=int).reshape(-1, q), mps.qntot,
                                               u.shape)
            return hop_b, u, imps - 1
        mps[imps] = u.reshape(shape[:-1] + [-1])
        mps.qn[imps + 1] = np.array(qnlset, dtype=int).reshape(-1, q)
        mps.qnidx = imps + 1
        l_array = environ.GetLR("L", imps, mps, mpo, itensor=l_array, method="System", canonical=True)
        hop_b = hop_expr(l_array, r_array, [], vt.shape)
        if self.use_cmask and vt.shape[0] * vt.shape[1] >= (1 << 14):
            hop_b.cmask = centre_tile_mask(eng, np.array(qnlset, dtype=int).reshape(-1, q), qnbigr, mps.qntot,
                                           vt.shape)
        return hop_b, vt, imps + 1

    def absorb(self, bond, nbr):
        mps, eng = self.mps, self.eng
        t = mps[nbr]
        if mps.to_right:
            return eng.matmul(bond, t.reshape(t.shape[0], -1)).reshape((bond.shape[0],) + t.shape[1:])
        return eng.matmul(t.reshape(-1, t.shape[-1]), bond).reshape(t.shape[:-1] + (bond.shape[1],))

    def finish(self):
        mps, local_steps = self.mps, self.local_steps
        mps.evolve_config.stat = dict(nobs=len(local_steps), min=int(np.min(local_steps)),
                                      max=int(np.max(local_steps)), mean=float(np.mean(local_steps)),
                                      steps=list(local_steps))
        _carry_environ(mps, self.mpo, self.environ, self.carry)
        return mps


_OPTIMISTIC_REDONE = [0]



class _QrNotes:
    FIRST = 8
# ... 351 lines not shown
```

Before: 610.6.

## Skip symmetry-forbidden output tiles in environment updates using quantum-number tile masks

Computes a per-64x64-tile pattern of the environment update result from bond and MPO channel quantum numbers. The final GEMM launches only the tiles that are allowed, and a separate fill kernel writes zeros (or identity for the unit channel) into the rest. This removes arithmetic on blocks that symmetry forces to vanish. In exchange it adds host-side mask construction and caching, a device mask upload and an extra fill launch, plus an optional verification mode.

```diff
diff --git a/include/mpsengine.h b/include/mpsengine.h
--- a/include/mpsengine.h
+++ b/include/mpsengine.h
@@ -112,6 +112,8 @@
                     const void* env, int env_dtype, const void* ket, const void* bra, int bra_conj,
                     const void* W, int w_dtype, void* out);
 
+int mpse_env_result_mask(mpse_ctx* ctx, const void* mask, int64_t nbytes, int64_t out_unit);
+
 int mpse_env_update_multi(mpse_ctx* ctx, int dtype, int domain, const mpse_dims* dims, int n_mpo,
                           const int64_t* wl, const int64_t* wr, const void* env, int env_dtype,
                           const void* ket, const void* bra, int bra_conj, const void* const* W, int w_dtype, void* out);
diff --git a/renormalizer_amd/csrc/mpse_contract.hip b/renormalizer_amd/csrc/mpse_contract.hip
--- a/renormalizer_amd/csrc/mpse_contract.hip
+++ b/renormalizer_amd/csrc/mpse_contract.hip
@@ -23,6 +23,32 @@
   for (long long t = (long long)blockIdx.x * blockDim.x + threadIdx.x; t < total; t += stride) {
     const long long i = t / nn, j = t - i * nn;
     dst[off2(mo, i) + off2(no, j)] = src[off2(mi, i) + off2(ni, j)];
+  }
+}
+
+template <bool CPLX>
+__global__ __launch_bounds__(256) void k_env_mask_check(const double* out, int M, int N, int tiles_n,
+                                                        const unsigned char* mask, int col0, double tol, int* bad) {
+  constexpr int E = CPLX ? 2 : 1;
+  const int st = mask[blockIdx.x];
+  if (st == 1) return;
+  const int tm = blockIdx.x / tiles_n, tn = blockIdx.x - tm * tiles_n;
+  const int j = tn * 64 + (threadIdx.x & 63);
+  if (j >= N) return;
+  bool wrong = false;
+  for (int r = threadIdx.x >> 6; r < 64; r += 4) {
+    const int i = tm * 64 + r;
+    if (i >= M) break;
+    const double* q = out + ((long long)i * N + j) * E;
+    const double re = q[0], im = CPLX ? q[1] : 0.0;
+    if (st == 0 && !(col0 >= 0 && j >= col0 && j < col0 + M))
+      wrong |= !(re == 0.0 && im == 0.0);
+    else
+      wrong |= !(fabs(re - (j - col0 == i ? 1.0 : 0.0)) <= tol && fabs(im) <= tol);
+  }
+  if (wrong) {
+    atomicOr(bad, st == 0 ? 1 : 2);
+    atomicMax(bad + 1, (int)blockIdx.x + 1);
   }
 }
 
@@ -246,6 +272,7 @@
   MatvecReq* mv;
   const int* skip;
   MatvecReq::Dot* dot;
+  const mpse_ctx::EnvMask* em = nullptr;
   TmpBuf slices;
   int slices_used = 0;
   PlanRun(mpse_ctx* c, int dt, const void* const* b, SolveScope* s, MatvecReq* m)
@@ -410,6 +437,11 @@
     rq.cin_m = s.mcin;
     rq.cin_n = s.ncin;
   }
+  if (s.env_result && r.em) {
+    rq.tmask = r.em->tiles.data();
+    rq.tmask_bytes = (long long)r.em->tiles.size();
+    rq.tm_col0 = r.em->out_unit >= 1 ? (r.em->out_unit - 1) * s.mc.ext : 0;
+  }
   if (s.slices_to >= 0) {
     const size_t blk = size_t(s.mc.ext) * size_t(s.nc.ext) * dtype_size(dtc);
     if (r.slices.alloc(4 * blk) == MPSE_OK) {
@@ -426,11 +458,12 @@
 }
 
 static int run_plan(mpse_ctx* ctx, int dtype, const Plan& p, const void* bufs_in[B_COUNT],
-                    SolveScope* sc = nullptr, MatvecReq* mv = nullptr) {
+                    SolveScope* sc = nullptr, MatvecReq* mv = nullptr, const mpse_ctx::EnvMask* em = nullptr) {
   if (p.error) return mpse_fail(ctx, MPSE_ERR_SHAPE, "%s", p.error);
   TmpBuf t1(ctx), t2(ctx), t3(ctx);
   TmpBuf* tmp[3] = {&t1, &t2, &t3};
   PlanRun r(ctx, dtype, bufs_in, sc, mv);
+  r.em = em;
   for (int i = 0; i < 3; ++i)
     if (p.tmp_elems[i]) {
       MPSE_TRY(tmp[i]->alloc(size_t(p.tmp_elems[i]) * r.es));
@@ -496,13 +529,92 @@
   return MPSE_OK;
 }
 
+extern "C" int mpse_env_result_mask(mpse_ctx* ctx, const void* mask, int64_t nbytes, int64_t out_unit) {
+  if (!ctx) return MPSE_ERR_ARG;
+  ctx->env_mask_pending = mpse_ctx::EnvMask();
+  if (!mask) return MPSE_OK;
+  if (nbytes <= 0 || out_unit < 0) return mpse_fail(ctx, MPSE_ERR_ARG, "env_result_mask: empty pattern or negative channel");
+  const unsigned char* m = static_cast<const unsigned char*>(mask);
+  ctx->env_mask_pending.tiles.assign(m, m + nbytes);
+  ctx->env_mask_pending.out_unit = out_unit;
+  ctx->env_mask_pending.set = true;
+  return MPSE_OK;
+}
+
+namespace {
+
+int env_mask_mode() {
+  const char* e = getenv("MPSE_ENV_MASK");
+  return !e ? 1 : e[0] == '0' ? 0 : e[0] == '2' ? 2 : 1;
+}
+
+int env_mask_check_shape(mpse_ctx* ctx, const mpse_ctx::EnvMask& em, int64_t Dp, int64_t w, int64_t Dh, bool* no_plane) {
+  const int64_t tiles_m = (Dp + 63) / 64, tiles_n = (w * Dh + 63) / 64, g = em.out_unit - 1;
+  *no_plane = false;
+  if ((int64_t)em.tiles.size() != tiles_m * tiles_n)
+    return mpse_fail(ctx, MPSE_ERR_SHAPE, "env_update: result pattern of %lld tiles for a result of %lld x %lld",
+                     (long long)em.tiles.size(), (long long)tiles_m, (long long)tiles_n);
+  if (em.out_unit > w || (em.out_unit >= 1 && Dp != Dh))
+    return mpse_fail(ctx, MPSE_ERR_SHAPE, "env_update: unit channel %lld of the result pattern does not fit (w %lld, bonds "
+                     "%lld / %lld)", (long long)em.out_unit, (long long)w, (long long)Dp, (long long)Dh);
+  const bool whole = em.out_unit >= 1 && Dh % 64 == 0;
+  const int64_t t0 = whole ? g * (Dh / 64) : 0, t1 = whole ? t0 + Dh / 64 : 0;
+  bool ones = false;
+  for (int64_t tm = 0; tm < tiles_m; ++tm)
+    for (int64_t tn = 0; tn < tiles_n; ++tn) {
+      const int st = em.tiles[tm * tiles_n + tn];
+      const bool in_unit = tn >= t0 && tn < t1;
+      if (st > 2 || (st == 2 && !(in_unit && tn - t0 == tm)))
+        return mpse_fail(ctx, MPSE_ERR_ARG, "env_update: result pattern: state %d at tile (%lld, %lld)", st, (long long)tm,
+                         (long long)tn);
+      ones |= in_unit && st == 1;
+    }
+  *no_plane = whole && !ones;
+  return MPSE_OK;
+}
+
+int env_mask_verify(mpse_ctx* ctx, int dtype, const mpse_ctx::EnvMask& em, const void* out, int64_t Dp, int64_t w, int64_t Dh) {
+  const int tiles_n = int((w * Dh + 63) / 64), ntile = (int)em.tiles.size();
+  const size_t mbytes = (size_t(ntile) + 7) & ~size_t(7);
+  TmpBuf buf(ctx);
+  MPSE_TRY(buf.alloc(mbytes + 8));
+  std::vector<unsigned char> host(mbytes + 8, 0);
+  memcpy(host.data(), em.tiles.data(), size_t(ntile));
+  MPSE_TRY(stage_h2d(ctx, buf.p, host.data(), host.size()));
+  const unsigned char* md = buf.as<unsigned char>();
+  int* bad = reinterpret_cast<int*>(buf.as<unsigned char>() + mbytes);
+  const int col0 = em.out_unit >= 1 ? int((em.out_unit - 1) * Dh) : -1;
+  if (dtype == MPSE_C128)
+    hipLaunchKernelGGL((k_env_mask_check<true>), dim3((unsigned)ntile), dim3(256), 0, ctx->stream, (const double*)out,
+                       (int)Dp, (int)(w * Dh), tiles_n, md, col0, 1e-12, bad);
+  else
+    hipLaunchKernelGGL((k_env_mask_check<false>), dim3((unsigned)ntile), dim3(256), 0, ctx->stream, (const double*)out,
+                       (int)Dp, (int)(w * Dh), tiles_n, md, col0, 1e-12, bad);
+  MPSE_HIP(ctx, hipGetLastError());
+  int flag[2] = {0, 0};
+  MPSE_HIP(ctx, hipMemcpyAsync(flag, bad, sizeof(flag), hipMemcpyDeviceToHost, ctx->stream));
+  MPSE_HIP(ctx, hipStreamSynchronize(ctx->stream));
+  if (flag[0])
+    return mpse_fail(ctx, MPSE_ERR_ARG, "env_update: MPSE_ENV_MASK=2: the update computed without the result pattern "
+                     "(%lld x %lld x %lld, unit channel %lld) %s%s%s, last in tile (%d, %d)", (long long)Dp, (long long)w,
+                     (long long)Dh, (long long)em.out_unit, (flag[0] & 1) ? "holds data in a tile of state 0" : "",
+                     flag[0] == 3 ? " and " : "", (flag[0] & 2) ? "differs from the identity in a tile of state 2" : "",
+                     (flag[1] - 1) / tiles_n, (flag[1] - 1) % tiles_n);
+  return MPSE_OK;
+}
+
+}
+
 extern "C" int mpse_env_update(mpse_ctx* ctx, int dtype, int domain, const mpse_dims* dims, const void* env,
                                int env_dtype, const void* ket, const void* bra, int bra_conj, const void* W,
                                int w_dtype, void* out) {
   if (!ctx || !dims || !env || !ket || !W || !out) return MPSE_ERR_ARG;
+  mpse_ctx::EnvMask em = std::move(ctx->env_mask_pending);
+  ctx->env_mask_pending = mpse_ctx::EnvMask();
   if (MPSE_RECORDING(ctx)) {
     const mpse_dims dc = *dims;
     ctx->defer_ops[ctx->defer_recording].push_back([=] {
+      ctx->env_mask_pending = em;
       return mpse_env_update(ctx, dtype, domain, &dc, env, env_dtype, ket, bra, bra_conj, W, w_dtype, out);
     });
     return MPSE_OK;
@@ -525,10 +637,22 @@
     auto it = ctx->wsite_info.find(W);
     if (fold_on && it != ctx->wsite_info.end()) wi_keep = it->second.info;
   }
-  Plan p = plan_env(dtype, domain, *dims, env_dtype, w_dtype, bra_conj, static_cast<const WSiteInfo*>(wi_keep.get()));
+  const WSiteInfo* wi = static_cast<const WSiteInfo*>(wi_keep.get());
   const void* bufs[B_COUNT] = {nullptr};
   bind_env(bufs, env, ket, bra, out, 1, &W);
-  return run_plan(ctx, dtype, p, bufs);
+  const int mode = env_mask_mode();
+  if (!em.set || mode == 0 || (domain != MPSE_DOMAIN_L && domain != MPSE_DOMAIN_R))
+    return run_plan(ctx, dtype, plan_env(dtype, domain, *dims, env_dtype, w_dtype, bra_conj, wi), bufs);
+  const bool left = domain == MPSE_DOMAIN_L;
+  const int64_t Dp = left ? dims->Dr_bra : dims->Dl_bra, Dh = left ? dims->Dr_ket : dims->Dl_ket, w = left ? dims->wr : dims->wl;
+  bool no_plane = false;
+  MPSE_TRY(env_mask_check_shape(ctx, em, Dp, w, Dh, &no_plane));
+  if (mode == 2) {
+    MPSE_TRY(run_plan(ctx, dtype, plan_env(dtype, domain, *dims, env_dtype, w_dtype, bra_conj, wi), bufs));
+    MPSE_TRY(env_mask_verify(ctx, dtype, em, out, Dp, w, Dh));
+  }
+  Plan p = plan_env(dtype, domain, *dims, env_dtype, w_dtype, bra_conj, wi, true, no_plane ? em.out_unit : 0);
+  return run_plan(ctx, dtype, p, bufs, nullptr, nullptr, &em);
 }
 
 extern "C" int mpse_env_update_multi(mpse_ctx* ctx, int dtype, int domain, const mpse_dims* dims, int n_mpo,
diff --git a/renormalizer_amd/csrc/mpse_gemm.hip b/renormalizer_amd/csrc/mpse_gemm.hip
--- a/renormalizer_amd/csrc/mpse_gemm.hip
+++ b/renormalizer_amd/csrc/mpse_gemm.hip
@@ -83,6 +83,8 @@
   const double* Cin;
   IdxMap mCin, nCin;
   unsigned long long* trace;
+  const unsigned char* tmask;
+  int tm_col0, nlive;
   GemmGroups gg;
 };
 
@@ -149,7 +151,7 @@
   const int wm = WS == 2 ? wave >> 1 : 0, wn = WS == 2 ? wave & 1 : 0;
   constexpr int WROWS = 16 * WI;
 
-  const int ntile = g.tiles_m * g.tiles_n;
+  const int ntile = (!GRP && g.nlive > 0) ? g.nlive : g.tiles_m * g.tiles_n;
   const int bid = blockIdx.x;
   int bs = bid / ntile;
   int t = bid - bs * ntile;
@@ -1013,6 +1015,18 @@
     const double* wrow = g.ws + ((long long)b * g.ksplit * mn + (long long)i * g.N) * EC;
     double* crow = g.C + ((long long)b * g.sbC + idx_off(g.mC, i)) * EC;
     for (int j = blockIdx.x * 256 + threadIdx.x; j < g.N; j += gridDim.x * 256) {
+      if (g.tmask) {
+        const int st = g.tmask[(i >> 6) * g.tiles_n + (j >> 6)];
+        if (st != 1) {
+          const double v = (st == 2 && j - g.tm_col0 == i) ? 1.0 : 0.0;
+          double* q = crow + idx_off(g.nC, j) * EC;
+          if constexpr (CC)
+            *reinterpret_cast<double2*>(q) = make_double2(v, 0.0);
+          else
+            *q = v;
+          continue;
+        }
+      }
       const double* w = wrow + (long long)j * EC;
       double xr = 0, xi = 0;
       int s = 0;
@@ -1078,6 +1092,31 @@
   }
 }
 
+template <bool CC>
+__global__ __launch_bounds__(256) void k_tile_fill(const GemmArgs g) {
+  constexpr int EC = CC ? 2 : 1;
+  if (g.skip && *g.skip) return;
+  const int ntile = g.tiles_m * g.tiles_n;
+  for (int t = blockIdx.x; t < ntile; t += gridDim.x) {
+    const int st = g.tmask[t];
+    if (st == 1) continue;
+    const int tm = t / g.tiles_n, tn = t - tm * g.tiles_n;
+    const int j = tn * 64 + (threadIdx.x & 63);
+    if (j >= g.N) continue;
+    const long long co = idx_off(g.nC, j);
+    for (int r = threadIdx.x >> 6; r < 64; r += 4) {
+      const int i = tm * 64 + r;
+      if (i >= g.M) break;
+      const double v = (st == 2 && j - g.tm_col0 == i) ? 1.0 : 0.0;
+      double* q = g.C + (idx_off(g.mC, i) + co) * EC;
+      if constexpr (CC)
+        *reinterpret_cast<double2*>(q) = make_double2(v, 0.0);
+      else
+        *q = v;
+    }
+  }
+}
+
 struct OccOperand {
   const double* base;
   IdxMap rmap, kmap;
@@ -1281,6 +1320,39 @@
   return MPSE_OK;
 }
 
+int tile_mask_source(mpse_ctx* ctx, const unsigned char* tiles, int ntile, int tiles_n, int nlive, TmpBuf& tmp,
+                     const int** list, const unsigned char** mask) {
+  const size_t list_bytes = (size_t(nlive) * sizeof(int) + 7) & ~size_t(7), bytes = list_bytes + ((size_t(ntile) + 7) & ~size_t(7));
+  auto bind = [&](void* dev) {
+    *list = static_cast<const int*>(dev);
+    *mask = static_cast<const unsigned char*>(dev) + list_bytes;
+  };
+  for (const auto& e : ctx->tile_masks)
+    if (e.tiles_n == tiles_n && e.tiles.size() == size_t(ntile) && memcmp(e.tiles.data(), tiles, size_t(ntile)) == 0) {
+      bind(e.dev);
+      return MPSE_OK;
+    }
+  std::vector<unsigned char> host(bytes, 0);
+  int* l = reinterpret_cast<int*>(host.data());
+  for (int t = 0, n = 0; t < ntile; ++t)
+    if (tiles[t] == 1) l[n++] = t;
+  memcpy(host.data() + list_bytes, tiles, size_t(ntile));
+  void* dev = nullptr;
+  if (ctx->tile_masks.size() < mpse_ctx::TILE_MASK_CAP) {
+    MPSE_TRY(mpse_malloc(ctx, bytes, &dev));
+    mpse_ctx::TileMaskDev e;
+    e.tiles.assign(tiles, tiles + ntile);
+    e.tiles_n = tiles_n, e.nlive = nlive, e.dev = dev;
+    ctx->tile_masks.push_back(std::move(e));
+  } else {
+    MPSE_TRY(tmp.alloc(bytes));
+    dev = tmp.p;
+  }
+  MPSE_TRY(stage_h2d(ctx, dev, host.data(), bytes));
+  bind(dev);
+  return MPSE_OK;
+}
+
 void launch_gemm(mpse_ctx* ctx, const GemmArgs& g, long long nwg, bool ca, bool cb, bool fast, bool wide, bool grouped,
                  dim3 rgrid = dim3(0), int batch = 1) {
   using Kern = void (*)(const GemmArgs);
@@ -1295,8 +1367,12 @@
       {k_gemm<false, true, true, 2, 1, true>, k_gemm<false, true, true, 2, 2, true>}};
   const int form = fast && wide ? 0 : fast ? 1 : 2;
   const Kern k = grouped ? groups[ca ? 0 : 1][form] : plain[(ca ? 0 : 2) + (cb ? 0 : 1)][form];
-  hipLaunchKernelGGL(k, dim3((unsigned)nwg), dim3(form == 0 ? 512 : 256), 0, ctx->stream, g);
-  if (rgrid.x) hipLaunchKernelGGL(reduce[(ca || cb) ? 0 : 1], rgrid, dim3(256), 0, ctx->stream, g, batch);
+  static void (*const fill[2])(const GemmArgs) = {k_tile_fill<true>, k_tile_fill<false>};
+  if (nwg > 0) hipLaunchKernelGGL(k, dim3((unsigned)nwg), dim3(form == 0 ? 512 : 256), 0, ctx->stream, g);
+  if (rgrid.x)
+    hipLaunchKernelGGL(reduce[(ca || cb) ? 0 : 1], rgrid, dim3(256), 0, ctx->stream, g, batch);
+  else if (g.tmask && !grouped)
+    hipLaunchKernelGGL(fill[(ca || cb) ? 0 : 1], dim3((unsigned)(g.tiles_m * g.tiles_n)), dim3(256), 0, ctx->stream, g);
 }
 
 void count_paths(long long* gp, const mpse_plan::GemmPlan& p, bool batched) {
@@ -1373,9 +1449,25 @@
   MatvecReq::Dot* dot = rq ? rq->dot : nullptr;
   const bool compact = is_single(g.mC) && is_single(g.nC) && g.mC.s_lo == g.N && (g.nC.s_lo == 1 || g.N == 1);
   const bool slices = rq && rq->slices && compact && d->alpha_re == 1.0 && d->alpha_im == 0.0;
+  const unsigned char* tmask = rq ? rq->tmask : nullptr;
+  long long nlive = -1;
+  if (tmask) {
+    const long long ntile = ((long long)(g.M + BM - 1) / BM) * ((g.N + BN - 1) / BN);
+    if (d->batch != 1 || g.use_beta || d->alpha_re != 1.0 || d->alpha_im != 0.0 || dot || slices || rq->tmask_bytes != ntile ||
+        ntile > 0x7fffffffLL)
+      return mpse_fail(ctx, MPSE_ERR_ARG, "mpse_gemm: a result pattern needs a plain product (batch 1, beta 0, alpha 1) "
+                       "and one byte per 64 x 64 tile (%lld given, %lld tiles)", rq->tmask_bytes, ntile);
+    nlive = 0;
+    for (long long t = 0; t < ntile; ++t) {
+      if (tmask[t] > 2) return mpse_fail(ctx, MPSE_ERR_ARG, "mpse_gemm: result pattern holds a state above 2");
+      nlive += tmask[t] == 1;
+    }
+    ++ctx->gemm_paths[mpse_ctx::GP_ENV_MASK];
+    if (nlive == ntile) tmask = nullptr;
+  }
   const mpse_plan::GemmPlan p = mpse_plan::launch_plan(
       {g.M, g.N, g.K, d->batch, n_cu_of(ctx), ca, cb, skip_zero, is_single(g.kA) && is_single(g.kB), fast_ok(g, ca, cb),
-       dot != nullptr, dot ? dot->cap : 0, slices, slices ? rq->slices_cap : 0, g.use_beta != 0});
+       dot != nullptr, dot ? dot->cap : 0, slices, slices ? rq->slices_cap : 0, g.use_beta != 0, tmask ? nlive : -1});
   if (p.nwg > 0x7fffffffLL) return mpse_fail(ctx, MPSE_ERR_SHAPE, "mpse_gemm: grid too large");
   g.ksplit = p.ksplit;
   g.kt_per_split = p.kt_per_split;
@@ -1437,6 +1529,15 @@
       hipLaunchKernelGGL(k_tile_order, dim3(1), dim3(1024), 0, ctx->stream, g.amask, g.bmask, g.nkw, p.nkt, g.tiles_m,
                          g.tiles_n, 1, pp, g.skip, GemmGroups(), (unsigned char*)nullptr, 0, 0, 0);
     g.perm = pp;
+  }
+
+  TmpBuf TMSK(ctx);
+  if (tmask) {
+    const int* list = nullptr;
+    MPSE_TRY(tile_mask_source(ctx, tmask, g.tiles_m * g.tiles_n, g.tiles_n, (int)nlive, TMSK, &list, &g.tmask));
+    g.perm = list;
+    g.nlive = (int)nlive;
+    g.tm_col0 = (int)rq->tm_col0;
   }
 
   count_paths(ctx->gemm_paths, p, d->batch > 1);
diff --git a/renormalizer_amd/csrc/mpse_internal.h b/renormalizer_amd/csrc/mpse_internal.h
--- a/renormalizer_amd/csrc/mpse_internal.h
+++ b/renormalizer_amd/csrc/mpse_internal.h
@@ -86,12 +86,24 @@
     const void* ptr = nullptr;
     long long bytes = 0;
   } cmask_pending;
+  struct EnvMask {
+    std::vector<unsigned char> tiles;
+    long long out_unit = 0;
+    bool set = false;
+  } env_mask_pending;
+  struct TileMaskDev {
+    std::vector<unsigned char> tiles;
+    int tiles_n = 0, nlive = 0;
+    void* dev = nullptr;
+  };
+  static constexpr size_t TILE_MASK_CAP = 1024;
+  std::vector<TileMaskDev> tile_masks;
   unsigned long long* gemm_trace = nullptr;
   bool gemm_trace_checked = false;
   long long f0_launches[2] = {0, 0};
   enum GemmPath {
     GP_LAUNCH, GP_GENERAL, GP_WIDE, GP_SPLIT_B1, GP_SPLIT_BN, GP_DIE1, GP_DIE2, GP_SKEW, GP_ORDER, GP_MASK,
-    GP_MASK_GLOBAL, GP_GROUPED, GP_GROUPED_SPLIT2, GP_GROUPED_MIX, GP_WMIX, GP_GROUPED_OUTMASK, GP_COUNT
+    GP_MASK_GLOBAL, GP_GROUPED, GP_GROUPED_SPLIT2, GP_GROUPED_MIX, GP_WMIX, GP_GROUPED_OUTMASK, GP_ENV_MASK, GP_COUNT
   };
   long long gemm_paths[GP_COUNT] = {0};
   long long qr_chol_calls = 0, qr_chol_fallbacks = 0, qr_calls = 0;
@@ -312,6 +324,9 @@
   void* slices = nullptr;
   size_t slices_cap = 0;
   int slices_used = 0;
+  const unsigned char* tmask = nullptr;
+  long long tmask_bytes = 0;
+  long long tm_col0 = 0;
 };
 
 int heff_apply(mpse_ctx* ctx, int dtype, const mpse_heff* h, const void* C, void* out, SolveScope* sc,
diff --git a/renormalizer_amd/csrc/mpse_plans.h b/renormalizer_amd/csrc/mpse_plans.h
--- a/renormalizer_amd/csrc/mpse_plans.h
+++ b/renormalizer_amd/csrc/mpse_plans.h
@@ -120,6 +120,7 @@
   int64_t slice_b_lo = 0, slice_b_hi = 0;
   int64_t slice_elems = 0;
   bool completes = false;
+  bool env_result = false;
 };
 
 struct Plan {
@@ -709,7 +710,8 @@
 }
 
 
-inline bool push_env_wmix(Plan& p, const WSiteInfo& wi, bool in_left, int w_dtype, const View& src, const View& dst) {
+inline bool push_env_wmix(Plan& p, const WSiteInfo& wi, bool in_left, int w_dtype, const View& src, const View& dst,
+                          int64_t skip_out = -1) {
   const int64_t d = wi.d, nout = in_left ? wi.wr : wi.wl;
   if (d > 32 || (d + WM_CHUNK - 1) / WM_CHUNK > WM_MAXCHUNKS) return false;
   std::vector<std::vector<const WBlock*>> by_out(nout);
@@ -728,6 +730,7 @@
   mix.wp_Da = src.ext('a'), mix.wp_d = d, mix.wp_Dk = src.ext('k'), mix.wp_wr = wi.wr;
   Step part = mix;
   for (int64_t o = 0; o < nout; ++o) {
+    if (o == skip_out) continue;
     const View dv = dst.sub('c', o, 1);
     WMixDst q;
     q.dst = dv.buf, q.dst_off = dv.off, q.s_a = dv.stride('a'), q.s_d = dv.stride('x');
@@ -752,8 +755,9 @@
 }
 
 inline Plan plan_env(int dtype, int domain, const mpse_dims& s, int env_dtype, int w_dtype, int bra_conj,
-                     const WSiteInfo* wi = nullptr) {
+                     const WSiteInfo* wi = nullptr, bool result_mask = false, int64_t out_unit = 0) {
   Plan p;
+  const int64_t no_plane = result_mask && out_unit >= 1 ? out_unit - 1 : -1;
   const bool wfold = wi && dtype == MPSE_C128 && w_dtype == MPSE_F64 && s.d0 >= 8 && (s.danc <= 1) && wi->wl == s.wl &&
                      wi->d == s.d0 && wi->wr == s.wr;
   const int64_t d = s.d0, wl = s.wl, wr = s.wr;
@@ -765,10 +769,12 @@
     p.tmp_elems[1] = Dlb * d * wr * anc * Drk;
     push_env_times(p, B_L, env_dtype, B_C, dtype, B_T1, Dlb, wl, Dlk, N, s.env_unit, true);
     if (!(wfold && push_env_wmix(p, *wi, true, w_dtype, View(B_T1, dtype, {{'c', wl}, {'a', Dlb}, {'x', d}, {'k', Drk}}),
-                                 View(B_T2, dtype, {{'a', Dlb}, {'x', d}, {'c', wr}, {'k', Drk}}))))
+                                 View(B_T2, dtype, {{'a', Dlb}, {'x', d}, {'c', wr}, {'k', Drk}}), no_plane)))
       push_w(p, B_W0, w_dtype, B_T1, B_T2, dtype, Dlb, wl, d, wr, anc * Drk);
-    if (Step* st = push_bra_l(p, B_T2, dtype, bra_conj, Dlb * d, anc, wr, Drk, Drb))
+    if (Step* st = push_bra_l(p, B_T2, dtype, bra_conj, Dlb * d, anc, wr, Drk, Drb)) {
       st->skip_zero = skip_pays(Drb, Dlb * d * anc, wr * Drk, 1);
+      st->env_result = result_mask;
+    }
     return marked(std::move(p));
   }
   if (domain == MPSE_DOMAIN_R) {
@@ -787,12 +793,14 @@
         st->skip_zero = skip_pays(M, Drk, nb * Drb);
     }
     if (!(wfold && push_env_wmix(p, *wi, false, w_dtype, View(B_T1, dtype, {{'a', Dlk}, {'x', d}, {'c', wr}, {'k', Drb}}),
-                                 View(B_T2, dtype, {{'a', Dlk}, {'c', wl}, {'x', d}, {'k', Drb}}))))
+                                 View(B_T2, dtype, {{'a', Dlk}, {'c', wl}, {'x', d}, {'k', Drb}}), no_plane)))
       contract(p, View(B_W0, w_dtype, {{'q', wl}, {'y', d}, {'e', d}, {'b', wr}}),
                View(B_T1, dtype, {{'h', Dlk}, {'e', d}, {'g', anc}, {'b', wr}, {'a', Drb}}),
                View(B_T2, dtype, {{'h', Dlk}, {'q', wl}, {'y', d}, {'g', anc}, {'a', Drb}}), "qy", "eb", "a", "h", "g");
-    if (Step* st = push_bra_r(p, B_T2, dtype, bra_conj, d * anc * Drb, wl, Dlk, Dlb))
+    if (Step* st = push_bra_r(p, B_T2, dtype, bra_conj, d * anc * Drb, wl, Dlk, Dlb)) {
       st->skip_zero = skip_pays(Dlb, d * anc * Drb, wl * Dlk, 1);
+      st->env_result = result_mask;
+    }
     return marked(std::move(p));
   }
   p.error = "env: bad domain";
@@ -1082,6 +1090,7 @@
   bool slices;
   unsigned long long slices_cap;
   bool use_beta;
+  long long live_tiles = -1;
 };
 struct GemmPlan {
   int tiles_m, tiles_n, nkt;
@@ -1096,11 +1105,14 @@
   int die_group;
   long long rgx, rgy;
   long long dot_producers;
+  bool listed;
 };
 inline GemmPlan launch_plan(const GemmShape& s) {
   GemmPlan p{};
   p.tiles_m = int((s.M + 63) / 64), p.tiles_n = int((s.N + 63) / 64), p.nkt = int((s.K + 15) / 16);
-  const long long ntile = (long long)p.tiles_m * p.tiles_n, base = ntile * s.batch;
+  const long long ntile = (long long)p.tiles_m * p.tiles_n;
+  p.listed = s.batch == 1 && s.live_tiles >= 0 && s.live_tiles < ntile;
+  const long long grid_tiles = p.listed ? s.live_tiles : ntile, base = (grid_tiles > 0 ? grid_tiles : 1) * s.batch;
   p.ksplit = 1;
   p.kt_per_split = p.nkt > 0 ? p.nkt : 1;
   if (base < s.n_cu && p.nkt >= 4) {
@@ -1113,7 +1125,7 @@
       p.leave_slices = s.slices && !s.dot && s.batch == 1 && !s.use_beta && p.ws_bytes <= s.slices_cap;
     }
   }
-  p.nwg = base * p.ksplit;
+  p.nwg = grid_tiles * s.batch * p.ksplit;
   p.rgx = (s.N + 255) / 256 > 64 ? 64 : (s.N + 255) / 256;
   p.rgy = s.M * s.batch > 32768 ? 32768 : s.M * s.batch;
   if (s.dot && s.batch == 1) {
@@ -1127,8 +1139,8 @@
   }
   p.masks = (s.skip_hint & 3) && s.k_single && p.nkt >= 2 && s.batch <= 16384;
   p.nkw = p.masks ? (p.nkt + 7) / 8 : 0;
-  p.order = s.batch == 1 && p.masks && order_pays(ntile, ntile * p.ksplit, s.n_cu);
-  if (!p.order && p.ksplit == 1 && s.batch == 1)
+  p.order = s.batch == 1 && p.masks && !p.listed && order_pays(ntile, ntile * p.ksplit, s.n_cu);
+  if (!p.order && !p.listed && p.ksplit == 1 && s.batch == 1)
     p.die_group = die_group_rule(ntile, p.tiles_m, p.tiles_n, double(s.M) * (s.ca ? 2 : 1), double(s.N) * (s.cb ? 2 : 1));
   p.fast = s.k_single && s.fast_ok;
   p.wide = p.fast && p.nwg <= s.n_cu && p.nkt >= 2;
diff --git a/renormalizer_amd/engine.py b/renormalizer_amd/engine.py
--- a/renormalizer_amd/engine.py
+++ b/renormalizer_amd/engine.py
@@ -140,6 +140,7 @@
     "mpse_env_update_multi": [C.c_void_p, C.c_int, C.c_int, C.POINTER(mpse_dims), C.c_int, _i64p, _i64p, C.c_void_p,
                               C.c_int, C.c_void_p, C.c_void_p, C.c_int, C.POINTER(C.c_void_p), C.c_int, C.c_void_p],
     "mpse_env_unit_channel": [C.c_void_p, C.c_int, C.c_void_p, C.c_int64, C.c_int64, C.c_double, _i64p],
+    "mpse_env_result_mask": [C.c_void_p, C.c_void_p, C.c_int64, C.c_int64],
     "mpse_expm_lanczos": [C.c_void_p, C.c_int, C.POINTER(mpse_heff), C.c_double, C.c_double, C.c_void_p, C.c_void_p,
                           C.c_double, C.c_double, C.c_int, C.POINTER(C.c_int)],
     "mpse_expm_lanczos_batch": [C.c_void_p, C.c_int, C.c_int, C.POINTER(mpse_heff), C.c_double, C.c_double,
@@ -810,6 +811,12 @@
         self._check(self.lib.mpse_gemm_path_stats(self.ctx, v, n + 3))
         return {"grouped_mix": int(v[n]), "wmix": int(v[n + 1]), "grouped_outmask": int(v[n + 2])}
 
+    def env_mask_stats(self):
+        n = len(self.GEMM_PATHS) + 4
+        v = (C.c_int64 * n)()
+        self._check(self.lib.mpse_gemm_path_stats(self.ctx, v, n))
+        return int(v[n - 1])
+
     def block_qr_optimistic(self, on):
         self._check(self.lib.mpse_block_qr_optimistic(self.ctx, int(bool(on))))
 
diff --git a/renormalizer_amd/mps/lib.py b/renormalizer_amd/mps/lib.py
--- a/renormalizer_amd/mps/lib.py
+++ b/renormalizer_amd/mps/lib.py
@@ -42,7 +42,45 @@
     return out
 
 
-def contract_one_site(environ, ms, mo, domain, ms_conj=None, canonical_mo_host=None):
+_EMASK_CACHE = {}
+ENV_MASK_MIN_TILES = 16
+
+
+def env_tile_mask(qn_bond, chan_qn, oshape, unit=0):
+    Dp, w, Dh = (int(x) for x in oshape)
+    qb = np.asarray(qn_bond)
+    qc = np.asarray(chan_qn)
+    if qb.ndim != 2 or qc.ndim != 2 or Dp != Dh or qb.shape[0] != Dp or qc.shape[0] != w or qb.shape[1] != qc.shape[1]:
+        return None
+    unit = int(unit)
+    if unit < 0 or unit > w or (unit and np.any(qc[unit - 1])):
+        return None
+    qb = np.ascontiguousarray(qb, dtype=np.int64)
+    qc = np.ascontiguousarray(qc, dtype=np.int64)
+    key = (Dp, w, unit, qb.tobytes(), qc.tobytes())
+    hit = _EMASK_CACHE.get(key)
+    if hit is not None:
+        return hit
+    ub, ib = np.unique(qb, axis=0, return_inverse=True)
+    ib = np.asarray(ib).reshape(-1)
+    ok = (ub[:, None, None, :] - ub[None, None, :, :] == qc[None, :, None, :]).all(-1)
+    allowed = ok[ib][:, :, ib].reshape(Dp, w * Dh)
+    tm, tn = (Dp + 63) // 64, (w * Dh + 63) // 64
+    pad = np.zeros((tm * 64, tn * 64), dtype=bool)
+    pad[:Dp, :w * Dh] = allowed
+    mask = pad.reshape(tm, 64, tn, 64).any(axis=(1, 3)).astype(np.uint8)
+    if unit and Dh % 64 == 0:
+        t0 = (unit - 1) * (Dh // 64)
+        mask[:, t0:t0 + Dh // 64] = 2 * np.eye(tm, dtype=np.uint8)
+    mask = np.ascontiguousarray(mask.reshape(-1))
+    mask.setflags(write=False)
+    if len(_EMASK_CACHE) > 4096:
+        _EMASK_CACHE.clear()
+    _EMASK_CACHE[key] = mask
+    return mask
+
+
+def contract_one_site(environ, ms, mo, domain, ms_conj=None, canonical_mo_host=None, result_qn=None):
     assert domain in ["L", "R"]
     eng = ms.eng
     mo = _as_w(eng, mo)
@@ -67,13 +105,22 @@
         assert environ.shape == (d.Dr_bra, d.wr, d.Dr_ket), (environ.shape, bra.shape, mo.shape, ket.shape)
         oshape = (d.Dl_bra, d.wl, d.Dl_ket)
     out = eng.empty(oshape, dt)
+    predicted = None
+    if ms_conj is None and oshape[0] == oshape[2] and canonical_mo_host is not None and ms.ndim == 3 and environ.unit > 0:
+        predicted = predict_unit_channel(canonical_mo_host, domain, environ.unit)
+    if (result_qn is not None and ms_conj is None and ms.ndim == 3 and oshape[0] == oshape[2]
+            and os.environ.get("MPSE_ENV_MASK", "1") != "0"
+            and ((oshape[0] + 63) // 64) * ((oshape[1] * oshape[2] + 63) // 64) >= ENV_MASK_MIN_TILES):
+        mask = env_tile_mask(result_qn[0], result_qn[1], oshape, 0)
+        if mask is not None:
+            eng._check(eng.lib.mpse_env_result_mask(eng.ctx, mask.ctypes.data, mask.size, 0))
     eng._check(eng.lib.mpse_env_update(
         eng.ctx, out.code, DOMAIN_L if domain == "L" else DOMAIN_R, C.byref(d), environ.ptr, environ.code,
         ket.ptr, bra.ptr, 1 if ms_conj is None else 0, mo.ptr, mo.code, out.ptr))
     if ms_conj is None and oshape[0] == oshape[2]:
         deferred = eng.recording_list >= 0
-        if canonical_mo_host is not None and ms.ndim == 3 and environ.unit > 0:
-            out.unit = predict_unit_channel(canonical_mo_host, domain, environ.unit)
+        if predicted is not None:
+            out.unit = predicted
             if VERIFY_UNIT and oshape[0] >= UNIT_MIN_BOND and not deferred:
                 measured = find_unit_channel(out)
                 if measured != out.unit and eng.block_qr_check():
@@ -135,10 +182,25 @@
     return int(unit.value)
 
 
+def _result_qn(mps, mpo, domain, siteidx):
+    qn, mqn, mtot = getattr(mps, "qn", None), getattr(mpo, "qn", None), getattr(mpo, "qntot", None)
+    qnidx = getattr(mps, "qnidx", None)
+    if qn is None or mqn is None or mtot is None or qnidx is None:
+        return None
+    if domain == "L":
+        if not qnidx > siteidx:
+            return None
+        return np.asarray(qn[siteidx + 1]), np.asarray(mqn[siteidx + 1])
+    if not qnidx < siteidx:
+        return None
+    return np.asarray(qn[siteidx]), np.asarray(mtot).reshape(1, -1) - np.asarray(mqn[siteidx])
+
+
 class Environ:
 
-    def __init__(self, mps, mpo, domain=None, mps_conj=None):
+    def __init__(self, mps, mpo, domain=None, mps_conj=None, qn_pattern=False):
         self.eng = get_engine()
+        self.qn_pattern = bool(qn_pattern)
         self._virtual_disk = {}
         self.multi = isinstance(mpo, (list, tuple))
         if self.multi:
@@ -153,10 +215,13 @@
             return [self._mo(m, idx) for m in mpo]
         return mpo.device(idx, self.eng) if hasattr(mpo, "device") else _as_w(self.eng, mpo[idx])
 
-    def _step(self, tensor, ms, mo, domain, ms_conj):
+    def _step(self, tensor, ms, mo, domain, ms_conj, result_qn=None):
         if isinstance(mo, list):
             return contract_one_site_multi_mpo(tensor, ms, mo, domain, ms_conj=ms_conj)
-        return contract_one_site(tensor, ms, mo, domain, ms_conj=ms_conj)
+        return contract_one_site(tensor, ms, mo, domain, ms_conj=ms_conj, result_qn=result_qn)
+
+    def _pattern(self, mps, mpo, domain, idx):
+        return _result_qn(mps, mpo, domain, idx) if self.qn_pattern and not self.multi else None
 
     def _construct(self, mps, mpo, domain=None, mps_conj=None):
         assert domain in ["L", "R", None]
@@ -171,7 +236,7 @@
         tensor = self.sentinel
         for idx in rng:
             cj = None if mps_conj is None else mps_conj[idx]
-            tensor = self._step(tensor, mps[idx], self._mo(mpo, idx), domain, cj)
+            tensor = self._step(tensor, mps[idx], self._mo(mpo, idx), domain, cj, self._pattern(mps, mpo, domain, idx))
             self.write(domain, idx, tensor)
 
     def GetLR(self, domain, siteidx, mps, mpo, itensor=None, method="Scratch", mps_conj=None, canonical=False):
@@ -185,7 +250,7 @@
             itensor = self.sentinel
             sites = range(siteidx + 1) if domain == "L" else range(len(mps) - 1, siteidx - 1, -1)
             for i in sites:
-                itensor = self._step(itensor, mps[i], self._mo(mpo, i), domain, mps_conj[i])
+                itensor = self._step(itensor, mps[i], self._mo(mpo, i), domain, mps_conj[i], self._pattern(mps, mpo, domain, i))
         elif method == "Enviro":
             itensor = self.read(domain, siteidx)
         else:
@@ -193,9 +258,11 @@
                 itensor = self.read(domain, siteidx + (-1 if domain == "L" else 1))
             mo = self._mo(mpo, siteidx)
             if canonical and not isinstance(mo, list) and mps_conj[siteidx] is None and hasattr(mpo, "device"):
-                itensor = contract_one_site(itensor, mps[siteidx], mo, domain, canonical_mo_host=mpo[siteidx])
+                itensor = contract_one_site(itensor, mps[siteidx], mo, domain, canonical_mo_host=mpo[siteidx],
+                                            result_qn=self._pattern(mps, mpo, domain, siteidx))
             else:
-                itensor = self._step(itensor, mps[siteidx], mo, domain, mps_conj[siteidx])
+                itensor = self._step(itensor, mps[siteidx], mo, domain, mps_conj[siteidx],
+                                     self._pattern(mps, mpo, domain, siteidx))
             self.write(domain, siteidx, itensor)
         return itensor
 
diff --git a/renormalizer_amd/mps/mps.py b/renormalizer_amd/mps/mps.py
--- a/renormalizer_amd/mps/mps.py
+++ b/renormalizer_amd/mps/mps.py
@@ -1399,7 +1399,7 @@
         ahead = "R" if mps.to_right else "L"
         environ = _carried_environ(mps, mpo, ahead, self.carry)
         if environ is None:
-            environ = Environ(mps, mpo, ahead)
+            environ = Environ(mps, mpo, ahead, qn_pattern=True)
         self.environ = environ
         self.local_steps = []
         self.q = len(mps.qntot)
```

Result: no change. 617.7, median of 6 (+1.2%).
